# JohannesErnst/WeaSAL

Hardware: AMD Instinct MI355X
Metric: points/sec fwd+bwd KPFCNN on DALES spheres; achieved HBM GB/s on KPConv gather (higher is better)
Workload: dtype f32; 1 GPU; DALES_PseudoLabel KP-FCNN, in_radius=10m, 50k pts/sphere, batch=8, fp32, step = GPU pyramid + fwd + loss + bwd + SGD; contrast_loss term included (trainer_PseudoLabel.py:204-208); pyramid of the next batch overlapped on a second stream; parallelism=dp1, dist_world_size=1, allreduce_bytes=0

## Files before the change

### include/weasal_hip.h

```cpp
#ifndef WEASAL_HIP_H
#define WEASAL_HIP_H

#include <stdint.h>

#ifdef __cplusplus
extern "C" {
#endif

typedef enum {
    WS_OK = 0,
    WS_ERR_INVALID = 1,
    WS_ERR_UNSUPPORTED = 2,
    WS_ERR_HIP = 3,
    WS_ERR_EMPTY = 4,
    WS_ERR_CAPACITY = 5
} ws_status;

enum { WS_INFLUENCE_LINEAR = 0, WS_INFLUENCE_CONSTANT = 1, WS_INFLUENCE_GAUSSIAN = 2 };
enum { WS_AGGREGATION_SUM = 0, WS_AGGREGATION_CLOSEST = 1 };

const char* ws_last_error(void);
int64_t ws_launch_count(void);
const char* ws_version(void);
int ws_device_count(void);
// ... 137 lines not shown
int ws_subsample_ws_create(ws_subsample_ws** ws);
void ws_subsample_ws_destroy(ws_subsample_ws* ws);
int ws_grid_subsample_plan(ws_subsample_ws* ws, const float* points, int64_t n,
                           const int32_t* h_lens, int32_t nb, float dl, int32_t max_p,
                           int32_t order_mode, int32_t* h_out_lens, int64_t* h_m, void* stream);
int ws_grid_subsample_fill(ws_subsample_ws* ws,
                           const float* features, int32_t fd,
                           const int32_t* labels, int32_t ld,
                           float* out_points, float* out_features, int32_t* out_labels,
                           uint64_t* out_keys,
                           int32_t* out_counts,
                           void* stream);

int ws_rotate_clouds(const float* points, int64_t n, const int32_t* lens , int32_t nb,
                     const float* rot , int32_t transpose, float* out, void* stream);

int ws_rotate_clouds_host(const float* points, int64_t n, const int32_t* h_lens, int32_t nb,
                          const float* h_rot, int32_t transpose, float* out, void* stream);

#define WS_PYRAMID_MAX_LEVELS 8
#define WS_PYRAMID_MAX_BATCH 64
typedef struct ws_pyramid_desc {
    int32_t n_levels, nb, want_grids, want_tables;
    const float* points;
    int64_t n0;
    const float* h_rot;
    void* arena; int64_t arena_bytes;
    void* scratch; int64_t scratch_bytes;
    int32_t conv_on[WS_PYRAMID_MAX_LEVELS], pool_on[WS_PYRAMID_MAX_LEVELS];
    float r_conv[WS_PYRAMID_MAX_LEVELS], r_pool[WS_PYRAMID_MAX_LEVELS], r_up[WS_PYRAMID_MAX_LEVELS], dl[WS_PYRAMID_MAX_LEVELS];
    int32_t limit[WS_PYRAMID_MAX_LEVELS + 1];
    int32_t nearest_up;
    int32_t lens[WS_PYRAMID_MAX_LEVELS][WS_PYRAMID_MAX_BATCH];
    int64_t needed_bytes;
    int64_t n[WS_PYRAMID_MAX_LEVELS];
    int64_t off_points[WS_PYRAMID_MAX_LEVELS], off_neighbors[WS_PYRAMID_MAX_LEVELS], off_pools[WS_PYRAMID_MAX_LEVELS],
            off_upsamples[WS_PYRAMID_MAX_LEVELS], off_order[WS_PYRAMID_MAX_LEVELS], off_key_last[WS_PYRAMID_MAX_LEVELS],
            off_blob[WS_PYRAMID_MAX_LEVELS], blob_bytes[WS_PYRAMID_MAX_LEVELS], grid_cells[WS_PYRAMID_MAX_LEVELS];
    int64_t off_lens, off_slots;
    int32_t max_count[3 * WS_PYRAMID_MAX_LEVELS], width[3 * WS_PYRAMID_MAX_LEVELS], final_width[3 * WS_PYRAMID_MAX_LEVELS];
    int32_t cap[3 * WS_PYRAMID_MAX_LEVELS];
    int64_t off_toffsets[3 * WS_PYRAMID_MAX_LEVELS], off_tpairs[3 * WS_PYRAMID_MAX_LEVELS];
} ws_pyramid_desc;
int ws_pyramid_build(ws_neighbors_ws* nws, ws_subsample_ws* sws, ws_pyramid_desc* desc, void* stream);
int64_t ws_pyramid_desc_bytes(void);



int ws_contrast_rows_fwd(const float* on, int64_t n, int32_t c, const float* xs, int32_t s, const int64_t* slc_idx,
                         const uint8_t* certain, const int64_t* lbl, float temperature, float eps, float* loss,
                         float* rowmax, float* den, float* npos, void* stream);
int64_t ws_contrast_rows_bwd_scratch_bytes(int64_t n, int32_t c, int32_t s);
int ws_contrast_rows_bwd(const float* on, int64_t n, int32_t c, const float* xs, int32_t s, const int64_t* slc_idx,
                         const uint8_t* certain, const int64_t* lbl, float temperature, const float* rowmax,
                         const float* den, const float* npos, const float* g, float* d_on, float* d_xs, void* scratch,
                         void* stream);

int64_t ws_contrast_head_scratch_bytes(int64_t n);
int ws_contrast_head_fwd(const float* x, int64_t n, int32_t c, int64_t ldx, const int64_t* labels, float threshold,
                         const float* u, const int64_t* r_given, int32_t s, float* on, float* inv_norm, uint8_t* certain,
                         int64_t* lbl, int64_t* slc_idx, float* xs, int32_t* state, void* scratch, void* stream);
int64_t ws_contrast_tail_scratch_bytes(int64_t n);
int ws_contrast_tail_fwd(const float* pts_loss, const int64_t* lbl, int64_t n, int32_t n_cls, int32_t* state, float* per_class,
                         float* w_cls, float* loss, void* scratch, void* stream);
int ws_contrast_tail_bwd(const float* pts_loss, const int64_t* lbl, int64_t n, int32_t n_cls, const float* w_cls, const float* g,
                         float* g_row, void* stream);
int ws_contrast_head_bwd(float* d_on, const float* d_xs, const int64_t* slc_idx, int32_t s, const float* on,
                         const float* inv_norm, int64_t n, int32_t c, float* d_x, int64_t ldd, void* stream);


int ws_kpconv_gather_fwd_bf16(const float* q_pts, int64_t nq, const float* s_pts, int64_t ns, const int64_t* inds, int32_t h,
                              const uint16_t* x, int32_t ci, const float* kernel_points, int32_t k, const float* deformed_kp,
                              const float* modulations, float extent, int32_t influence, int32_t aggregation,
                              const int32_t* order, uint16_t* wf, float* min_d2, void* stream);
int ws_kpconv_gather_bwd_x_bf16(const float* q_pts, int64_t nq, const float* s_pts, int64_t ns, const int64_t* inds, int32_t h,
                                const int32_t* t_offsets, const int32_t* t_pairs, const uint16_t* dwf, int32_t ci,
                                const float* kernel_points, int32_t k, const float* deformed_kp, const float* modulations,
                                float extent, int32_t influence, int32_t aggregation, const int32_t* order, uint16_t* dx,
                                void* stream);
int ws_kpconv_gather_bwd_x_grid_bf16(const float* s_pts, int64_t ns, const void* grid_blob, int32_t nb, int64_t cells,
                                     const uint64_t* key_last, float radius, const uint16_t* dwf, int32_t ci,
                                     const float* kernel_points, int32_t k, const float* deformed_kp, const float* modulations,
                                     float extent, int32_t influence, int32_t aggregation, const int32_t* order, uint16_t* dx,
                                     int32_t* overflow, void* stream);
int ws_kpconv_gather_bwd_geom_bf16(const float* q_pts, int64_t nq, const float* s_pts, int64_t ns, const int64_t* inds, int32_t h,
                                   const uint16_t* x, int32_t ci, const uint16_t* dwf, const float* kernel_points, int32_t k,
                                   const float* deformed_kp, const float* modulations, const float* d_min_d2, float extent,
                                   int32_t influence, int32_t aggregation, float* d_deformed_kp, float* d_modulations,
                                   void* stream);
int ws_max_pool_fwd_bf16(const uint16_t* x, int64_t ns, int32_t c, const int64_t* inds, int64_t nq, int32_t h,
                         uint16_t* out, int32_t* arg, void* stream);
int ws_max_pool_bwd_bf16(const uint16_t* dy, const int32_t* arg, int64_t nq, int32_t h, int32_t c, const int32_t* t_offsets,
                         const int32_t* t_pairs, int64_t ns, uint16_t* dx, void* stream);
int ws_closest_pool_fwd_bf16(const uint16_t* x, int64_t ns, int32_t c, const int64_t* inds, int64_t nq, int32_t h,
                             uint16_t* out, void* stream);
int ws_closest_pool_bwd_bf16(const uint16_t* dy, int64_t nq, int32_t h, int32_t c, const int32_t* t_offsets,
                             const int32_t* t_pairs, int64_t ns, uint16_t* dx, void* stream);

int ws_gemm_xbt_bf16(const uint16_t* x, int64_t m, int32_t k, int64_t ldx, const uint16_t* bt, int32_t n, int64_t ldbt,
                     const float* bias, const uint16_t* residual, int64_t ldr, int32_t act, float slope,
                     void* y, int64_t ldy, int32_t out_f32, void* stream);
int ws_gemm_xty_bf16(const uint16_t* x, int64_t m, int32_t k, int64_t ldx, const uint16_t* y, int32_t n, int64_t ldy,
                     float* out, void* scratch, void* stream);
int64_t ws_act_bwd_colsum_bf16_scratch_bytes(int64_t m, int32_t n);
int ws_act_bwd_colsum_bf16(const void* dy, int32_t dy_f32, int64_t m, int32_t n, int64_t lddy, const uint16_t* y, int64_t ldy,
                           float slope, uint16_t* dz, int64_t lddz, float* colsum, void* scratch, void* stream);


typedef struct ws_kpblock {
    const float* q_pts; int64_t nq;
    const float* s_pts; int64_t ns;
    const int64_t* inds; int32_t h;
    const float* kernel_points; int32_t k; float extent;
    const int32_t* order_q;
    const int32_t* order_s;
    const void* grid_blob; int32_t grid_nb; int64_t grid_cells; const uint64_t* key_last; float grid_radius;
    int32_t* grid_overflow;
    const int32_t* t_offsets; const int32_t* t_pairs;
    int32_t in_dim, conv_in, conv_out, out_dim, strided;
    float slope;
    const float *w1, *b1, *wk, *bk, *w2, *b2, *ws, *bs;
    const float* feat; float* x1; float* wf; float* x2; float* pooled; int32_t* arg; float* out;
    const float* dout; float* dfeat; float *dw1, *db1, *dwk, *dbk, *dw2, *db2, *dws;
    int32_t timed;
    int32_t rows_sorted;
    int32_t infer;
    int32_t dout_pregated;
    int32_t gate_dfeat;
    const float* dfeat_add;
} ws_kpblock;

int64_t ws_kpblock_fwd_scratch_bytes(const ws_kpblock* d);
int64_t ws_kpblock_bwd_scratch_bytes(const ws_kpblock* d);
int ws_kpblock_fwd(const ws_kpblock* d, void* scratch, int64_t scratch_bytes, void* stream);
int ws_kpblock_bwd(const ws_kpblock* d, void* scratch, int64_t scratch_bytes, void* stream);

typedef struct ws_upunary {
    const float* xc; int64_t nc; int32_t c_up;
    const float* skip; int64_t nf; int32_t c_skip;
    const int64_t* ups; int32_t h_up;
    const int32_t* t_offsets; const int32_t* t_pairs;
    const float* w; int64_t ldw; const float* b; int32_t out_dim; int32_t relu; float slope;
    float* yc; float* out;
    const float* dout; float* dxc; float* dskip; float* dw; float* db;
    float drop_p; uint64_t drop_seed;
    int32_t dout_pregated;
    int32_t gate_dxc;
} ws_upunary;

int64_t ws_upunary_fwd_scratch_bytes(const ws_upunary* d);
int64_t ws_upunary_bwd_scratch_bytes(const ws_upunary* d);
int ws_upunary_fwd(const ws_upunary* d, void* scratch, int64_t scratch_bytes, void* stream);
int ws_upunary_bwd(const ws_upunary* d, void* scratch, int64_t scratch_bytes, void* stream);

int ws_gemm_xb_epilogue_strided(const float* x, int64_t m, int32_t k, int64_t ldx, const float* b, int64_t b_row_stride,
                                int64_t b_col_stride, int32_t n, const float* bias, const float* residual, int64_t ldr,
                                int32_t act, float slope, float* y, int64_t ldy, void* scratch, int64_t scratch_bytes,
                                void* stream);

int ws_gemm_xb_dropout_strided(const float* x, int64_t m, int32_t k, int64_t ldx, const float* b, int64_t b_row_stride,
                               int64_t b_col_stride, int32_t n, const float* bias, const float* residual, int64_t ldr,
                               int32_t act, float slope, float drop_p, uint64_t drop_seed, float* y, int64_t ldy, void* scratch,
                               int64_t scratch_bytes, void* stream);

int ws_gemm_xb_gate_dropout(const float* x, int64_t m, int32_t k, int64_t ldx, const float* b, int32_t n, const float* gate_y,
                            int64_t ldg, float gate_slope, float drop_p, uint64_t drop_seed, float* y, int64_t ldy, void* scratch,
                            int64_t scratch_bytes, void* stream);

int ws_act_bwd_colsum_dropout(const float* dy, int64_t m, int32_t n, int64_t lddy, const float* y, int64_t ldy, float slope,
                              float drop_p, uint64_t drop_seed, float* dz, int64_t lddz, float* colsum, void* scratch, void* stream);

int ws_gemm_xb_gated_strided(const float* x, int64_t m, int32_t k, int64_t ldx, const float* b, int64_t b_row_stride,
                             int64_t b_col_stride, int32_t n, const float* bias, const float* residual, int64_t ldr,
                             int32_t act, float slope, const float* gate_y, int64_t ldg, float gate_slope, const uint8_t* mask,
                             int64_t ldm, float mask_scale, float* y, int64_t ldy, void* scratch, int64_t scratch_bytes,
                             void* stream);

int ws_timer_reset(void);
int ws_timer_count(void);
int ws_timer_read(int32_t i, int64_t* nq, int32_t* h, int32_t* ci, float* ms);
int ws_timer_read_layer(int32_t i, float* ms);


int ws_vote_update(const float* logits, int64_t n, int32_t c, const float* points, float radius_mask, const int64_t* inds,
                   float* probs, int64_t n_cloud, float smooth, void* stream);
int ws_project_confusion(const float* probs, int32_t c, const int32_t* proj, int64_t m, const int32_t* labels, int32_t* preds,
                         int32_t nc, int64_t* confusion, void* stream);
int64_t ws_potentials_scratch_bytes(int64_t n);
int ws_potentials_update(const float* pot_points, int64_t n, const double* h_center, double radius, double* potentials,
                         double* out_min, int64_t* out_argmin, void* scratch, void* stream);

int ws_al_point_scores(const float* probs, int64_t n, int32_t c, const double* class_score, float* entropy, int32_t* preds,
                       double* score, void* stream);
int ws_al_anchor_scores(const float* entropy, const int32_t* preds, int64_t n, const int64_t* anchor_ptr, const int64_t* anchor_idx,
                        int64_t nnz, int64_t n_anchors, const double* class_score, int32_t c, float* out, void* stream);
int64_t ws_topk_scratch_bytes(int64_t n, int64_t k);
int ws_topk_select(const double* score, int64_t n, const int64_t* h_exclude, int64_t m, int64_t k, int64_t* ids, void* scratch,
                   void* stream);

enum { WS_REFINE_BAD_ANCHOR_IDX = 0, WS_REFINE_BAD_ANCHOR_SEL = 1, WS_REFINE_BAD_PROJ = 2, WS_REFINE_STATUS_WORDS = 3 };
int ws_weak_mask(uint32_t* mask, int64_t n, int32_t c, const int64_t* anchor_ptr, const int64_t* anchor_idx, int64_t nnz,
                 const uint32_t* anchor_bits, int64_t n_anchors, const int64_t* anchor_sel, int64_t n_sel, int64_t* status,
                 void* stream);
int ws_refine_labels(const float* probs, const int32_t* preds, int64_t m, int32_t c, const uint32_t* mask, const int32_t* proj,
                     int64_t n, double thr, int32_t no_label, int32_t* labels, int64_t* counts, int32_t n_counts, int64_t* status,
                     void* stream);

enum { WS_ANCHOR_BAD_LABEL = 0, WS_ANCHOR_BAD_SEL = 1, WS_ANCHOR_STATUS_WORDS = 2 };
enum { WS_ANCHOR_TOTAL_ROWS = 0, WS_ANCHOR_TOTAL_NNZ = 1, WS_ANCHOR_TOTAL_BASE = 2, WS_ANCHOR_TOTAL_WORDS = 3 };
int ws_anchor_bounds(const float* points, int64_t n, float* bounds, void* stream);
int64_t ws_anchor_scratch_bytes(int64_t items);
int ws_anchor_members_plan(const float* points, const int32_t* labels, int64_t n, int32_t n_class, const double* anchors, int64_t a0,
                           double radius, const double* h_grid, const int32_t* cell_start, const int32_t* cell_item,
                           int32_t* counts, int32_t* slot, int32_t* ptr32, uint32_t* bits, int64_t* totals, int64_t* status,
                           void* scratch, void* stream);
int ws_anchor_members_fill(const float* points, int64_t n, const double* anchors, int64_t a0, double radius, const double* h_grid,
                           const int32_t* cell_start, const int32_t* cell_item, int32_t* counts, const int32_t* slot,
                           const int32_t* ptr32, const uint32_t* bits, int64_t n_kept, int64_t nnz, int64_t* kept, int64_t* anchor_ptr,
                           int64_t* anchor_idx, double* centres, uint32_t* anchor_bits, int32_t* cursor, void* stream);
int ws_anchor_pairs_plan(const double* centres, int64_t n_anchors, const int64_t* sel, int64_t n_sel, double radius,
                         const double* h_grid, const int32_t* cell_start, const int32_t* cell_item, int32_t* pair_cnt,
                         int32_t* pair_ptr, int64_t* totals, int64_t* status, void* scratch, void* stream);
int ws_anchor_pairs_fill(const double* centres, int64_t n_anchors, const int64_t* sel, int64_t n_sel, double radius,
                         const double* h_grid, const int32_t* cell_start, const int32_t* cell_item, const int32_t* pair_ptr,
                         int64_t n_pairs, int32_t* pair_i, int32_t* pair_j, void* stream);
int ws_anchor_overlap_plan(const int64_t* anchor_ptr, const int64_t* anchor_idx, int64_t nnz, const uint32_t* anchor_bits,
                           int64_t n_anchors, const int64_t* sel, int64_t n_sel, const int32_t* pair_i, const int32_t* pair_j,
                           int64_t n_pairs, int32_t* inter_cnt, int32_t* new_slot, int32_t* new_ptr, int32_t* sel_ptr, int64_t* totals,
                           void* scratch, void* stream);
int ws_anchor_overlap_fill(const float* points, int64_t n, const int64_t* anchor_ptr, const int64_t* anchor_idx, int64_t nnz,
                           const uint32_t* anchor_bits, const double* centres, int64_t n_anchors, const int64_t* sel, int64_t n_sel,
                           const int32_t* pair_i, const int32_t* pair_j, int64_t n_pairs, const int32_t* inter_cnt,
                           const int32_t* new_slot, const int32_t* new_ptr, const int32_t* sel_ptr, int64_t n_new, int64_t nnz_new,
                           int64_t nnz_sel, int64_t* out_ptr, int64_t* out_idx, uint32_t* out_bits, double* out_centres, void* stream);

enum { WS_REGION_TOTAL_ROWS = 0, WS_REGION_TOTAL_NNZ = 1, WS_REGION_BAD_LABEL = 2, WS_REGION_WORDS = 3 };
enum { WS_REGION_MAX_SPHERES = 64, WS_REGION_MAX_WIDTH = 256 };
int64_t ws_region_scratch_bytes(int64_t pairs);
int ws_region_cut_count(const double* centres, const int64_t* anchor_ptr, const int64_t* anchor_idx, int64_t anchor_nnz,
                        int64_t n_anchors, const int32_t* group, int32_t n_group, int32_t n_spheres, const double* sphere_centres,
                        const int64_t* row_off, const int64_t* pair_off, const int64_t* input_inds, int64_t n_rows, int64_t pairs,
                        double radius, int32_t* cnt, void* stream);
int ws_region_cut_scan(int32_t* cnt, int64_t pairs, int32_t* slot, int32_t* ptr32, const int64_t* labels, const int64_t* row_off,
                       int64_t n_rows, int32_t n_spheres, int32_t n_class, float* cloud_lb, int64_t* words, void* scratch, void* stream);
int ws_region_cut_fill(const int64_t* anchor_ptr, const int64_t* anchor_idx, int64_t anchor_nnz, const uint32_t* anchor_bits,
                       int64_t n_anchors, const int32_t* group, int32_t n_group, int32_t n_spheres, const int64_t* row_off,
                       const int64_t* pair_off, const int64_t* input_inds, int64_t n_rows, int64_t pairs, const int32_t* cnt,
                       const int32_t* slot, const int32_t* ptr32, int64_t n_regions, int64_t nnz, int32_t n_class, int64_t* out_ptr,
                       int64_t* out_idx, int32_t* out_reg, int32_t* out_sphere, int64_t* out_anchor, float* out_lb, float* out_inv_len,
                       void* stream);
int ws_region_mean_fwd(const float* x, int64_t n, int32_t w, const int64_t* region_ptr, const int64_t* region_idx, int64_t nnz,
                       const float* inv_len, int64_t n_regions, float* out, void* stream);
int ws_region_mean_bwd(const float* grad_out, int64_t n_regions, int32_t w, const int64_t* t_ptr, const int32_t* t_reg, int64_t nnz,
                       const float* inv_len, int64_t n, float* grad_x, void* stream);

typedef struct ws_sampler ws_sampler;
int ws_sampler_create(ws_sampler** ws);
void ws_sampler_destroy(ws_sampler* ws);
int ws_sampler_add_cloud(ws_sampler* ws, const float* sub_points, const int32_t* sub_labels, int64_t n, const float* pot_points,
                         double* potentials, int64_t p, void* stream);
int64_t ws_sampler_state_bytes(void);
int64_t ws_sampler_draw_bytes(void);
int ws_sampler_batch(ws_sampler* ws, const void* h_draws, int32_t max_spheres, int32_t resume, int64_t batch_limit, double in_radius,
                     float augment_noise, uint64_t seed, uint64_t seq0, int32_t fd, const int32_t* label_lut, int32_t lut_n,
                     int32_t labels_zero, int32_t update_potentials, float* out_points, float* out_features, int64_t* out_labels,
                     int64_t* out_input_inds, int32_t* out_lengths, float* out_scales, float* out_rots, int32_t* out_cloud_inds,
                     int32_t* out_point_inds, int64_t capacity_rows, void* d_state, void* stream);

int ws_dropout_apply(const float* in, int64_t n, float p, uint64_t seed, float* out, void* stream);

int64_t ws_softmax_ce_scratch_bytes(int64_t n);
int ws_softmax_ce_fwd(const float* logits, int64_t n, int32_t c, int64_t ldl, const int64_t* labels, const int64_t* lut,
                      int32_t lut_n, const float* class_w, float* loss, float* wsum, void* scratch, void* stream);
int ws_softmax_ce_bwd(const float* logits, int64_t n, int32_t c, int64_t ldl, const int64_t* labels, const int64_t* lut,
                      int32_t lut_n, const float* class_w, const float* grad_loss, const float* wsum, float* dlogits, int64_t ldd,
                      void* stream);
int ws_sgd_step(float* const* h_params, const float* const* h_grads, float* const* h_bufs, const int64_t* h_sizes, int32_t count,
                float lr, float momentum, float weight_decay, float clip_value, int32_t first, void* stream);

int ws_kpconv_deform_prepare(const float* offset_features, int64_t n, int32_t od, const float* kernel_points, int32_t k,
                             float extent, int32_t modulated, float* deformed_kp, float* modulations, float* kp4, float* kp_rmax,
                             void* stream);
int ws_kpconv_deform_prepare_bwd(const float* d_kp4, const float* d_deformed_kp, const float* kp4, int64_t n, int32_t od, int32_t k,
                                 float extent, int32_t modulated, float* d_offset_features, void* stream);
int ws_kpconv_gather_fwd_def(const float* q_pts, int64_t nq, const float* s_pts, int64_t ns, const int64_t* inds, int32_t h,
                             const void* x, int32_t ci, const float* kp4, int32_t k, float extent, const int32_t* order,
                             void* wf, float* min_d2, int32_t rows_bf16, int32_t rows_sorted, void* stream);
int ws_kpconv_gather_fwd_ex(const float* q_pts, int64_t nq, const float* s_pts, int64_t ns, const int64_t* inds, int32_t h,
                            const void* x, int32_t ci, const float* kernel_points, int32_t k, const float* deformed_kp,
                            const float* modulations, float extent, int32_t influence, int32_t aggregation, const int32_t* order,
                            void* wf, float* min_d2, int32_t rows_bf16, int32_t rows_sorted, void* stream);
int ws_kpconv_gather_bwd_x_def(const float* q_pts, int64_t nq, const float* s_pts, int64_t ns, int32_t h,
                               const int32_t* t_offsets, const int32_t* t_pairs, const void* dwf, int32_t ci, const float* kp4,
                               int32_t k, float extent, const int32_t* order, void* dx, int32_t rows_bf16, void* stream);
int ws_kpconv_gather_bwd_x_grid_wide(const float* s_pts, int64_t ns, const void* grid_blob, int32_t nb, int64_t cells,
                                     const uint64_t* key_last, float radius, const void* dwf, int32_t ci,
                                     const float* kernel_points, int32_t k, const float* kp4, const float* kp_rmax, float extent,
                                     const int32_t* order, const int64_t* rows, int32_t rows_h, void* dx, int32_t rows_bf16,
                                     void* stream);
int ws_kpconv_gather_bwd_geom_def(const float* q_pts, int64_t nq, const float* s_pts, int64_t ns, const int64_t* inds, int32_t h,
                                  const void* x, int32_t ci, const void* dwf, const float* kp4, int32_t k, const float* d_min_d2,
                                  float extent, const int32_t* order, float* d_kp4, int32_t rows_bf16, int32_t rows_sorted,
                                  void* stream);
int ws_kpconv_layer_fwd_fused(const float* q_pts, int64_t nq, const float* s_pts, int64_t ns, const int64_t* inds, int32_t h,
                              const float* x, int32_t ci, const float* kernel_points, int32_t k, float extent,
                              const int32_t* order, const float* weights, int32_t co, const float* bias, int32_t act, float slope,
// ... 47 lines not shown
```

### weasal_amd/_lib.py

```python
import ctypes as C
import os

_HERE = os.path.dirname(os.path.abspath(__file__))
LIB_PATH = os.path.join(_HERE, "libweasal_hip.so")

_vp = C.c_void_p
_i32 = C.c_int32
_i64 = C.c_int64
_f32 = C.c_float

SIGNATURES = {
    "ws_last_error": (C.c_char_p, []),
    "ws_version": (C.c_char_p, []),
    "ws_device_count": (C.c_int, []),
    "ws_kpconv_gather_fwd": (C.c_int, [_vp, _i64, _vp, _i64, _vp, _i32, _vp, _i32, _vp, _i32, _vp, _vp,
                                      _f32, _i32, _i32, _vp, _vp, _vp, _vp]),
    "ws_kpconv_gather_bwd_x": (C.c_int, [_vp, _i64, _vp, _i64, _vp, _i32, _vp, _vp, _vp, _i32, _vp, _i32,
                                        _vp, _vp, _f32, _i32, _i32, _vp, _vp, _vp]),
    "ws_kpconv_gather_bwd_geom": (C.c_int, [_vp, _i64, _vp, _i64, _vp, _i32, _vp, _i32, _vp, _vp, _i32,
                                           _vp, _vp, _vp, _f32, _i32, _i32, _vp, _vp, _vp]),
    "ws_transpose_scratch_bytes": (_i64, [_i64, _i32, _i64]),
    "ws_transpose_build": (C.c_int, [_vp, _i64, _i32, _i64, _vp, _vp, _vp, _vp]),
    "ws_max_pool_fwd": (C.c_int, [_vp, _i64, _i32, _vp, _i64, _i32, _vp, _vp, _vp]),
    "ws_max_pool_bwd": (C.c_int, [_vp, _vp, _i64, _i32, _i32, _vp, _vp, _i64, _vp, _vp]),
    "ws_closest_pool_fwd": (C.c_int, [_vp, _i64, _i32, _vp, _i64, _i32, _vp, _vp]),
    "ws_closest_pool_bwd": (C.c_int, [_vp, _i64, _i32, _i32, _vp, _vp, _i64, _vp, _vp]),
    "ws_gemm_xb": (C.c_int, [_vp, _i64, _i32, _i64, _vp, _i32, _vp, _i64, _vp]),
    "ws_gemm_xb_epilogue": (C.c_int, [_vp, _i64, _i32, _i64, _vp, _i32, _vp, _vp, _i64, _i32, _f32, _vp, _i64, _vp]),
    "ws_act_bwd_colsum_scratch_bytes": (_i64, [_i64, _i32]),
    "ws_act_bwd_colsum": (C.c_int, [_vp, _i64, _i32, _i64, _vp, _i64, C.c_float, _vp, _i64, _vp, _vp, _vp]),
    "ws_contrast_rows_fwd": (C.c_int, [_vp, _i64, _i32, _vp, _i32, _vp, _vp, _vp, C.c_float, C.c_float, _vp, _vp, _vp, _vp, _vp]),
    "ws_contrast_rows_bwd_scratch_bytes": (_i64, [_i64, _i32, _i32]),
    "ws_contrast_rows_bwd": (C.c_int, [_vp, _i64, _i32, _vp, _i32, _vp, _vp, _vp, C.c_float, _vp, _vp, _vp, _vp, _vp, _vp,
                                       _vp, _vp]),
    "ws_launch_count": (_i64, []),
    "ws_radius_neighbors_async_cap": (_i32, [_i32]),
    "ws_radius_neighbors_nearest_async": (C.c_int, [_vp, _vp, _i64, _vp, _i64, _vp, _vp, _i32, C.c_float, _vp, _vp, _vp, _vp]),
    "ws_max_pool_fwd_ordered": (C.c_int, [_vp, _i64, _i32, _vp, _i64, _i32, _vp, _vp, _vp, _vp]),
    "ws_max_pool_bwd_ordered": (C.c_int, [_vp, _vp, _i64, _i32, _i32, _vp, _vp, _i64, _vp, _vp, _vp]),
    "ws_max_pool_fwd_ordered_bf16": (C.c_int, [_vp, _i64, _i32, _vp, _i64, _i32, _vp, _vp, _vp, _vp]),
    "ws_max_pool_bwd_ordered_bf16": (C.c_int, [_vp, _vp, _i64, _i32, _i32, _vp, _vp, _i64, _vp, _vp, _vp]),
    "ws_dropout_apply": (C.c_int, [_vp, _i64, C.c_float, C.c_uint64, _vp, _vp]),
    "ws_gemm_xb_dropout_strided": (C.c_int, [_vp, _i64, _i32, _i64, _vp, _i64, _i64, _i32, _vp, _vp, _i64, _i32, _f32, _f32, C.c_uint64,
                                             _vp, _i64, _vp, _i64, _vp]),
    "ws_gemm_xb_gate_dropout": (C.c_int, [_vp, _i64, _i32, _i64, _vp, _i32, _vp, _i64, _f32, _f32, C.c_uint64, _vp, _i64, _vp, _i64, _vp]),
    "ws_act_bwd_colsum_dropout": (C.c_int, [_vp, _i64, _i32, _i64, _vp, _i64, _f32, _f32, C.c_uint64, _vp, _i64, _vp, _vp, _vp]),
    "ws_pyramid_build": (C.c_int, [_vp, _vp, _vp, _vp]),
    "ws_pyramid_desc_bytes": (_i64, []),
    "ws_contrast_head_scratch_bytes": (_i64, [_i64]),
    "ws_contrast_head_fwd": (C.c_int, [_vp, _i64, _i32, _i64, _vp, C.c_float, _vp, _vp, _i32, _vp, _vp, _vp, _vp, _vp, _vp, _vp,
                                       _vp, _vp]),
    "ws_contrast_tail_scratch_bytes": (_i64, [_i64]),
    "ws_contrast_tail_fwd": (C.c_int, [_vp, _vp, _i64, _i32, _vp, _vp, _vp, _vp, _vp, _vp]),
    "ws_contrast_tail_bwd": (C.c_int, [_vp, _vp, _i64, _i32, _vp, _vp, _vp, _vp]),
    "ws_contrast_head_bwd": (C.c_int, [_vp, _vp, _vp, _i32, _vp, _vp, _i64, _i32, _vp, _i64, _vp]),
    "ws_radius_neighbors_set_key_last": (C.c_int, [_vp, _vp]),
    "ws_radius_neighbors_reuse_grid": (C.c_int, [_vp, _i32]),
    "ws_radius_neighbors_grid_info": (C.c_int, [_vp, _vp, _vp, _vp, _vp]),
    "ws_radius_neighbors_grid_export": (C.c_int, [_vp, _vp, _vp]),
    "ws_kpconv_gather_bwd_x_grid": (C.c_int, [_vp, _i64, _vp, _i32, _i64, _vp, C.c_float, _vp, _i32, _vp, _i32, _vp, _vp,
                                              C.c_float, _i32, _i32, _vp, _vp, _vp, _vp]),
    "ws_gemm_xb_scratch_bytes": (_i64, [_i64, _i32, _i32]),
    "ws_gemm_xb_epilogue_splitk": (C.c_int, [_vp, _i64, _i32, _i64, _vp, _i32, _vp, _vp, _i64, _i32, C.c_float, _vp, _i64,
                                             _vp, _i64, _vp]),
    "ws_gemm_xty_scratch_bytes": (_i64, [_i64, _i32, _i32]),
    "ws_gemm_xty": (C.c_int, [_vp, _i64, _i32, _i64, _vp, _i32, _i64, _vp, _vp, _vp]),
    "ws_neighbors_ws_create": (C.c_int, [C.POINTER(_vp)]),
    "ws_neighbors_ws_destroy": (None, [_vp]),
    "ws_radius_neighbors_plan": (C.c_int, [_vp, _vp, _i64, _vp, _i64, _vp, _vp, _i32, _f32,
                                          C.POINTER(_i32), _vp]),
    "ws_radius_neighbors_fill": (C.c_int, [_vp, _i32, _vp, _vp, _vp]),
    "ws_radius_neighbors_search": (C.c_int, [_vp, _vp, _i64, _vp, _i64, _vp, _vp, _i32, _f32, _i32, _vp, _vp,
                                            C.POINTER(_i32), _vp]),
    "ws_radius_neighbors_search_async": (C.c_int, [_vp, _vp, _i64, _vp, _i64, _vp, _vp, _i32, _f32, _i32, _vp, _vp,
                                                  _vp, _vp]),
    "ws_radius_neighbors_order": (C.c_int, [_vp, _vp, _vp]),
    "ws_radius_neighbors_counts": (_vp, [_vp]),
    "ws_subsample_ws_create": (C.c_int, [C.POINTER(_vp)]),
    "ws_subsample_ws_destroy": (None, [_vp]),
    "ws_grid_subsample_plan": (C.c_int, [_vp, _vp, _i64, _vp, _i32, _f32, _i32, _i32, _vp,
                                        C.POINTER(_i64), _vp]),
    "ws_grid_subsample_fill": (C.c_int, [_vp, _vp, _i32, _vp, _i32, _vp, _vp, _vp, _vp, _vp, _vp]),
    "ws_rotate_clouds": (C.c_int, [_vp, _i64, _vp, _i32, _vp, _i32, _vp, _vp]),
    "ws_rotate_clouds_host": (C.c_int, [_vp, _i64, _vp, _i32, _vp, _i32, _vp, _vp]),
    "ws_kpconv_gather_fwd_bf16": (C.c_int, [_vp, _i64, _vp, _i64, _vp, _i32, _vp, _i32, _vp, _i32, _vp, _vp,
                                           _f32, _i32, _i32, _vp, _vp, _vp, _vp]),
    "ws_kpconv_gather_bwd_x_bf16": (C.c_int, [_vp, _i64, _vp, _i64, _vp, _i32, _vp, _vp, _vp, _i32, _vp, _i32,
                                             _vp, _vp, _f32, _i32, _i32, _vp, _vp, _vp]),
    "ws_kpconv_gather_bwd_geom_bf16": (C.c_int, [_vp, _i64, _vp, _i64, _vp, _i32, _vp, _i32, _vp, _vp, _i32,
                                                _vp, _vp, _vp, _f32, _i32, _i32, _vp, _vp, _vp]),
    "ws_kpconv_gather_bwd_x_grid_bf16": (C.c_int, [_vp, _i64, _vp, _i32, _i64, _vp, C.c_float, _vp, _i32, _vp, _i32, _vp, _vp,
                                                   C.c_float, _i32, _i32, _vp, _vp, _vp, _vp]),
    "ws_max_pool_fwd_bf16": (C.c_int, [_vp, _i64, _i32, _vp, _i64, _i32, _vp, _vp, _vp]),
    "ws_max_pool_bwd_bf16": (C.c_int, [_vp, _vp, _i64, _i32, _i32, _vp, _vp, _i64, _vp, _vp]),
    "ws_closest_pool_fwd_bf16": (C.c_int, [_vp, _i64, _i32, _vp, _i64, _i32, _vp, _vp]),
    "ws_closest_pool_bwd_bf16": (C.c_int, [_vp, _i64, _i32, _i32, _vp, _vp, _i64, _vp, _vp]),
    "ws_gemm_xbt_bf16": (C.c_int, [_vp, _i64, _i32, _i64, _vp, _i32, _i64, _vp, _vp, _i64, _i32, _f32, _vp, _i64, _i32, _vp]),
    "ws_gemm_xty_bf16": (C.c_int, [_vp, _i64, _i32, _i64, _vp, _i32, _i64, _vp, _vp, _vp]),
    "ws_act_bwd_colsum_bf16_scratch_bytes": (_i64, [_i64, _i32]),
    "ws_act_bwd_colsum_bf16": (C.c_int, [_vp, _i32, _i64, _i32, _i64, _vp, _i64, C.c_float, _vp, _i64, _vp, _vp, _vp]),
    "ws_kpblock_fwd_scratch_bytes": (_i64, [_vp]),
    "ws_kpblock_bwd_scratch_bytes": (_i64, [_vp]),
    "ws_kpblock_fwd": (C.c_int, [_vp, _vp, _i64, _vp]),
    "ws_kpblock_bwd": (C.c_int, [_vp, _vp, _i64, _vp]),
    "ws_upunary_fwd_scratch_bytes": (_i64, [_vp]),
    "ws_upunary_bwd_scratch_bytes": (_i64, [_vp]),
    "ws_upunary_fwd": (C.c_int, [_vp, _vp, _i64, _vp]),
    "ws_upunary_bwd": (C.c_int, [_vp, _vp, _i64, _vp]),
    "ws_gemm_xb_epilogue_strided": (C.c_int, [_vp, _i64, _i32, _i64, _vp, _i64, _i64, _i32, _vp, _vp, _i64, _i32, _f32, _vp, _i64,
                                              _vp, _i64, _vp]),
    "ws_gemm_xb_gated_strided": (C.c_int, [_vp, _i64, _i32, _i64, _vp, _i64, _i64, _i32, _vp, _vp, _i64, _i32, _f32, _vp, _i64, _f32,
                                           _vp, _i64, _f32, _vp, _i64, _vp, _i64, _vp]),
    "ws_kpconv_gather_bwd_x_gated": (C.c_int, [_vp, _i64, _vp, _i64, _vp, _i32, _vp, _vp, _vp, _i32, _vp, _i32,
                                              _vp, _vp, _f32, _i32, _i32, _vp, _vp, _f32, _vp, _vp]),
    "ws_kpconv_gather_bwd_x_packed": (C.c_int, [_vp, _i64, _vp, _i64, _vp, _i32, _vp, _vp, _vp, _i32, _vp, _i32,
                                               _vp, _vp, _f32, _i32, _i32, _vp, _vp, _f32, _vp, _vp]),
    "ws_kpconv_gather_bwd_x_packed_variant": (C.c_int, [_i64, _i64, _i32, _i32, _vp, _vp, _i32, _i32, _i32, _i32, _i32, _i32,
                                                       C.c_char_p, _i32]),
    "ws_kpconv_gather_bwd_x_grid_gated": (C.c_int, [_vp, _i64, _vp, _i32, _i64, _vp, C.c_float, _vp, _i32, _vp, _i32, _vp, _vp,
                                                    C.c_float, _i32, _i32, _vp, _vp, _f32, _vp, _i32, _vp, _vp, _vp]),
    "ws_vote_update": (C.c_int, [_vp, _i64, _i32, _vp, _f32, _vp, _vp, _i64, _f32, _vp]),
    "ws_project_confusion": (C.c_int, [_vp, _i32, _vp, _i64, _vp, _vp, _i32, _vp, _vp]),
    "ws_potentials_scratch_bytes": (_i64, [_i64]),
    "ws_potentials_update": (C.c_int, [_vp, _i64, _vp, C.c_double, _vp, _vp, _vp, _vp, _vp]),
    "ws_al_point_scores": (C.c_int, [_vp, _i64, _i32, _vp, _vp, _vp, _vp, _vp]),
    "ws_al_anchor_scores": (C.c_int, [_vp, _vp, _i64, _vp, _vp, _i64, _i64, _vp, _i32, _vp, _vp]),
    "ws_topk_scratch_bytes": (_i64, [_i64, _i64]),
    "ws_topk_select": (C.c_int, [_vp, _i64, _vp, _i64, _i64, _vp, _vp, _vp]),
    "ws_weak_mask": (C.c_int, [_vp, _i64, _i32, _vp, _vp, _i64, _vp, _i64, _vp, _i64, _vp, _vp]),
    "ws_refine_labels": (C.c_int, [_vp, _vp, _i64, _i32, _vp, _vp, _i64, C.c_double, _i32, _vp, _vp, _i32, _vp, _vp]),
    "ws_anchor_bounds": (C.c_int, [_vp, _i64, _vp, _vp]),
    "ws_anchor_scratch_bytes": (_i64, [_i64]),
    "ws_anchor_members_plan": (C.c_int, [_vp, _vp, _i64, _i32, _vp, _i64, C.c_double, _vp, _vp, _vp, _vp, _vp, _vp, _vp, _vp, _vp,
                                        _vp, _vp]),
    "ws_anchor_members_fill": (C.c_int, [_vp, _i64, _vp, _i64, C.c_double, _vp, _vp, _vp, _vp, _vp, _vp, _vp, _i64, _i64, _vp, _vp,
                                        _vp, _vp, _vp, _vp, _vp]),
    "ws_anchor_pairs_plan": (C.c_int, [_vp, _i64, _vp, _i64, C.c_double, _vp, _vp, _vp, _vp, _vp, _vp, _vp, _vp, _vp]),
    "ws_anchor_pairs_fill": (C.c_int, [_vp, _i64, _vp, _i64, C.c_double, _vp, _vp, _vp, _vp, _i64, _vp, _vp, _vp]),
    "ws_anchor_overlap_plan": (C.c_int, [_vp, _vp, _i64, _vp, _i64, _vp, _i64, _vp, _vp, _i64, _vp, _vp, _vp, _vp, _vp, _vp, _vp]),
    "ws_anchor_overlap_fill": (C.c_int, [_vp, _i64, _vp, _vp, _i64, _vp, _vp, _i64, _vp, _i64, _vp, _vp, _i64, _vp, _vp, _vp, _vp,
                                        _i64, _i64, _i64, _vp, _vp, _vp, _vp, _vp]),
    "ws_region_scratch_bytes": (_i64, [_i64]),
    "ws_region_cut_count": (C.c_int, [_vp, _vp, _vp, _i64, _i64, _vp, _i32, _i32, _vp, _vp, _vp, _vp, _i64, _i64, C.c_double, _vp, _vp]),
    "ws_region_cut_scan": (C.c_int, [_vp, _i64, _vp, _vp, _vp, _vp, _i64, _i32, _i32, _vp, _vp, _vp, _vp]),
    "ws_region_cut_fill": (C.c_int, [_vp, _vp, _i64, _vp, _i64, _vp, _i32, _i32, _vp, _vp, _vp, _i64, _i64, _vp, _vp, _vp, _i64, _i64,
                                    _i32, _vp, _vp, _vp, _vp, _vp, _vp, _vp, _vp]),
    "ws_region_mean_fwd": (C.c_int, [_vp, _i64, _i32, _vp, _vp, _i64, _vp, _i64, _vp, _vp]),
    "ws_region_mean_bwd": (C.c_int, [_vp, _i64, _i32, _vp, _vp, _i64, _vp, _i64, _vp, _vp]),
    "ws_sampler_create": (C.c_int, [C.POINTER(_vp)]),
    "ws_sampler_destroy": (None, [_vp]),
    "ws_sampler_add_cloud": (C.c_int, [_vp, _vp, _vp, _i64, _vp, _vp, _i64, _vp]),
    "ws_sampler_state_bytes": (_i64, []),
    "ws_sampler_draw_bytes": (_i64, []),
    "ws_sampler_batch": (C.c_int, [_vp, _vp, _i32, _i32, _i64, C.c_double, _f32, C.c_uint64, C.c_uint64, _i32, _vp, _i32, _i32, _i32,
                                   _vp, _vp, _vp, _vp, _vp, _vp, _vp, _vp, _vp, _i64, _vp, _vp]),
    "ws_softmax_ce_scratch_bytes": (_i64, [_i64]),
    "ws_softmax_ce_fwd": (C.c_int, [_vp, _i64, _i32, _i64, _vp, _vp, _i32, _vp, _vp, _vp, _vp, _vp]),
    "ws_softmax_ce_bwd": (C.c_int, [_vp, _i64, _i32, _i64, _vp, _vp, _i32, _vp, _vp, _vp, _vp, _i64, _vp]),
    "ws_sgd_step": (C.c_int, [_vp, _vp, _vp, _vp, _i32, _f32, _f32, _f32, _f32, _i32, _vp]),
    "ws_kpconv_deform_prepare": (C.c_int, [_vp, _i64, _i32, _vp, _i32, _f32, _i32, _vp, _vp, _vp, _vp, _vp]),
    "ws_kpconv_gather_fwd_ex": (C.c_int, [_vp, _i64, _vp, _i64, _vp, _i32, _vp, _i32, _vp, _i32, _vp, _vp, _f32, _i32, _i32, _vp,
                                         _vp, _vp, _i32, _i32, _vp]),
    "ws_kpconv_deform_prepare_bwd": (C.c_int, [_vp, _vp, _vp, _i64, _i32, _i32, _f32, _i32, _vp, _vp]),
    "ws_kpconv_gather_fwd_def": (C.c_int, [_vp, _i64, _vp, _i64, _vp, _i32, _vp, _i32, _vp, _i32, _f32, _vp, _vp, _vp, _i32, _i32, _vp]),
    "ws_kpconv_gather_bwd_x_def": (C.c_int, [_vp, _i64, _vp, _i64, _i32, _vp, _vp, _vp, _i32, _vp, _i32, _f32, _vp, _vp, _i32, _vp]),
    "ws_kpconv_gather_bwd_x_grid_wide": (C.c_int, [_vp, _i64, _vp, _i32, _i64, _vp, _f32, _vp, _i32, _vp, _i32, _vp, _vp, _f32, _vp,
                                                   _vp, _i32, _vp, _i32, _vp]),
    "ws_kpconv_gather_bwd_geom_def": (C.c_int, [_vp, _i64, _vp, _i64, _vp, _i32, _vp, _i32, _vp, _vp, _i32, _vp, _f32, _vp, _vp,
                                                _i32, _i32, _vp]),
    "ws_kpconv_layer_fwd_fused": (C.c_int, [_vp, _i64, _vp, _i64, _vp, _i32, _vp, _i32, _vp, _i32, _f32, _vp, _vp, _i32, _vp, _i32, _f32,
                                           _vp, _vp]),
    "ws_kpconv_gather_fwd_variant": (C.c_int, [_i32, _i32, _i32, _i32, _i32, _i32, C.c_char_p, _i32]),
    "ws_kpconv_gather_variant": (C.c_int, [_i32, _i64, _i64, _i32, _vp, _vp, _i32, _i32, _i32, _i32, _i32, _i32, _i32, C.c_char_p, _i32]),
    "ws_gemm_xb_variant": (C.c_int, [_vp, _i64, _i32, _i64, _vp, _i64, _i64, _i32, _vp, _vp, _i64, _vp, _i64, _vp, _i64, _vp, _i64,
                                     _vp, _i64, C.c_char_p, _i32]),
    "ws_gemm_xty_variant": (C.c_int, [_vp, _i64, _i32, _i64, _vp, _i32, _i64, _vp, _i64, _vp, _i32, C.c_char_p, _i32]),
    "ws_act_bwd_colsum_variant": (C.c_int, [_vp, _i64, _i32, _i64, _vp, _i64, _vp, _i64, _vp, _vp, C.c_char_p, _i32]),
    "ws_gemm_xbt_bf16_variant": (C.c_int, [_i64, _i32, _i32, _vp, _vp, _i64, _vp, _i64, _i32, C.c_char_p, _i32]),
    "ws_act_bwd_colsum_bf16_variant": (C.c_int, [_i32, _i64, _i32, _vp, _vp, C.c_char_p, _i32]),
    "ws_p2p_regularizer_scratch_bytes": (_i64, [_i64]),
    "ws_p2p_regularizer_fwd": (C.c_int, [_vp, _vp, _vp, _i64, _i32, _f32, _f32, _vp, _vp, _vp]),
    "ws_p2p_regularizer_bwd": (C.c_int, [_vp, _vp, _vp, _i64, _i32, _f32, _f32, _vp, _vp, _vp, _vp]),
    "ws_sphere_attention_fwd": (C.c_int, [_vp, _vp, _vp, _i64, _i32, _i32, _vp, _i32, _vp, _vp, _vp, _vp]),
    "ws_sphere_attention_bwd_scratch_bytes": (_i64, [_i64, _i32]),
    "ws_sphere_attention_bwd": (C.c_int, [_vp, _vp, _vp, _vp, _vp, _vp, _vp, _i64, _i32, _i32, _vp, _i32, _vp, _vp, _vp, _vp, _i64, _vp]),
    "ws_channel_attention_scratch_bytes": (_i64, [_vp, _i32, _i32, _i32]),
    "ws_channel_attention_fwd": (C.c_int, [_vp, _vp, _vp, _i64, _i32, _vp, _i32, _i32, _vp, _vp, _vp, _i64, _vp]),
    "ws_channel_attention_bwd": (C.c_int, [_vp, _vp, _vp, _vp, _vp, _i64, _i32, _vp, _i32, _i32, _vp, _vp, _vp, _vp, _i64, _vp]),
    "ws_timer_reset": (C.c_int, []),
    "ws_timer_count": (C.c_int, []),
    "ws_timer_read": (C.c_int, [_i32, _vp, _vp, _vp, _vp]),
    "ws_timer_read_layer": (C.c_int, [_i32, _vp]),
}

ENV_SWITCHES = (
    ("WEASAL_NB_WIDE_CAPS", "ws_nb_wide_caps"),
    ("WEASAL_CLOSEST_BWD_VEC", "ws_closest_bwd_vec"),
    ("WEASAL_GEMM_STAGED", "ws_gemm_staged"),
    ("WEASAL_GEMM_SHALLOW", "ws_gemm_shallow"),
)

_lib = None


class WeasalHipError(RuntimeError):
    pass


def lib():
    global _lib
    if _lib is None:
        if not os.path.exists(LIB_PATH):
            raise WeasalHipError(
                "%s not found: build it with `python -c 'import __graft_entry__ as g; g.build()'` "
                "or `make -C weasal_amd/csrc` (there is no CPU fallback)" % LIB_PATH)
        handle = C.CDLL(LIB_PATH)
        for name, (res, args) in SIGNATURES.items():
            fn = getattr(handle, name)
            fn.restype = res
            fn.argtypes = args
        for env, sym in ENV_SWITCHES:
            if env in os.environ:
                C.c_int.in_dll(handle, sym).value = int(os.environ[env])
        _lib = handle
    return _lib


def check(rc):
    if rc != 0:
        msg = lib().ws_last_error()
        raise WeasalHipError("libweasal_hip status %d: %s" % (rc, msg.decode() if msg else "?"))


def ptr(t):
    return None if t is None else _vp(t.data_ptr())


_raw_stream = None


def current_stream():
    global _raw_stream
    import torch
    if _raw_stream is None:
        get = getattr(torch._C, "_cuda_getCurrentRawStream", None)
        dev = getattr(torch._C, "_cuda_getDevice", None)
        if get is not None and dev is not None and torch.cuda.is_available():
            torch.cuda.current_stream()
            _raw_stream = lambda: get(dev())
        else:
            _raw_stream = lambda: torch.cuda.current_stream().cuda_stream
    return _vp(_raw_stream())
```

### weasal_amd/architectures.py

```python
import os

import numpy as np
import torch
import torch.nn as nn

from . import fused, ops
from .blocks import KPConv, NearestUpsampleBlock, UnaryBlock, block_decider, closest_pool
from .regions import SphereRegions

_LAYER_CHANGE = ('pool', 'strided', 'upsample', 'global')
REGULARIZER_KERNEL = os.environ.get("WEASAL_REG_KERNEL", "1") != "0"
DROPOUT_KERNEL = os.environ.get("WEASAL_DROPOUT_KERNEL", "1") != "0"
DROPOUT_FUSED = os.environ.get("WEASAL_DROPOUT_FUSED", "1") != "0"
CONTRAST_KERNELS = os.environ.get("WEASAL_CONTRAST_KERNELS", "1") != "0"


def p2p_fitting_regularizer(net):
    fitting_loss = 0
    repulsive_loss = 0
    layers = getattr(net, "_deformable_layers", None)
    if layers is None:
        layers = [m for m in net.modules() if isinstance(m, KPConv) and m.deformable]
        net._deformable_layers = layers
    for m in layers:
        if REGULARIZER_KERNEL and m.min_d2.is_cuda and net.K == 15 and ops.kpconv_gather is ops._KPCONV_GATHER_SELF:
            fr = ops.p2p_regularizer(m.deformed_KP, m.min_d2, m.KP_extent, net.repulse_extent)
            fitting_loss = fitting_loss + fr[0]
            repulsive_loss = repulsive_loss + fr[1]
            continue
        kp_min_d2 = m.min_d2 / (m.KP_extent ** 2)
        fitting_loss = fitting_loss + net.l1(kp_min_d2, torch.zeros_like(kp_min_d2))
        locs = m.deformed_KP / m.KP_extent
        diff = locs.unsqueeze(2) - locs.detach().unsqueeze(1)
        off_diag = ~torch.eye(net.K, dtype=torch.bool, device=locs.device)
        dist = torch.sqrt(torch.sum(diff ** 2, dim=3) + (~off_diag).to(locs.dtype))
        pen = torch.clamp_max(dist - net.repulse_extent, max=0.0) ** 2
        rep = torch.sum(pen * off_diag, dim=2)
        repulsive_loss = repulsive_loss + torch.sum(torch.mean(torch.abs(rep), dim=0)) / net.K
    return net.deform_fitting_power * (2 * fitting_loss + repulsive_loss)


class KPFCNN(nn.Module):

    def __init__(self, config, lbl_values, ign_lbls):
        super(KPFCNN, self).__init__()
        arch = list(config.architecture)
        layer = 0
        r = config.first_subsampling_dl * config.conv_radius
        in_dim = config.in_features_dim
        out_dim = config.first_features_dim
        self.K = config.num_kernel_points
        self.C = len(lbl_values) - len(ign_lbls)

        self.encoder_blocks = nn.ModuleList()
        self.encoder_skip_dims = []
        self.encoder_skips = []
        for block_i, block in enumerate(arch):
            if 'equivariant' in block and out_dim % 3 != 0:
                raise ValueError('Equivariant block but features dimension is not a factor of 3')
            if any(tag in block for tag in _LAYER_CHANGE):
                self.encoder_skips.append(block_i)
                self.encoder_skip_dims.append(in_dim)
            if 'upsample' in block:
                break
            self.encoder_blocks.append(block_decider(block, r, in_dim, out_dim, layer, config))
            in_dim = out_dim // 2 if 'simple' in block else out_dim
            if 'pool' in block or 'strided' in block:
                layer += 1
                r *= 2
                out_dim *= 2

        self.decoder_blocks = nn.ModuleList()
        self.decoder_concats = []
        start_i = next((i for i, b in enumerate(arch) if 'upsample' in b), 0)
        for block_i, block in enumerate(arch[start_i:]):
            if block_i > 0 and 'upsample' in arch[start_i + block_i - 1]:
                in_dim += self.encoder_skip_dims[layer]
                self.decoder_concats.append(block_i)
            self.decoder_blocks.append(block_decider(block, r, in_dim, out_dim, layer, config))
            in_dim = out_dim
            if 'upsample' in block:
                layer -= 1
                r *= 0.5
                out_dim = out_dim // 2

        self.head_mlp = UnaryBlock(out_dim, config.first_features_dim, False, 0)
        self.head_softmax = UnaryBlock(config.first_features_dim, self.C, False, 0)
        self.dropout = config.dropout
        if config.dropout:
            self.droplayer = nn.Dropout(p=float(config.dropout))

        self.valid_labels = np.sort([c for c in lbl_values if c not in ign_lbls])
        if len(config.class_w) > 0:
            class_w = torch.from_numpy(np.array(config.class_w, dtype=np.float32))
            self.criterion = torch.nn.CrossEntropyLoss(weight=class_w, ignore_index=-1)
        else:
            self.criterion = torch.nn.CrossEntropyLoss(ignore_index=-1)
        self.deform_fitting_mode = config.deform_fitting_mode
        self.deform_fitting_power = config.deform_fitting_power
        self.deform_lr_factor = config.deform_lr_factor
        self.repulse_extent = config.repulse_extent
        self.output_loss = 0
        self.reg_loss = 0
        self.l1 = nn.L1Loss()
        self.fuse_decoder = True
        self.feature_dtype = torch.bfloat16 if getattr(config, 'feature_dtype', 'f32') == 'bf16' else torch.float32
        if self.feature_dtype == torch.bfloat16:
            self.head_softmax.out_f32 = True

    def _fused_upsample_unary(self, x, skip, up_block, unary, batch, drop=None):
        if fused.upunary_eligible(x, skip, unary):
            return fused.upunary(x, skip, unary, batch.upsamples[up_block.layer_ind - 1], drop, batch)
        assert drop is None
        c_up = x.shape[1]
        w = unary.mlp.weight
        y = closest_pool(ops.linear(x, w[:, :c_up]), batch.upsamples[up_block.layer_ind - 1])
        return ops.matmul_epilogue(skip, w[:, c_up:].t(), bias=unary.batch_norm.epilogue_bias(), residual=y,
                                   slope=None if unary.no_relu else 0.1)

    def forward(self, batch, config):
        if hasattr(batch, "activate"):
            batch.activate()
        else:
            ops.clear_batch_hints()
        x = batch.features.clone().detach()
        skips = []
        slots = []
        link = None
        for block_i, block_op in enumerate(self.encoder_blocks):
            slot = None
            if block_i in self.encoder_skips:
                skips.append(x)
                slot = fused.SkipSlot()
                slots.append(slot)
            batch.skip_slot = slot
            batch.gate_link_in, batch.gate_link_out = link, fused.GateLink()
            link = batch.gate_link_out
            x = block_op(x, batch)
            batch.skip_slot = None
            batch.gate_link_in = batch.gate_link_out = None
            if block_i == 0 and self.feature_dtype == torch.bfloat16 and x.dtype == torch.float32 and x.shape[1] % 32 == 0:
                x = x.to(torch.bfloat16)
        nd = len(self.decoder_blocks)
        block_i = 0
        dropped = False
        while block_i < nd:
            block_op = self.decoder_blocks[block_i]
            nxt = self.decoder_blocks[block_i + 1] if block_i + 1 < nd else None
            if (self.fuse_decoder and isinstance(block_op, NearestUpsampleBlock) and isinstance(nxt, UnaryBlock)
                    and (block_i + 1) in self.decoder_concats and block_i not in self.decoder_concats):
                drop = None
                if (block_i + 2 == nd and self.dropout and DROPOUT_KERNEL and DROPOUT_FUSED and self.training and not nxt.no_relu
                        and torch.is_grad_enabled() and x.dtype == torch.float32 and fused.upunary_eligible(x, skips[-1], nxt)):
                    drop = (float(self.dropout), int(torch.randint(0, 1 << 62, (1,)).item()))
                    dropped = True
                batch.gate_link_in, batch.gate_link_out = link, fused.GateLink()
                link = batch.gate_link_out
                x = self._fused_upsample_unary(x, fused.skip_tap(skips.pop(), slots.pop()), block_op, nxt, batch, drop)
                batch.gate_link_in = batch.gate_link_out = None
                block_i += 2
                continue
            if block_i in self.decoder_concats:
                x = torch.cat([x, fused.skip_tap(skips.pop(), slots.pop())], dim=1)
            link = None
            x = block_op(x, batch)
            block_i += 1
        if self.dropout and not dropped:
            link = None
            if DROPOUT_KERNEL and self.training and x.is_cuda and x.dtype == torch.float32 and x.requires_grad:
                x = ops.dropout(x, float(self.dropout))
            else:
                x = self.droplayer(x)
        batch.gate_link_in, batch.gate_link_out = link, fused.GateLink()
        link = batch.gate_link_out
        x = self.head_mlp(x, batch)
        batch.gate_link_in, batch.gate_link_out = link, None
        x = self.head_softmax(x, batch)
        batch.gate_link_in = None
        return x

    def _label_lut(self, device):
        lut = getattr(self, "_target_lut", None)
        if lut is None or lut.device != device:
            vmax = int(max(int(np.max(self.valid_labels)) if len(self.valid_labels) else 0, 0))
            lut = -torch.ones(vmax + 2, dtype=torch.int64)
            for i, c in enumerate(self.valid_labels):
                if 0 <= int(c) <= vmax:
                    lut[int(c)] = i
            lut = lut.to(device)
            self._target_lut = lut
        return lut

    def _targets(self, labels):
        lut = self._label_lut(labels.device)
        idx = torch.where((labels >= 0) & (labels < lut.shape[0] - 1), labels, torch.full_like(labels, lut.shape[0] - 1))
        return lut[idx]

    def loss(self, outputs, labels):
        self.output_loss = ops.cross_entropy(outputs, labels, self._label_lut(labels.device), self.criterion.weight)
        if self.deform_fitting_mode == 'point2point':
            self.reg_loss = p2p_fitting_regularizer(self)
        elif self.deform_fitting_mode == 'point2plane':
            raise ValueError('point2plane fitting mode not implemented yet.')
        else:
            raise ValueError('Unknown fitting mode: ' + self.deform_fitting_mode)
        return self.output_loss + self.reg_loss

    def contrast_loss(self, outputs, labels, config, threshold=0.2, slice_draw=None):
        temperature = 0.1
        base_temperature = 1
        slc_con = 1000
        dev = outputs.device
        N = outputs.shape[0]
        eps = 1e-8
        threshold = config.contrast_thd / 100
        self.pts_loss = 0
        self.pts_loss_self = 0

        if CONTRAST_KERNELS and outputs.is_cuda and outputs.dtype == torch.float32 and outputs.shape[1] <= 16:
            if slice_draw is None:
                draw = torch.rand(slc_con, device=dev)
            else:
                slice_draw = slice_draw.to(dev).to(torch.int64)
                nv_host = slc_con - slice_draw.shape[0]
                draw = slice_draw if nv_host <= 0 else torch.cat((torch.arange(nv_host, device=dev), slice_draw), dim=0)
            loss, self.pts_loss, self.contrast_slice, _ = ops.contrast_loss(outputs, labels, draw, threshold, temperature, eps)
            return loss if base_temperature == 1 else loss / base_temperature

        prob = torch.softmax(outputs, 1)
        pseudo_logits = prob.max(1)[0]
        label_id = labels < 10
        certain_label = (pseudo_logits > threshold) | label_id
        pseudo_lbs = torch.argmax(prob, dim=1)
        pseudo_lbs = torch.where(label_id, labels.to(pseudo_lbs.dtype), pseudo_lbs)
        cs = torch.cumsum(certain_label.to(torch.int64), dim=0)
        num_valid = cs[-1]
        j = torch.arange(slc_con, device=dev)
        if slice_draw is None:
            u = torch.rand(slc_con, device=dev)
            r_rand = (u * num_valid.to(torch.float32)).floor().to(torch.int64)
            r = torch.where((num_valid < slc_con) & (j < num_valid), j, r_rand)
        else:
            slice_draw = slice_draw.to(dev).to(torch.int64)
            nv_host = slc_con - slice_draw.shape[0]
            r = slice_draw if nv_host <= 0 else torch.cat((torch.arange(nv_host, device=dev), slice_draw), dim=0)
        r = torch.minimum(r, (num_valid - 1).clamp(min=0).to(torch.int64))
        slc_idx = torch.searchsorted(cs, r + 1).clamp(max=N - 1)

        outputs = nn.functional.normalize(outputs, dim=1)
        pts_loss = ops.contrast_rows(outputs, outputs[slc_idx], slc_idx, certain_label, pseudo_lbs, temperature, eps)
        if base_temperature != 1:
            pts_loss = pts_loss / base_temperature
        keep = (pts_loss > 0).to(pts_loss.dtype)
        n_cls = max(int(outputs.shape[1]), 10)
        sums = torch.zeros(n_cls, dtype=pts_loss.dtype, device=dev).index_add(0, pseudo_lbs, pts_loss * keep)
        cnts = torch.zeros(n_cls, dtype=pts_loss.dtype, device=dev).index_add(0, pseudo_lbs, keep)
        per_class = sums / cnts.clamp(min=1)
        sel = (per_class > 0).to(pts_loss.dtype)
        self.pts_loss = per_class
        loss = (per_class * sel).sum() / sel.sum()
        return torch.where(num_valid > 0, loss, torch.zeros((), dtype=loss.dtype, device=dev))

    def accuracy(self, outputs, labels):
        target = self._targets(labels)
        predicted = torch.argmax(outputs.data, dim=1)
        return (predicted == target).sum().item() / target.size(0)


class KPFCNN_mprm(nn.Module):

    def __init__(self, config, lbl_values, ign_lbls):
        super(KPFCNN_mprm, self).__init__()
        from .blocks import ele_att, global_average_block, multi_path_att
        arch = list(config.architecture)
        layer = 0
        r = config.first_subsampling_dl * config.conv_radius
        in_dim = config.in_features_dim
        out_dim = config.first_features_dim
        self.K = config.num_kernel_points
        self.C = len(lbl_values) - len(ign_lbls)
        self.features_layer = 'encoder_blocks.5.unary_shortcut.mlp'
        self.forward_features = {}
        self.backward_features = {}

        self.encoder_blocks = nn.ModuleList()
        self.encoder_skip_dims = []
        self.encoder_skips = []
        for block_i, block in enumerate(arch):
            if 'equivariant' in block and out_dim % 3 != 0:
                raise ValueError('Equivariant block but features dimension is not a factor of 3')
            if any(tag in block for tag in _LAYER_CHANGE + ('attention',)):
                self.encoder_skips.append(block_i)
                self.encoder_skip_dims.append(in_dim)
            if 'attention' in block or 'upsample' in block:
                break
            self.encoder_blocks.append(block_decider(block, r, in_dim, out_dim, layer, config))
            in_dim = out_dim // 2 if 'simple' in block else out_dim
            if 'pool' in block or 'strided' in block:
                layer += 1
                r *= 2
                out_dim *= 2

        nc = config.num_classes
        self.multi_att = multi_path_att('attention', out_dim, out_dim, r, layer, config)
        self.ele_head = ele_att('ele_attention', 2, out_dim, r, layer, config)
        self.no_ga = global_average_block('ga1', nc, nc, layer, config)
        self.da_ga = global_average_block('ga2', nc, nc, layer, config)
        self.spa_ga = global_average_block('ga3', nc, nc, layer, config)
# ... 121 lines not shown
```

### weasal_amd/csrc/blocks.hip

```cpp
#include <vector>

#include "ws_common.h"

extern "C" int ws_block_gates = 1;
extern "C" int ws_block_gather_residual = 1;
extern "C" int64_t ws_block_group_rows = (int64_t)1 << 62;
extern "C" int ws_block_fused_infer = 1;
extern "C" int ws_block_pool_order = 1;
extern "C" int ws_block_packed_k4 = 1;

namespace {

struct Arena {
    char* base;
    int64_t cap, off;
    Arena(void* b, int64_t c) : base((char*)b), cap(c), off(0) {}
    template <typename T> T* take(int64_t count)
    {
        off = (off + 255) & ~(int64_t)255;
        T* p = base ? reinterpret_cast<T*>(base + off) : nullptr;
        off += count * (int64_t)sizeof(T);
        return p;
    }
    bool fits() const { return off <= cap; }
};

inline int64_t arena_bytes(const Arena& ar) { return ((ar.off + 255) & ~(int64_t)255) + 256; }

inline int64_t max3(int64_t a, int64_t b, int64_t c) { return a > b ? (a > c ? a : c) : (b > c ? b : c); }

__global__ __launch_bounds__(256) void transpose_small_kernel(const float* __restrict__ w, int rows, int cols, int64_t ld,
                                                               float* __restrict__ out)
{
    const int64_t e = (int64_t)blockIdx.x * 256 + threadIdx.x;
    if (e >= (int64_t)rows * cols) return;
    const int c = (int)(e / rows), r = (int)(e % rows);
    out[e] = w[(int64_t)r * ld + c];
}

__global__ __launch_bounds__(256) void add_rows_kernel(float* __restrict__ a, const float* __restrict__ b, int64_t n4)
{
    for (int64_t e = (int64_t)blockIdx.x * 256 + threadIdx.x; e < n4; e += (int64_t)gridDim.x * 256) {
        float4 x = reinterpret_cast<float4*>(a)[e];
        const float4 y = reinterpret_cast<const float4*>(b)[e];
        x.x += y.x; x.y += y.y; x.z += y.z; x.w += y.w;
        reinterpret_cast<float4*>(a)[e] = x;
    }
}

struct Lin {
    const float* w; int n, k; int64_t ldw;
    bool in_place() const { return k % 32 == 0 && n % 4 == 0 && ldw % 4 == 0 && ((uintptr_t)w & 15u) == 0; }
    int64_t tr_floats() const { return in_place() ? 0 : (int64_t)k * n; }
};

int linear_fwd(const Lin& l, const float* x, int64_t m, int64_t ldx, const float* bias, const float* residual, int64_t ldr,
               int act, float slope, float* y, float* tr, void* tmp, int64_t tmp_bytes, hipStream_t st)
{
    if (l.in_place())
        return ws_gemm_xb_epilogue_strided(x, m, l.k, ldx, l.w, 1, l.ldw, l.n, bias, residual, ldr, act, slope, y, l.n, tmp, tmp_bytes, st);
    transpose_small_kernel<<<(unsigned)ws_ceil_div((int64_t)l.k * l.n, 256), 256, 0, st>>>(l.w, l.n, l.k, l.ldw, tr);
    return ws_gemm_xb_epilogue_strided(x, m, l.k, ldx, tr, l.n, 1, l.n, bias, residual, ldr, act, slope, y, l.n, tmp, tmp_bytes, st);
}

#define WS_TRY(call)            \
    do {                        \
        int rc__ = (call);      \
        if (rc__) return rc__;  \
    } while (0)

inline bool grouped_rows(int64_t rows) { return ws_block_group_rows > 0 && rows > 0 && rows < ws_block_group_rows; }

inline ws_xb_problem xb_problem(const float* x, int64_t m, int k, int64_t ldx, const float* b, int64_t brs, int64_t bcs, int n,
                                const float* bias, const float* residual, int64_t ldr, int act, float slope, const float* gate_y,
                                int64_t ldg, float gate_slope, float* y, int64_t ldy, void* scratch, int64_t scratch_bytes)
{
    ws_xb_problem q{};
    q.x = x; q.m = m; q.k = k; q.ldx = ldx; q.b = b; q.b_row_stride = brs; q.b_col_stride = bcs; q.n = n;
    q.bias = bias; q.residual = residual; q.ldr = ldr; q.act = act; q.slope = slope;
    q.gate_y = gate_y; q.ldg = ldg; q.gate_slope = gate_slope;
    q.y = y; q.ldy = ldy; q.scratch = scratch; q.scratch_bytes = scratch_bytes;
    return q;
}

struct Leaves {
    bool on;
    hipStream_t st;
    ws_xty_problem q[4];
    int n = 0;
    Leaves(bool on_, hipStream_t st_) : on(on_), st(st_) {}
    int add(const float* x, int64_t m, int k, int64_t ldx, const float* y, int nn, int64_t ldy, float* out, int64_t ldo, void* scratch,
            int64_t scratch_bytes)
    {
        if (!on) return ws_priv_gemm_xty_pitched(x, m, k, ldx, y, nn, ldy, out, ldo > nn ? ldo : nn, scratch, st);
        WS_REQUIRE(n < 4, "more than 4 collected weight-gradient products");
        q[n++] = ws_xty_problem{x, m, k, ldx, y, nn, ldy, out, ldo, scratch, scratch_bytes};
        return WS_OK;
    }
    int flush()
    {
        const int c = n;
        n = 0;
        return c ? ws_priv_gemm_xty_group(q, c, st) : WS_OK;
    }
};

struct TimerRec { hipEvent_t a, b, c; int64_t nq; int32_t h, ci; };
std::vector<TimerRec>& timer_recs() { static std::vector<TimerRec> v; return v; }

bool arg_bytes(const ws_kpblock* d)
{
    return d->h <= 255 && d->in_dim % 4 == 0 && ((uintptr_t)d->feat & 15u) == 0 && ((uintptr_t)d->pooled & 15u) == 0 &&
           ((uintptr_t)d->arg & 3u) == 0;
}

int check_kpblock(const ws_kpblock* d)
{
    WS_REQUIRE(d, "NULL descriptor");
    WS_REQUIRE(d->nq >= 0 && d->ns >= 0 && d->h >= 1, "bad sizes nq=%lld ns=%lld h=%d", (long long)d->nq, (long long)d->ns, d->h);
    if (d->k != 15) return ws_fail(WS_ERR_UNSUPPORTED, "num_kernel_points=%d: K=15 only", d->k);
    WS_REQUIRE(d->in_dim >= 1 && d->conv_in >= 1 && d->conv_out >= 1 && d->out_dim >= 1, "bad widths");
    WS_REQUIRE(d->q_pts && d->s_pts && d->inds && d->kernel_points && d->feat && d->wk && (d->wf || d->infer) && d->out, "NULL argument");
    WS_REQUIRE(d->w1 ? (d->x1 != nullptr) : (d->conv_in == d->in_dim), "unary1: x1 buffer missing or conv_in != in_dim");
    WS_REQUIRE(d->w2 ? (d->x2 != nullptr) : (d->out_dim == d->conv_out), "unary2: x2 buffer missing or out_dim != conv_out");
    WS_REQUIRE(!d->w2 || d->ws || d->in_dim == d->out_dim, "shortcut needs a projection (ws) when in_dim != out_dim");
    WS_REQUIRE(!d->strided || !d->w2 || (d->pooled && d->arg), "strided block: pooled / arg buffers missing");
    WS_REQUIRE(d->strided || d->nq == d->ns, "non-strided block: nq must equal ns");
    if (d->conv_out % 4 || d->out_dim % 4 || (d->w1 && d->conv_in % 4) || (d->w2 && d->in_dim % 4))
        return ws_fail(WS_ERR_UNSUPPORTED, "block widths must be multiples of 4 (in=%d conv=%d->%d out=%d)", d->in_dim, d->conv_in,
                       d->conv_out, d->out_dim);
    return WS_OK;
}

int64_t kpblock_tmp_fwd(const ws_kpblock* d)
{
    int64_t t = ws_gemm_xb_scratch_bytes(d->nq, d->k * d->conv_in, d->conv_out);
    if (d->w1) t = max3(t, ws_gemm_xb_scratch_bytes(d->ns, d->in_dim, d->conv_in), 0);
    if (d->w2) t = max3(t, ws_gemm_xb_scratch_bytes(d->nq, d->conv_out, d->out_dim), d->ws ? ws_gemm_xb_scratch_bytes(d->nq, d->in_dim, d->out_dim) : 0);
    return t;
}

int kpblock_fwd(const ws_kpblock* d, Arena& ar, hipStream_t st, bool run)
{
    const int64_t nq = d->nq, ns = d->ns;
    const Lin l1{d->w1, d->conv_in, d->in_dim, d->in_dim}, l2{d->w2, d->out_dim, d->conv_out, d->conv_out},
        lsc{d->ws, d->out_dim, d->in_dim, d->in_dim};
    float* tr1 = d->w1 ? ar.take<float>(l1.tr_floats()) : nullptr;
    float* tr2 = d->w2 ? ar.take<float>(l2.tr_floats()) : nullptr;
    float* trs = d->ws ? ar.take<float>(lsc.tr_floats()) : nullptr;
    float* sc = (d->w2 && d->ws) ? ar.take<float>(nq * d->out_dim) : nullptr;
    const int64_t tmp_bytes = kpblock_tmp_fwd(d);
    void* tmp = ar.take<char>(tmp_bytes > 16 ? tmp_bytes : 16);
    const bool pair_in = grouped_rows(nq) && d->w1 && d->w2 && d->ws && !d->strided && l1.in_place() && lsc.in_place();
    const int64_t sc_bytes = pair_in ? ws_gemm_xb_scratch_bytes(nq, d->in_dim, d->out_dim) : 0;
    void* tmp_sc = pair_in ? (void*)ar.take<char>(sc_bytes > 16 ? sc_bytes : 16) : nullptr;
    if (!run) return WS_OK;
    if (nq == 0) return WS_OK;
    const float* x1 = d->feat;
    if (pair_in) {
        const ws_xb_problem q[2] = {
            xb_problem(d->feat, ns, l1.k, d->in_dim, l1.w, 1, l1.ldw, l1.n, d->b1, nullptr, 0, 1, d->slope, nullptr, 0, 0.0f, d->x1, l1.n,
                       tmp, tmp_bytes),
// ... 103 lines not shown
            else WS_HIP(hipMemsetAsync(d->dfeat, 0, sizeof(float) * (size_t)ns * d->in_dim, st));
        }
        return WS_OK;
    }
    bool gated2 = false;
    Leaves leaves(grp, st);
    const float* sc_res = nullptr;
    bool added = false;
    const float* gin = d->dout;
    const float* yconv = d->out;
    WS_REQUIRE(!(d->gate_dfeat && d->dfeat_add && !(d->strided && want_sc)),
               "gate_dfeat with dfeat_add needs the strided shortcut (the sum has to be complete before the gate)");
    if (d->w2) {
        if (d->dout_pregated) {
            if (d->db2) WS_TRY(ws_act_bwd_colsum(d->dout, nq, d->out_dim, d->out_dim, nullptr, 0, 0.0f, nullptr, 0, d->db2, tmp, st));
            dz = const_cast<float*>(d->dout);
        } else
        WS_TRY(ws_act_bwd_colsum(d->dout, nq, d->out_dim, d->out_dim, d->out, d->out_dim, d->slope, dz, d->out_dim, d->db2, tmp, st));
        WS_TRY(leaves.add(dz, nq, d->out_dim, d->out_dim, d->x2, d->conv_out, d->conv_out, d->dw2, 0, t_dw2, b_dw2));
        if (d->ws) {
            const float* sc_in = d->strided ? d->pooled : d->feat;
            WS_TRY(leaves.add(dz, nq, d->out_dim, d->out_dim, sc_in, d->in_dim, d->in_dim, d->dws, 0, t_dws, b_dws));
        }
        gated2 = !d->dbk && ws_block_gates;
        const bool pair_dz = grp && want_sc && d->ws;
        if (pair_dz) {
            const ws_xb_problem q[2] = {
                xb_problem(dz, nq, d->out_dim, d->out_dim, d->ws, d->in_dim, 1, d->in_dim, nullptr, nullptr, 0, 0, 0.0f, nullptr, 0, 0.0f,
                           dscin, d->in_dim, tmp, tmp_bytes),
                xb_problem(dz, nq, d->out_dim, d->out_dim, d->w2, d->conv_out, 1, d->conv_out, nullptr, nullptr, 0, 0, 0.0f,
                           gated2 ? d->x2 : nullptr, d->conv_out, d->slope, g2, d->conv_out, t_g2, b_g2)};
            WS_TRY(ws_priv_gemm_xb_group(q, 2, st));
        }
        if (want_sc) {
            const float* dsc = dz;
            if (d->ws) {
                if (!pair_dz)
                    WS_TRY(ws_gemm_xb_epilogue_strided(dz, nq, d->out_dim, d->out_dim, d->ws, d->in_dim, 1, d->in_dim, nullptr, nullptr, 0,
                                                       0, 0.0f, dscin, d->in_dim, tmp, tmp_bytes, st));
                dsc = dscin;
            }
            if (d->strided) {
                WS_REQUIRE(d->t_offsets && d->t_pairs, "strided block backward needs the transposed table");
                if (arg_bytes(d))
                {
                    WS_TRY(ws_priv_max_pool_bwd_u8(dsc, reinterpret_cast<const uint8_t*>(d->arg), nq, d->h, d->in_dim, d->t_offsets,
                                                   d->t_pairs, ns, dfsc, ws_block_pool_order ? d->order_s : nullptr, d->dfeat_add, st));
                    added = d->dfeat_add != nullptr;
                }
                else {
                    WS_TRY(ws_max_pool_bwd(dsc, d->arg, nq, d->h, d->in_dim, d->t_offsets, d->t_pairs, ns, dfsc, st));
                    if (d->dfeat_add) {
                        WS_REQUIRE(d->in_dim % 4 == 0, "dfeat_add needs in_dim %% 4 == 0");
                        const int64_t n4 = ns * d->in_dim / 4;
                        add_rows_kernel<<<ws_grid(n4, 256), 256, 0, st>>>(dfsc, d->dfeat_add, n4);
                        WS_LAUNCH_CHECK();
                        added = true;
                    }
                }
                sc_res = dfsc;
            } else {
                sc_res = dsc;
            }
        }
        if (!pair_dz)
            WS_TRY(ws_gemm_xb_gated_strided(dz, nq, d->out_dim, d->out_dim, d->w2, d->conv_out, 1, d->conv_out, nullptr, nullptr, 0, 0, 0.0f,
                                            gated2 ? d->x2 : nullptr, d->conv_out, d->slope, nullptr, 0, 0.0f, g2, d->conv_out, tmp,
                                            tmp_bytes, st));
        gin = g2;
        yconv = d->x2;
    }
    if (!d->w2 && d->dout_pregated) {
        if (d->dbk) WS_TRY(ws_act_bwd_colsum(gin, nq, d->conv_out, d->conv_out, nullptr, 0, 0.0f, nullptr, 0, d->dbk, tmp, st));
        g2 = const_cast<float*>(gin);
    } else if (!gated2)
        WS_TRY(ws_act_bwd_colsum(gin, nq, d->conv_out, d->conv_out, yconv, d->conv_out, d->slope, g2, d->conv_out, d->dbk, tmp, st));
    WS_TRY(leaves.add(d->wf, nq, kc, kc, g2, d->conv_out, d->conv_out, d->dwk, 0, t_dwk, b_dwk));
    if (!need_dx1) return leaves.flush();
    WS_TRY(linear_fwd(lk, g2, nq, d->conv_out, nullptr, nullptr, 0, 0, 0.0f, dwf, trk, tmp, tmp_bytes, st));
    float* dx1_out = d->w1 ? dx1 : d->dfeat;
    const float* gate1 = (d->w1 && !d->db1 && ws_block_gates) ? d->x1 : nullptr;
    if (!d->w1 && d->gate_dfeat && d->dfeat) gate1 = d->feat;
    if (d->grid_blob) {
        WS_REQUIRE(d->key_last && d->grid_overflow && nq == ns, "grid backward needs key_last / overflow and a self-query layer");
        WS_TRY(ws_kpconv_gather_bwd_x_grid_gated(d->s_pts, ns, d->grid_blob, d->grid_nb, d->grid_cells, d->key_last, d->grid_radius, dwf,
                                                 d->conv_in, d->kernel_points, d->k, nullptr, nullptr, d->extent, WS_INFLUENCE_LINEAR,
                                                 WS_AGGREGATION_SUM, d->order_s, gate1, d->slope, d->inds, d->h, dx1_out,
                                                 d->grid_overflow, st));
    } else {
        WS_REQUIRE(d->t_offsets && d->t_pairs, "KPConv backward needs the search grid or the transposed table");
        WS_TRY((ws_block_packed_k4 ? ws_kpconv_gather_bwd_x_packed : ws_kpconv_gather_bwd_x_gated)(
            d->q_pts, nq, d->s_pts, ns, d->inds, d->h, d->t_offsets, d->t_pairs, dwf, d->conv_in, d->kernel_points, d->k, nullptr, nullptr,
            d->extent, WS_INFLUENCE_LINEAR, WS_AGGREGATION_SUM, d->order_s, gate1, d->slope, dx1_out, st));
    }
    if (d->w1) {
        if (!gate1)
            WS_TRY(ws_act_bwd_colsum(dx1, ns, d->conv_in, d->conv_in, d->x1, d->conv_in, d->slope, dx1, d->conv_in, d->db1, tmp, st));
        WS_TRY(leaves.add(dx1, ns, d->conv_in, d->conv_in, d->feat, d->in_dim, d->in_dim, d->dw1, 0, t_dw1, b_dw1));
        if (d->dfeat)
            WS_TRY(ws_gemm_xb_gated_strided(dx1, ns, d->conv_in, d->conv_in, d->w1, d->in_dim, 1, d->in_dim, nullptr, sc_res, d->in_dim,
                                            0, 0.0f, d->gate_dfeat ? d->feat : nullptr, d->in_dim, d->slope, nullptr, 0, 0.0f, d->dfeat,
                                            d->in_dim, tmp, tmp_bytes, st));
    } else if (d->dfeat && sc_res) {
        WS_REQUIRE(!d->gate_dfeat, "gate_dfeat: a block without unary1 has no shortcut to add after the gate");
        const int64_t n4 = ns * d->in_dim / 4;
        add_rows_kernel<<<ws_grid(n4, 256), 256, 0, st>>>(d->dfeat, sc_res, n4);
        WS_LAUNCH_CHECK();
    }
    if (d->dfeat && d->dfeat_add && !added) {
        WS_REQUIRE(d->in_dim % 4 == 0, "dfeat_add needs in_dim %% 4 == 0");
        const int64_t n4 = ns * d->in_dim / 4;
        add_rows_kernel<<<ws_grid(n4, 256), 256, 0, st>>>(d->dfeat, d->dfeat_add, n4);
        WS_LAUNCH_CHECK();
    }
    return leaves.flush();
}

int check_upunary(const ws_upunary* d)
{
    WS_REQUIRE(d, "NULL descriptor");
    WS_REQUIRE(d->nc >= 0 && d->nf >= 0 && d->c_up >= 1 && d->c_skip >= 1 && d->out_dim >= 1 && d->h_up >= 1, "bad sizes");
    WS_REQUIRE(d->xc && d->skip && d->ups && d->w && d->out && d->ldw >= d->c_up + d->c_skip, "NULL argument / bad ldw");
    if (d->c_up % 32 || d->c_skip % 32 || d->out_dim % 32 || d->ldw % 4 || ((uintptr_t)d->w & 15u))
        return ws_fail(WS_ERR_UNSUPPORTED, "decoder step: widths must be multiples of 32 (c_up=%d c_skip=%d out=%d)", d->c_up, d->c_skip,
                       d->out_dim);
    WS_REQUIRE(d->drop_p >= 0.0f && d->drop_p < 1.0f, "bad drop probability %g", (double)d->drop_p);
    if (d->drop_p > 0.0f && !d->relu) return ws_fail(WS_ERR_UNSUPPORTED, "decoder step: the fused dropout follows a LeakyReLU (relu = 0)");
    WS_REQUIRE(!(d->dout_pregated && !d->relu), "dout_pregated needs this step's LeakyReLU");
    return WS_OK;
}

int upunary_fwd(const ws_upunary* d, Arena& ar, hipStream_t st, bool run)
{
    float* up = ar.take<float>(d->nf * d->out_dim);
    const int64_t tmp_bytes = max3(ws_gemm_xb_scratch_bytes(d->nc, d->c_up, d->out_dim), ws_gemm_xb_scratch_bytes(d->nf, d->c_skip, d->out_dim), 16);
    void* tmp = ar.take<char>(tmp_bytes);
    if (!run || d->nf == 0) return WS_OK;
    WS_REQUIRE(d->yc, "yc buffer missing");
    if (d->nc > 0)
        WS_TRY(ws_gemm_xb_epilogue_strided(d->xc, d->nc, d->c_up, d->c_up, d->w, 1, d->ldw, d->out_dim, nullptr, nullptr, 0, 0, 0.0f, d->yc,
                                           d->out_dim, tmp, tmp_bytes, st));
    if (ws_block_gather_residual && d->nc > 0)
        return ws_priv_gemm_xb_ex(d->skip, d->nf, d->c_skip, d->c_skip, d->w + d->c_up, 1, d->ldw, d->out_dim, d->b, d->yc, d->out_dim,
                                  d->ups, d->h_up, d->nc, d->relu ? 1 : 0, d->slope, d->drop_p, d->drop_seed, d->out, d->out_dim, tmp,
                                  tmp_bytes, st);
    WS_TRY(ws_closest_pool_fwd(d->yc, d->nc, d->out_dim, d->ups, d->nf, d->h_up, up, st));
    if (d->drop_p > 0.0f)
        return ws_gemm_xb_dropout_strided(d->skip, d->nf, d->c_skip, d->c_skip, d->w + d->c_up, 1, d->ldw, d->out_dim, d->b, up, d->out_dim,
                                          1, d->slope, d->drop_p, d->drop_seed, d->out, d->out_dim, tmp, tmp_bytes, st);
    return ws_gemm_xb_epilogue_strided(d->skip, d->nf, d->c_skip, d->c_skip, d->w + d->c_up, 1, d->ldw, d->out_dim, d->b, up, d->out_dim,
                                       d->relu ? 1 : 0, d->slope, d->out, d->out_dim, tmp, tmp_bytes, st);
}

int upunary_bwd(const ws_upunary* d, Arena& ar, hipStream_t st, bool run)
{
    float* dz = ar.take<float>(d->nf * d->out_dim);
    float* dyc = ar.take<float>(d->nc * d->out_dim);
    int64_t tmp_bytes = max3(ws_act_bwd_colsum_scratch_bytes(d->nf, d->out_dim), ws_gemm_xty_scratch_bytes(d->nf, d->out_dim, d->c_skip),
                             ws_gemm_xty_scratch_bytes(d->nc, d->out_dim, d->c_up));
    tmp_bytes = max3(tmp_bytes, ws_gemm_xb_scratch_bytes(d->nf, d->out_dim, d->c_skip), ws_gemm_xb_scratch_bytes(d->nc, d->out_dim, d->c_up));
    void* tmp = ar.take<char>(tmp_bytes > 16 ? tmp_bytes : 16);
    const bool grp = grouped_rows(d->nf > d->nc ? d->nf : d->nc) && d->nf > 0 && d->nc > 0;
    const int64_t b_skip = ws_gemm_xty_scratch_bytes(d->nf, d->out_dim, d->c_skip), b_up = ws_gemm_xty_scratch_bytes(d->nc, d->out_dim, d->c_up);
    void* t_skip = grp ? (void*)ar.take<char>(b_skip > 16 ? b_skip : 16) : tmp;
    void* t_up = grp ? (void*)ar.take<char>(b_up > 16 ? b_up : 16) : tmp;
    if (!run) return WS_OK;
    WS_REQUIRE(d->dout && d->dw && d->dxc && d->dskip && d->t_offsets && d->t_pairs, "NULL gradient buffer / table");
    const int64_t cw = d->c_up + d->c_skip;
    if (d->nf == 0 || d->nc == 0) {
        WS_HIP(hipMemsetAsync(d->dw, 0, sizeof(float) * (size_t)d->out_dim * cw, st));
        if (d->db) WS_HIP(hipMemsetAsync(d->db, 0, sizeof(float) * d->out_dim, st));
        if (d->nc > 0) WS_HIP(hipMemsetAsync(d->dxc, 0, sizeof(float) * (size_t)d->nc * d->c_up, st));
        if (d->nf > 0) WS_HIP(hipMemsetAsync(d->dskip, 0, sizeof(float) * (size_t)d->nf * d->c_skip, st));
        return WS_OK;
    }
    const float* g = d->dout;
    if (d->relu && d->dout_pregated) {
        if (d->db) WS_TRY(ws_act_bwd_colsum(d->dout, d->nf, d->out_dim, d->out_dim, nullptr, 0, 0.0f, nullptr, 0, d->db, tmp, st));
    } else if (d->drop_p > 0.0f) {
        WS_TRY(ws_act_bwd_colsum_dropout(d->dout, d->nf, d->out_dim, d->out_dim, d->out, d->out_dim, d->slope, d->drop_p, d->drop_seed, dz,
                                         d->out_dim, d->db, tmp, st));
        g = dz;
    } else if (d->relu) {
        WS_TRY(ws_act_bwd_colsum(d->dout, d->nf, d->out_dim, d->out_dim, d->out, d->out_dim, d->slope, dz, d->out_dim, d->db, tmp, st));
        g = dz;
    } else if (d->db) {
        WS_TRY(ws_act_bwd_colsum(d->dout, d->nf, d->out_dim, d->out_dim, nullptr, 0, 0.0f, nullptr, 0, d->db, tmp, st));
    }
    Leaves leaves(grp, (hipStream_t)st);
    WS_TRY(leaves.add(g, d->nf, d->out_dim, d->out_dim, d->skip, d->c_skip, d->c_skip, d->dw + d->c_up, cw, t_skip, b_skip));
    WS_TRY(ws_gemm_xb_epilogue_strided(g, d->nf, d->out_dim, d->out_dim, d->w + d->c_up, d->ldw, 1, d->c_skip, nullptr, nullptr, 0, 0, 0.0f,
                                       d->dskip, d->c_skip, tmp, tmp_bytes, st));
    WS_TRY(ws_closest_pool_bwd(g, d->nf, 1, d->out_dim, d->t_offsets, d->t_pairs, d->nc, dyc, st));
    WS_TRY(leaves.add(dyc, d->nc, d->out_dim, d->out_dim, d->xc, d->c_up, d->c_up, d->dw, cw, t_up, b_up));
    WS_TRY(ws_gemm_xb_gated_strided(dyc, d->nc, d->out_dim, d->out_dim, d->w, d->ldw, 1, d->c_up, nullptr, nullptr, 0, 0, 0.0f,
                                    d->gate_dxc ? d->xc : nullptr, d->c_up, d->slope, nullptr, 0, 0.0f, d->dxc, d->c_up, tmp, tmp_bytes, st));
    return leaves.flush();
}

}

extern "C" {

int64_t ws_kpblock_fwd_scratch_bytes(const ws_kpblock* d)
{
    if (check_kpblock(d)) return -1;
    Arena ar(nullptr, 0);
    kpblock_fwd(d, ar, nullptr, false);
    return arena_bytes(ar);
}

int64_t ws_kpblock_bwd_scratch_bytes(const ws_kpblock* d)
{
    if (check_kpblock(d)) return -1;
    Arena ar(nullptr, 0);
    kpblock_bwd(d, ar, nullptr, false);
    return arena_bytes(ar);
}

int ws_kpblock_fwd(const ws_kpblock* d, void* scratch, int64_t scratch_bytes, void* stream)
{
    WS_TRY(check_kpblock(d));
    WS_REQUIRE(scratch && ((uintptr_t)scratch & 15u) == 0, "scratch must be a 16-byte aligned device buffer");
    Arena plan(nullptr, 0);
    kpblock_fwd(d, plan, nullptr, false);
    if (arena_bytes(plan) > scratch_bytes) return ws_fail(WS_ERR_CAPACITY, "scratch too small: %lld < %lld bytes", (long long)scratch_bytes, (long long)arena_bytes(plan));
    Arena ar(scratch, scratch_bytes);
    return kpblock_fwd(d, ar, (hipStream_t)stream, true);
}

int ws_kpblock_bwd(const ws_kpblock* d, void* scratch, int64_t scratch_bytes, void* stream)
{
    WS_TRY(check_kpblock(d));
    WS_REQUIRE(scratch && ((uintptr_t)scratch & 15u) == 0, "scratch must be a 16-byte aligned device buffer");
    Arena plan(nullptr, 0);
    kpblock_bwd(d, plan, nullptr, false);
    if (arena_bytes(plan) > scratch_bytes) return ws_fail(WS_ERR_CAPACITY, "scratch too small: %lld < %lld bytes", (long long)scratch_bytes, (long long)arena_bytes(plan));
    Arena ar(scratch, scratch_bytes);
    return kpblock_bwd(d, ar, (hipStream_t)stream, true);
}

int64_t ws_upunary_fwd_scratch_bytes(const ws_upunary* d)
{
    if (check_upunary(d)) return -1;
    Arena ar(nullptr, 0);
    upunary_fwd(d, ar, nullptr, false);
    return arena_bytes(ar);
}

int64_t ws_upunary_bwd_scratch_bytes(const ws_upunary* d)
{
    if (check_upunary(d)) return -1;
    Arena ar(nullptr, 0);
    upunary_bwd(d, ar, nullptr, false);
    return arena_bytes(ar);
}

int ws_upunary_fwd(const ws_upunary* d, void* scratch, int64_t scratch_bytes, void* stream)
{
    WS_TRY(check_upunary(d));
    WS_REQUIRE(scratch && ((uintptr_t)scratch & 15u) == 0, "scratch must be a 16-byte aligned device buffer");
    Arena plan(nullptr, 0);
    upunary_fwd(d, plan, nullptr, false);
    if (arena_bytes(plan) > scratch_bytes) return ws_fail(WS_ERR_CAPACITY, "scratch too small: %lld < %lld bytes", (long long)scratch_bytes, (long long)arena_bytes(plan));
    Arena ar(scratch, scratch_bytes);
    return upunary_fwd(d, ar, (hipStream_t)stream, true);
}

int ws_upunary_bwd(const ws_upunary* d, void* scratch, int64_t scratch_bytes, void* stream)
{
    WS_TRY(check_upunary(d));
    WS_REQUIRE(scratch && ((uintptr_t)scratch & 15u) == 0, "scratch must be a 16-byte aligned device buffer");
    Arena plan(nullptr, 0);
    upunary_bwd(d, plan, nullptr, false);
    if (arena_bytes(plan) > scratch_bytes) return ws_fail(WS_ERR_CAPACITY, "scratch too small: %lld < %lld bytes", (long long)scratch_bytes, (long long)arena_bytes(plan));
    Arena ar(scratch, scratch_bytes);
    return upunary_bwd(d, ar, (hipStream_t)stream, true);
}

int ws_timer_reset(void)
{
    for (auto& r : timer_recs()) {
        (void)hipEventDestroy(r.a);
        (void)hipEventDestroy(r.b);
        (void)hipEventDestroy(r.c);
    }
    timer_recs().clear();
    return WS_OK;
}

int ws_timer_count(void) { return (int)timer_recs().size(); }

int ws_timer_read(int32_t i, int64_t* nq, int32_t* h, int32_t* ci, float* ms)
{
    WS_REQUIRE(i >= 0 && i < (int)timer_recs().size() && nq && h && ci && ms, "bad timer record index %d", i);
    const TimerRec& r = timer_recs()[i];
    WS_HIP(hipEventSynchronize(r.b));
    WS_HIP(hipEventElapsedTime(ms, r.a, r.b));
    *nq = r.nq; *h = r.h; *ci = r.ci;
    return WS_OK;
}

int ws_timer_read_layer(int32_t i, float* ms)
{
    WS_REQUIRE(i >= 0 && i < (int)timer_recs().size() && ms, "bad timer record index %d", i);
    const TimerRec& r = timer_recs()[i];
    WS_HIP(hipEventSynchronize(r.c));
    WS_HIP(hipEventElapsedTime(ms, r.a, r.c));
    return WS_OK;
}

}
```

### weasal_amd/csrc/gemm.hip

```cpp
#include "ws_common.h"
#include "ws_bf16.h"

namespace {

typedef float f32x16 __attribute__((ext_vector_type(16)));

constexpr int BM = 128;
constexpr int BK = 32;

struct XbGate {
    const float* y; int64_t ld; float slope;
    const uint8_t* mask; int64_t ldm; float mscale;
    WsDrop drop; int64_t dn;
    const int64_t* rrows; int64_t rld; int64_t rn;
};
__device__ __forceinline__ const float* xb_res_row(const float* residual, int64_t ldr, const XbGate& g, int64_t row)
{
    if (!residual) return nullptr;
    if (!g.rrows) return residual + row * ldr;
    const int64_t i = g.rrows[row * g.rld];
    return (i >= 0 && i < g.rn) ? residual + i * ldr : nullptr;
}
__device__ __forceinline__ void xb_gate4(float4& v, const XbGate& g, int64_t row, int col)
{
// ... 336 lines not shown
        load_x(c + 1 < last ? c + 1 : last);
        load_w(c + 2 < last ? c + 2 : last);
        const float* wb = &Ws[((c - cbeg) & 1) * WBUF + wn * (NT * 1024) + (h * 32 + idx) * 4];
#pragma unroll
        for (int j = 0; j < 4; ++j) {
            __builtin_amdgcn_sched_barrier(0);
#pragma unroll
            for (int i = 0; i < NT; ++i) {
                const float4 a4 = *reinterpret_cast<const float4*>(wb + (i * 4 + j) * 256);
                acc[i] = __builtin_amdgcn_mfma_f32_32x32x2f32(a4.x, xc[j].x, acc[i], 0, 0, 0);
                acc[i] = __builtin_amdgcn_mfma_f32_32x32x2f32(a4.y, xc[j].y, acc[i], 0, 0, 0);
                acc[i] = __builtin_amdgcn_mfma_f32_32x32x2f32(a4.z, xc[j].z, acc[i], 0, 0, 0);
                acc[i] = __builtin_amdgcn_mfma_f32_32x32x2f32(a4.w, xc[j].w, acc[i], 0, 0, 0);
            }
        }
        __syncthreads();
    }
    if (staged) {
        const int64_t row0 = (int64_t)bx * (32 * WM) + wm * 32;
        float* stage = &Ws[wave * XB_STAGE_FLOATS];
        if (partial)
            xb_rows_epilogue_staged<NT>(acc, row0, m, n0 + wn * (32 * NT), n, lane, partial + (int64_t)bz * m * n, n, nullptr,
                                        nullptr, 0, 0, 0.0f, XbGate{}, stage);
        else
            xb_rows_epilogue_staged<NT>(acc, row0, m, n0 + wn * (32 * NT), n, lane, y, ldy, bias, residual, ldr, act, slope, gate, stage);
        return;
    }
    if (partial)
        xb_rows_epilogue<NT>(acc, row, m, n0 + wn * (32 * NT), n, h, partial + (int64_t)bz * m * n, n, nullptr, nullptr, 0,
                             0, 0.0f, XbGate{});
    else
        xb_rows_epilogue<NT>(acc, row, m, n0 + wn * (32 * NT), n, h, y, ldy, bias, residual, ldr, act, slope, gate);
}

template <int NT, int WN>
__global__ __launch_bounds__(256) __attribute__((amdgpu_waves_per_eu(3))) void gemm_xb2_kernel(
    const float* __restrict__ x, int64_t m, int k, int64_t ldx, const float* __restrict__ b, int n, int ldb, int bcs,
    float* __restrict__ y, int64_t ldy, const float* __restrict__ bias, const float* __restrict__ residual, int64_t ldr,
    int act, float slope, int csplit, float* __restrict__ partial, const XbGate gate, int staged)
{
    gemm_xb2_body<NT, WN>(blockIdx.x, blockIdx.y, blockIdx.z, x, m, k, ldx, b, n, ldb, bcs, y, ldy, bias, residual, ldr, act, slope,
                          csplit, partial, gate, staged);
}

constexpr int GROUP_MAX = 8;
struct GroupIndex { unsigned end[GROUP_MAX]; };
__device__ __forceinline__ int group_find(const GroupIndex& gi, unsigned& local)
{
    const unsigned b = blockIdx.x;
    int i = 0;
    unsigned beg = 0;
#pragma unroll
    for (int j = 0; j < GROUP_MAX - 1; ++j) {
        const bool past = b >= gi.end[j];
        i += past ? 1 : 0;
        beg = past ? gi.end[j] : beg;
    }
    local = b - beg;
    return i;
}

struct Xb2Problem {
    const float* x; int64_t m; int64_t ldx; const float* b; float* y; int64_t ldy; const float* bias; const float* residual;
    int64_t ldr; float* partial; XbGate gate;
    int k, n, ldb, bcs, act, csplit, staged; float slope;
    unsigned gx, gy;
};
struct Xb2Group { GroupIndex gi; Xb2Problem p[GROUP_MAX]; };
static_assert(sizeof(Xb2Group) < 4096, "the group travels in the kernel arguments");

template <int NT, int WN>
__global__ __launch_bounds__(256) __attribute__((amdgpu_waves_per_eu(3))) void gemm_xb2_group_kernel(const Xb2Group g)
{
    unsigned l;
    const Xb2Problem& p = g.p[group_find(g.gi, l)];
    const unsigned gx = p.gx, gy = p.gy;
    const unsigned bx = l % gx, q = l / gx;
    gemm_xb2_body<NT, WN>(bx, q % gy, q / gy, p.x, p.m, p.k, p.ldx, p.b, p.n, p.ldb, p.bcs, p.y, p.ldy, p.bias, p.residual, p.ldr,
                          p.act, p.slope, p.csplit, p.partial, p.gate, p.staged);
}

__global__ __launch_bounds__(256) void gemm_xb_shallow_kernel(const float* __restrict__ x, int64_t m, int k, int64_t ldx,
                                                               const float* __restrict__ b, int n, float* __restrict__ y, int64_t ldy,
                                                               const float* __restrict__ bias, const float* __restrict__ residual,
                                                               int64_t ldr, int act, float slope, const XbGate gate, int rows_per_wg)
{
    extern __shared__ __attribute__((aligned(16))) float shallow_lds[];
    const int kp = (k + 3) & ~3;
    float* bs = shallow_lds;
    float* xs = shallow_lds + kp * n;
    const int t = threadIdx.x;
    for (int e = t; e < kp * n / 4; e += 256)
        reinterpret_cast<float4*>(bs)[e] = e < k * n / 4 ? reinterpret_cast<const float4*>(b)[e] : make_float4(0.f, 0.f, 0.f, 0.f);
    const int64_t r0 = (int64_t)blockIdx.x * rows_per_wg;
    const int64_t r1 = r0 + rows_per_wg < m ? r0 + rows_per_wg : m;
    const int nrows = (int)(r1 - r0);
    {
        int r = t / kp, kk = t - r * kp;
        const int dr = 256 / kp, dk = 256 - dr * kp;
        for (int e = t; e < nrows * kp; e += 256) {
            xs[e] = kk < k ? x[(r0 + r) * ldx + kk] : 0.0f;
            r += dr; kk += dk;
            if (kk >= kp) { kk -= kp; ++r; }
        }
    }
    __syncthreads();
    const int n4 = n >> 2;
    const int per = 256 / n4;
    const int c = (t % n4) * 4, rl = t / n4;
    if (rl >= per) return;
    float4 bq = make_float4(0.f, 0.f, 0.f, 0.f);
    if (bias) bq = *reinterpret_cast<const float4*>(bias + c);
    for (int rb = rl; rb < nrows; rb += 4 * per) {
        float4 v[4];
        const float* xr[4];
#pragma unroll
        for (int u = 0; u < 4; ++u) {
            v[u] = make_float4(0.f, 0.f, 0.f, 0.f);
            const int r = rb + u * per;
            xr[u] = xs + (r < nrows ? r : rb) * kp;
        }
        for (int kk = 0; kk < kp; kk += 4) {
            const float4 w0 = *reinterpret_cast<const float4*>(&bs[kk * n + c]);
            const float4 w1 = *reinterpret_cast<const float4*>(&bs[(kk + 1) * n + c]);
            const float4 w2 = *reinterpret_cast<const float4*>(&bs[(kk + 2) * n + c]);
            const float4 w3 = *reinterpret_cast<const float4*>(&bs[(kk + 3) * n + c]);
#pragma unroll
            for (int u = 0; u < 4; ++u) {
                const float4 a = *reinterpret_cast<const float4*>(xr[u] + kk);
                v[u].x = fmaf(a.x, w0.x, v[u].x); v[u].y = fmaf(a.x, w0.y, v[u].y); v[u].z = fmaf(a.x, w0.z, v[u].z); v[u].w = fmaf(a.x, w0.w, v[u].w);
                v[u].x = fmaf(a.y, w1.x, v[u].x); v[u].y = fmaf(a.y, w1.y, v[u].y); v[u].z = fmaf(a.y, w1.z, v[u].z); v[u].w = fmaf(a.y, w1.w, v[u].w);
                v[u].x = fmaf(a.z, w2.x, v[u].x); v[u].y = fmaf(a.z, w2.y, v[u].y); v[u].z = fmaf(a.z, w2.z, v[u].z); v[u].w = fmaf(a.z, w2.w, v[u].w);
                v[u].x = fmaf(a.w, w3.x, v[u].x); v[u].y = fmaf(a.w, w3.y, v[u].y); v[u].z = fmaf(a.w, w3.z, v[u].z); v[u].w = fmaf(a.w, w3.w, v[u].w);
            }
        }
#pragma unroll
        for (int u = 0; u < 4; ++u) {
            const int r = rb + u * per;
            if (r >= nrows) break;
            const int64_t row = r0 + r;
            float4 o = v[u];
            if (residual) {
                const float* rrow = xb_res_row(residual, ldr, gate, row);
                if (rrow) { const float4 rq = *reinterpret_cast<const float4*>(rrow + c); o.x += rq.x; o.y += rq.y; o.z += rq.z; o.w += rq.w; }
            }
            o.x += bq.x; o.y += bq.y; o.z += bq.z; o.w += bq.w;
            if (act) {
                o.x = o.x > 0.0f ? o.x : o.x * slope; o.y = o.y > 0.0f ? o.y : o.y * slope;
                o.z = o.z > 0.0f ? o.z : o.z * slope; o.w = o.w > 0.0f ? o.w : o.w * slope;
            }
            if (gate.y || gate.mask || gate.drop.on) xb_gate4(o, gate, row, c);
            *reinterpret_cast<float4*>(y + row * ldy + c) = o;
        }
    }
}

__device__ __forceinline__ void splitk_epilogue_body(const unsigned bx, const unsigned nb, const float* __restrict__ partial, int splits,
                                                     int64_t m, int n, float* __restrict__ y, int64_t ldy,
                                                     const float* __restrict__ bias, const float* __restrict__ residual, int64_t ldr,
                                                     int act, float slope, const XbGate& gate)
{
    const int n4 = n >> 2;
    const int64_t total = m * n4;
    for (int64_t e = (int64_t)bx * 256 + threadIdx.x; e < total; e += (int64_t)nb * 256) {
        const int64_t r = e / n4;
        const int c = (int)(e % n4) * 4;
        float4 v = *reinterpret_cast<const float4*>(partial + r * n + c);
        for (int z = 1; z < splits; ++z) {
            const float4 p = *reinterpret_cast<const float4*>(partial + ((int64_t)z * m + r) * n + c);
            v.x += p.x; v.y += p.y; v.z += p.z; v.w += p.w;
        }
        if (bias) { const float4 bq = *reinterpret_cast<const float4*>(bias + c); v.x += bq.x; v.y += bq.y; v.z += bq.z; v.w += bq.w; }
        if (residual) {
            const float* rrow = xb_res_row(residual, ldr, gate, r);
            if (rrow) {
                const float4 rq = *reinterpret_cast<const float4*>(rrow + c);
                v.x += rq.x; v.y += rq.y; v.z += rq.z; v.w += rq.w;
            }
        }
        if (act) {
            v.x = v.x > 0.0f ? v.x : v.x * slope; v.y = v.y > 0.0f ? v.y : v.y * slope;
            v.z = v.z > 0.0f ? v.z : v.z * slope; v.w = v.w > 0.0f ? v.w : v.w * slope;
        }
        xb_gate4(v, gate, r, c);
        *reinterpret_cast<float4*>(y + r * ldy + c) = v;
    }
}

__global__ __launch_bounds__(256) void splitk_epilogue_kernel(const float* __restrict__ partial, int splits, int64_t m, int n,
                                                               float* __restrict__ y, int64_t ldy, const float* __restrict__ bias,
                                                               const float* __restrict__ residual, int64_t ldr, int act, float slope,
                                                               const XbGate gate)
{
    splitk_epilogue_body(blockIdx.x, gridDim.x, partial, splits, m, n, y, ldy, bias, residual, ldr, act, slope, gate);
}

struct SplitkProblem {
    const float* partial; int64_t m; float* y; int64_t ldy; const float* bias; const float* residual; int64_t ldr; XbGate gate;
    int splits, n, act; float slope; unsigned nb;
};
struct SplitkGroup { GroupIndex gi; SplitkProblem p[GROUP_MAX]; };
static_assert(sizeof(SplitkGroup) < 4096, "the group travels in the kernel arguments");
__global__ __launch_bounds__(256) void splitk_epilogue_group_kernel(const SplitkGroup g)
{
    unsigned l;
    const SplitkProblem& p = g.p[group_find(g.gi, l)];
    splitk_epilogue_body(l, p.nb, p.partial, p.splits, p.m, p.n, p.y, p.ldy, p.bias, p.residual, p.ldr, p.act, p.slope, p.gate);
}

template <int NT, int KT>
__global__ __launch_bounds__(256) void gemm_xty_kernel(const float* __restrict__ x, int64_t m, int k, int64_t ldx,
                                                        const float* __restrict__ yy, int n, int64_t ldy,
                                                        float* __restrict__ partial, int64_t chunk, int vecx, int vecy)
{
    constexpr int BN = 32 * NT;
    constexpr int BKO = 32 * KT;
    constexpr int RG = 4 / KT;
    constexpr int XS_FLOATS = BK * BKO, YS_FLOATS = BK * BN;
    constexpr int RED_FLOATS = (RG > 1) ? KT * NT * 16 * 64 : 0;
    constexpr int LDS_FLOATS = (XS_FLOATS + YS_FLOATS) > RED_FLOATS ? (XS_FLOATS + YS_FLOATS) : RED_FLOATS;
    __shared__ __attribute__((aligned(16))) float lds[LDS_FLOATS];
    float (*Xs)[BKO] = reinterpret_cast<float (*)[BKO]>(lds);
    float (*Ys)[BN] = reinterpret_cast<float (*)[BN]>(lds + XS_FLOATS);
    const int t = threadIdx.x;
    const int wave = __builtin_amdgcn_readfirstlane(t >> 6);
    const int lane = t & 63;
    const int kt = wave % KT, rg = wave / KT;
    const int k0 = blockIdx.y * BKO;
    const int n0 = blockIdx.z * BN;
    const int64_t mbeg = (int64_t)blockIdx.x * chunk;
    const int64_t mend = mbeg + chunk < m ? mbeg + chunk : m;
    constexpr int XPT = (XS_FLOATS / 4 + 255) / 256;
    constexpr int YPT = (YS_FLOATS / 4 + 255) / 256;
    f32x16 acc[NT];
#pragma unroll
    for (int i = 0; i < NT; ++i)
#pragma unroll
        for (int r = 0; r < 16; ++r) acc[i][r] = 0.0f;

    float4 xv[XPT], yv[YPT];
    auto load_tiles = [&](int64_t r0) {
#pragma unroll
        for (int i = 0; i < XPT; ++i) {
            const int idx = t + 256 * i;
            const int rr = idx / (BKO / 4), cc = (idx % (BKO / 4)) * 4;
            xv[i] = (rr < BK) ? ld4_guard(x, r0 + rr, mend, k0 + cc, k, ldx, vecx) : make_float4(0.f, 0.f, 0.f, 0.f);
        }
#pragma unroll
        for (int i = 0; i < YPT; ++i) {
            const int idx = t + 256 * i;
            const int rr = idx / (BN / 4), cc = (idx % (BN / 4)) * 4;
            yv[i] = (rr < BK) ? ld4_guard(yy, r0 + rr, mend, n0 + cc, n, ldy, vecy) : make_float4(0.f, 0.f, 0.f, 0.f);
        }
    };
    auto store_tiles = [&]() {
#pragma unroll
        for (int i = 0; i < XPT; ++i) {
            const int idx = t + 256 * i;
            const int rr = idx / (BKO / 4), cc = (idx % (BKO / 4)) * 4;
            if (rr < BK) *reinterpret_cast<float4*>(&Xs[rr][cc]) = xv[i];
        }
#pragma unroll
        for (int i = 0; i < YPT; ++i) {
            const int idx = t + 256 * i;
            const int rr = idx / (BN / 4), cc = (idx % (BN / 4)) * 4;
            if (rr < BK) *reinterpret_cast<float4*>(&Ys[rr][cc]) = yv[i];
        }
    };

    load_tiles(mbeg);
    const int ai = kt * 32 + (lane & 31), kk = lane >> 5, bj = lane & 31;
    for (int64_t r0 = mbeg; r0 < mend; r0 += BK) {
        store_tiles();
        __syncthreads();
        if (r0 + BK < mend) load_tiles(r0 + BK);
#pragma unroll
        for (int ss = 0; ss < BK / 2 / RG; ++ss) {
            const int s = ss * RG + rg;
            const float a = Xs[2 * s + kk][ai];
#pragma unroll
            for (int i = 0; i < NT; ++i) {
                const float bb = Ys[2 * s + kk][32 * i + bj];
                acc[i] = __builtin_amdgcn_mfma_f32_32x32x2f32(a, bb, acc[i], 0, 0, 0);
            }
        }
        __syncthreads();
    }
    if (RG > 1) {
        float* red = lds;
        for (int src = 1; src < RG; ++src) {
            if (rg == src) {
#pragma unroll
                for (int i = 0; i < NT; ++i)
#pragma unroll
                    for (int r = 0; r < 16; ++r) red[((kt * NT + i) * 16 + r) * 64 + lane] = acc[i][r];
            }
            __syncthreads();
            if (rg == 0) {
#pragma unroll
                for (int i = 0; i < NT; ++i)
#pragma unroll
                    for (int r = 0; r < 16; ++r) acc[i][r] += red[((kt * NT + i) * 16 + r) * 64 + lane];
            }
            __syncthreads();
        }
    }
// ... 604 lines not shown
int ws_gemm_xb_dropout_strided(const float* x, int64_t m, int32_t k, int64_t ldx, const float* b, int64_t b_row_stride,
                               int64_t b_col_stride, int32_t n, const float* bias, const float* residual, int64_t ldr,
                               int32_t act, float slope, float drop_p, uint64_t drop_seed, float* y, int64_t ldy, void* scratch,
                               int64_t scratch_bytes, void* stream)
{
    WS_REQUIRE(drop_p >= 0.0f && drop_p < 1.0f, "bad drop probability %g", (double)drop_p);
    XbGate gate{};
    gate.drop = ws_drop_args(drop_p, drop_seed);
    gate.dn = n;
    return gemm_xb_impl(x, m, k, ldx, b, n, bias, residual, ldr, act, slope, y, ldy, scratch, scratch_bytes, stream,
                        b_row_stride, b_col_stride, gate);
}

int ws_gemm_xb_gate_dropout(const float* x, int64_t m, int32_t k, int64_t ldx, const float* b, int32_t n, const float* gate_y,
                            int64_t ldg, float gate_slope, float drop_p, uint64_t drop_seed, float* y, int64_t ldy, void* scratch,
                            int64_t scratch_bytes, void* stream)
{
    WS_REQUIRE(drop_p >= 0.0f && drop_p < 1.0f, "bad drop probability %g", (double)drop_p);
    WS_REQUIRE(!gate_y || ldg >= n, "gate leading dimension too small");
    XbGate gate{};
    gate.y = gate_y; gate.ld = ldg; gate.slope = gate_slope;
    gate.drop = ws_drop_args(drop_p, drop_seed);
    gate.dn = n;
    return gemm_xb_impl(x, m, k, ldx, b, n, nullptr, nullptr, 0, 0, 0.0f, y, ldy, scratch, scratch_bytes, stream, -1, 1, gate);
}

int ws_priv_gemm_xb_ex(const float* x, int64_t m, int32_t k, int64_t ldx, const float* b, int64_t b_row_stride, int64_t b_col_stride,
                       int32_t n, const float* bias, const float* residual, int64_t ldr, const int64_t* res_rows, int64_t res_rows_ld,
                       int64_t res_nrows, int32_t act, float slope, float drop_p, uint64_t drop_seed, float* y, int64_t ldy,
                       void* scratch, int64_t scratch_bytes, void* stream)
{
    WS_REQUIRE(drop_p >= 0.0f && drop_p < 1.0f, "bad drop probability %g", (double)drop_p);
    WS_REQUIRE(!res_rows || (residual && res_rows_ld >= 1 && res_nrows >= 0), "gathered residual: NULL residual / bad sizes");
    XbGate gate{};
    gate.drop = ws_drop_args(drop_p, drop_seed);
    gate.dn = n;
    gate.rrows = res_rows; gate.rld = res_rows_ld; gate.rn = res_nrows;
    return gemm_xb_impl(x, m, k, ldx, b, n, bias, residual, ldr, act, slope, y, ldy, scratch, scratch_bytes, stream,
                        b_row_stride, b_col_stride, gate);
}

static XbGate xb_problem_gate(const ws_xb_problem& q)
{
    XbGate g{};
    g.y = q.gate_y; g.ld = q.ldg; g.slope = q.gate_slope;
    g.mask = q.mask; g.ldm = q.ldm; g.mscale = q.mask_scale;
    g.drop = ws_drop_args(q.drop_p, q.drop_seed);
    g.dn = q.n;
    g.rrows = q.res_rows; g.rld = q.res_rows_ld; g.rn = q.res_nrows;
    return g;
}
static int xb_problem_alone(const ws_xb_problem& q, void* stream)
{
    return gemm_xb_impl(q.x, q.m, q.k, q.ldx, q.b, q.n, q.bias, q.residual, q.ldr, q.act, q.slope, q.y, q.ldy, q.scratch, q.scratch_bytes,
                        stream, q.b_row_stride, q.b_col_stride, xb_problem_gate(q));
}
constexpr int GROUP_CALL_MAX = 16;
struct IdList {
    int n = 0;
    int v[GROUP_CALL_MAX];
    void push_back(int i) { v[n++] = i; }
    int size() const { return n; }
    const int* data() const { return v; }
    int operator[](int i) const { return v[i]; }
};
constexpr int64_t GROUP_MEMBER_BLOCKS = 1ll << 27;

static int xb2_group_launch(const ws_xb_problem* q, const XbPlan* plan, const int* ids, int cnt, hipStream_t st)
{
    Xb2Group g{};
    SplitkGroup e{};
    int ne = 0, last_e = -1;
    unsigned total = 0, etotal = 0;
    for (int j = 0; j < cnt; ++j) {
        const ws_xb_problem& a = q[ids[j]];
        const XbPlan& p = plan[ids[j]];
        const XbGate gate = xb_problem_gate(a);
        float* part = p.splits > 1 ? (float*)a.scratch : nullptr;
        g.p[j] = Xb2Problem{a.x, a.m, a.ldx, a.b, a.y, a.ldy, a.bias, a.residual, a.ldr, part, gate, a.k, a.n,
                            (int)(a.b_row_stride < 0 ? a.n : a.b_row_stride), (int)a.b_col_stride, a.act, p.csplit, p.staged, a.slope,
                            p.grid.x, p.grid.y};
        total += p.grid.x * p.grid.y * p.grid.z;
        g.gi.end[j] = total;
        if (p.splits > 1) {
            const unsigned nb = (unsigned)ws_grid(a.m * (a.n / 4), 256);
            e.p[ne] = SplitkProblem{part, a.m, a.y, a.ldy, a.bias, a.residual, a.ldr, gate, p.splits, a.n, a.act, a.slope, nb};
            etotal += nb;
            e.gi.end[ne++] = etotal;
            last_e = ids[j];
        }
    }
    for (int j = cnt; j < GROUP_MAX; ++j) g.gi.end[j] = total;
    for (int j = ne; j < GROUP_MAX; ++j) e.gi.end[j] = etotal;
    const XbPlan& p0 = plan[ids[0]];
    if (p0.wn == 1) {
        if (p0.nt == 1) gemm_xb2_group_kernel<1, 1><<<total, 256, 0, st>>>(g);
        else if (p0.nt == 2) gemm_xb2_group_kernel<2, 1><<<total, 256, 0, st>>>(g);
        else gemm_xb2_group_kernel<4, 1><<<total, 256, 0, st>>>(g);
    } else {
        if (p0.nt == 1) gemm_xb2_group_kernel<1, 2><<<total, 256, 0, st>>>(g);
        else gemm_xb2_group_kernel<2, 2><<<total, 256, 0, st>>>(g);
    }
    WS_LAUNCH_CHECK();
    if (ne == 1) {
        const SplitkProblem& s1 = e.p[0];
        splitk_epilogue_kernel<<<s1.nb, 256, 0, st>>>(s1.partial, s1.splits, s1.m, s1.n, s1.y, s1.ldy, s1.bias, s1.residual, s1.ldr, s1.act,
                                                      s1.slope, xb_problem_gate(q[last_e]));
        WS_HIP(hipGetLastError());
    } else if (ne > 1) {
        splitk_epilogue_group_kernel<<<etotal, 256, 0, st>>>(e);
        WS_LAUNCH_CHECK();
    }
    return WS_OK;
}

int ws_priv_gemm_xb_group(const ws_xb_problem* q, int32_t count, void* stream)
{
    WS_REQUIRE(count >= 0 && (q || count == 0), "bad group");
    for (; count > GROUP_CALL_MAX; q += GROUP_CALL_MAX, count -= GROUP_CALL_MAX) {
        const int rc = ws_priv_gemm_xb_group(q, GROUP_CALL_MAX, stream);
        if (rc != WS_OK) return rc;
    }
    hipStream_t st = (hipStream_t)stream;
    XbPlan plan[GROUP_CALL_MAX];
    IdList bucket[5];
    for (int i = 0; i < count; ++i) {
        const ws_xb_problem& a = q[i];
        WS_REQUIRE(a.m >= 0 && a.k >= 1 && a.n >= 1 && a.ldx >= a.k && a.ldy >= a.n, "member %d: bad sizes m=%lld k=%d n=%d", i, (long long)a.m, a.k, a.n);
        WS_REQUIRE(!a.residual || a.ldr >= a.n, "member %d: residual leading dimension too small", i);
        WS_REQUIRE(a.act == 0 || a.act == 1, "member %d: unknown activation %d", i, a.act);
        WS_REQUIRE(a.drop_p >= 0.0f && a.drop_p < 1.0f, "member %d: bad drop probability %g", i, (double)a.drop_p);
        WS_REQUIRE(!a.res_rows || (a.residual && a.res_rows_ld >= 1 && a.res_nrows >= 0), "member %d: gathered residual: NULL residual / bad sizes", i);
        WS_REQUIRE(!a.gate_y || a.ldg >= a.n, "member %d: gate leading dimension too small", i);
        WS_REQUIRE(!a.mask || a.ldm >= a.n, "member %d: mask leading dimension too small", i);
        if (a.m == 0) continue;
        WS_REQUIRE(a.x && a.b && a.y, "member %d: NULL argument", i);
        const int rc = xb_plan(a.x, a.m, a.k, a.ldx, a.b, a.n, a.bias, a.residual, a.ldr, a.y, a.ldy, a.scratch, a.scratch_bytes,
                               a.b_row_stride < 0 ? a.n : a.b_row_stride, a.b_col_stride, xb_problem_gate(a), plan[i]);
        if (rc != WS_OK) return rc;
        const XbPlan& p = plan[i];
        if (p.kind != XB_XB2 || (int64_t)p.grid.x * p.grid.y * p.grid.z >= GROUP_MEMBER_BLOCKS) {
            const int r1 = xb_problem_alone(a, stream);
            if (r1 != WS_OK) return r1;
            continue;
        }
        bucket[p.wn == 1 ? (p.nt == 1 ? 0 : p.nt == 2 ? 1 : 2) : (p.nt == 1 ? 3 : 4)].push_back(i);
    }
    for (const IdList& ids : bucket)
        for (int off = 0; off < ids.size(); off += GROUP_MAX) {
            const int cnt = ids.size() - off < GROUP_MAX ? ids.size() - off : GROUP_MAX;
            const int rc = cnt == 1 ? xb_problem_alone(q[ids[off]], stream) : xb2_group_launch(q, plan, ids.data() + off, cnt, st);
            if (rc != WS_OK) return rc;
        }
    return WS_OK;
}

int ws_gemm_xb(const float* x, int64_t m, int32_t k, int64_t ldx, const float* b, int32_t n, float* y, int64_t ldy,
               void* stream)
{
    return gemm_xb_impl(x, m, k, ldx, b, n, nullptr, nullptr, 0, 0, 0.0f, y, ldy, nullptr, 0, stream);
}

int64_t ws_gemm_xty_scratch_bytes(int64_t m, int32_t k, int32_t n)
{
    const int64_t rows = m > 0 ? m : 1;
    return ws_ceil_div(rows, xty_chunk(rows, k, n)) * (int64_t)k * n * (int64_t)sizeof(float);
}

static int gemm_xty_core(const float* x, int64_t m, int32_t k, int64_t ldx, const float* y, int32_t n, int64_t ldy,
                         float* out, void* scratch, void* stream, int64_t ldo = 0);

int ws_gemm_xty(const float* x, int64_t m, int32_t k, int64_t ldx, const float* y, int32_t n, int64_t ldy,
                float* out, void* scratch, void* stream)
{
    return gemm_xty_core(x, m, k, ldx, y, n, ldy, out, scratch, stream);
}

struct XtyPlan {
    int lds;
    int kt, nt, wk, wn;
    int vecx, vecy;
    int64_t chunk;
    int chunks;
    float* partial;
    int reduce;
    bool pitched;
    dim3 grid;
};

static int xty_plan(const void* x, int64_t m, int32_t k, int64_t ldx, const void* y, int32_t n, int64_t ldy, float* out, void* scratch,
                    int64_t ldo, bool bf16, XtyPlan& p)
{
    p = XtyPlan{};
    p.pitched = ldo > n;
    if (m == 0) return WS_OK;
    p.chunk = xty_chunk(m, k, n);
    p.chunks = (int)ws_ceil_div(m, p.chunk);
    const int64_t span = p.chunk * (ldx > ldy ? ldx : ldy);
    if (bf16) WS_REQUIRE(span * 2 < (1ll << 31), "operand exceeds the 32-bit buffer offsets");
    p.partial = (p.chunks == 1 && !p.pitched) ? out : (float*)scratch;
    p.lds = !bf16 && span * 4 >= (1ll << 31);
    if (!p.lds) {
        const bool a2x = bf16 ? (reinterpret_cast<uintptr_t>(x) & 3u) == 0 && ldx % 2 == 0 && k % 2 == 0
                              : (reinterpret_cast<uintptr_t>(x) & 7u) == 0 && ldx % 2 == 0;
        const bool a2y = bf16 ? (reinterpret_cast<uintptr_t>(y) & 3u) == 0 && ldy % 2 == 0 && n % 2 == 0
                              : (reinterpret_cast<uintptr_t>(y) & 7u) == 0 && ldy % 2 == 0;
        p.kt = (k > 32 && a2x) ? 2 : 1;
        p.nt = (n > 32 && a2y) ? 2 : 1;
        p.wk = k > 32 * p.kt ? 2 : 1;
        p.wn = (n > 32 * p.nt && p.wk == 1) || (n > 32 * p.nt && k > 32 * p.kt) ? 2 : 1;
        p.grid = dim3(p.chunks, (unsigned)ws_ceil_div(k, 32 * p.kt * p.wk), (unsigned)ws_ceil_div(n, 32 * p.nt * p.wn));
    } else {
        p.vecx = al16(x) && (ldx % 4 == 0);
        p.vecy = al16(y) && (ldy % 4 == 0);
        p.kt = k <= 32 ? 1 : (k <= 64 ? 2 : 4);
        p.nt = n <= 32 ? 1 : (n <= 64 ? 2 : 4);
        p.grid = dim3(p.chunks, (unsigned)ws_ceil_div(k, 32 * p.kt), (unsigned)ws_ceil_div(n, 32 * p.nt));
    }
    if (p.chunks > 1 || p.pitched)
        p.reduce = reduce_partials_wide(p.partial, (int64_t)k * n, p.chunks, out, n, p.pitched ? ldo : 0) ? 2 : 1;
    return WS_OK;
}

static void xty_product_launch(const XtyPlan& p, const float* x, int64_t m, int32_t k, int64_t ldx, const float* y, int32_t n, int64_t ldy,
                               hipStream_t st);

static int gemm_xty_core(const float* x, int64_t m, int32_t k, int64_t ldx, const float* y, int32_t n, int64_t ldy,
                         float* out, void* scratch, void* stream, int64_t ldo)
{
    const bool pitched = ldo > n;
    WS_REQUIRE(m >= 0 && k >= 1 && n >= 1 && ldx >= k && ldy >= n, "bad sizes m=%lld k=%d n=%d", (long long)m, k, n);
    WS_REQUIRE(out, "NULL argument");
    hipStream_t st = (hipStream_t)stream;
    if (m == 0) {
        if (pitched) WS_HIP(hipMemset2DAsync(out, sizeof(float) * (size_t)ldo, 0, sizeof(float) * (size_t)n, (size_t)k, st));
        else WS_HIP(hipMemsetAsync(out, 0, sizeof(float) * (size_t)k * n, st));
        return WS_OK;
    }
    WS_REQUIRE(x && y && scratch, "NULL argument");
    XtyPlan p;
    const int rc = xty_plan(x, m, k, ldx, y, n, ldy, out, scratch, ldo, false, p);
    if (rc != WS_OK) return rc;
    xty_product_launch(p, x, m, k, ldx, y, n, ldy, st);
    WS_LAUNCH_CHECK();
    if (p.reduce) {
        const int64_t elems = (int64_t)k * n;
        launch_reduce_partials(p.partial, elems, p.chunks, out, st, n, pitched ? ldo : 0);
        WS_LAUNCH_CHECK();
    }
    return WS_OK;
}

static void xty_product_launch(const XtyPlan& p, const float* x, int64_t m, int32_t k, int64_t ldx, const float* y, int32_t n, int64_t ldy,
                               hipStream_t st)
{
    if (!p.lds) {
#define WS_XTY2(KTV, NTV, WKV, WNV) gemm_xty2_kernel<KTV, NTV, WKV, WNV><<<p.grid, 256, 0, st>>>(x, m, k, ldx, y, n, ldy, p.partial, p.chunk)
#define WS_XTY2_W(KTV, NTV)                          \
    do {                                             \
        if (p.wk == 2 && p.wn == 2) WS_XTY2(KTV, NTV, 2, 2); \
        else if (p.wk == 2) WS_XTY2(KTV, NTV, 2, 1);   \
        else if (p.wn == 2) WS_XTY2(KTV, NTV, 1, 2);   \
        else WS_XTY2(KTV, NTV, 1, 1);                \
    } while (0)
        if (p.kt == 2 && p.nt == 2) WS_XTY2_W(2, 2);
        else if (p.kt == 2) WS_XTY2_W(2, 1);
        else if (p.nt == 2) WS_XTY2_W(1, 2);
        else WS_XTY2_W(1, 1);
#undef WS_XTY2_W
#undef WS_XTY2
    } else {
#define WS_XTY(NTV, KTV) gemm_xty_kernel<NTV, KTV><<<p.grid, 256, 0, st>>>(x, m, k, ldx, y, n, ldy, p.partial, p.chunk, p.vecx, p.vecy)
#define WS_XTY_K(NTV)                    \
    do {                                 \
        if (p.kt == 1) WS_XTY(NTV, 1);     \
        else if (p.kt == 2) WS_XTY(NTV, 2); \
        else WS_XTY(NTV, 4);             \
    } while (0)
        if (p.nt == 1) WS_XTY_K(1);
        else if (p.nt == 2) WS_XTY_K(2);
        else WS_XTY_K(4);
#undef WS_XTY_K
#undef WS_XTY
    }
}

int ws_priv_gemm_xty_pitched(const float* x, int64_t m, int32_t k, int64_t ldx, const float* y, int32_t n, int64_t ldy, float* out,
                             int64_t ldo, void* scratch, void* stream)
{
    WS_REQUIRE(ldo >= n, "output pitch smaller than a row");
    return gemm_xty_core(x, m, k, ldx, y, n, ldy, out, scratch, stream, ldo);
}

static int xty2_group_launch(const ws_xty_problem* q, const XtyPlan* plan, const int* ids, int cnt, hipStream_t st)
{
    Xty2Group g{};
    unsigned total = 0;
    for (int j = 0; j < cnt; ++j) {
        const ws_xty_problem& a = q[ids[j]];
        const XtyPlan& p = plan[ids[j]];
        g.p[j] = Xty2Problem{a.x, a.m, a.ldx, a.y, a.ldy, p.partial, p.chunk, a.k, a.n, p.grid.x, p.grid.y};
        total += p.grid.x * p.grid.y * p.grid.z;
        g.gi.end[j] = total;
    }
    for (int j = cnt; j < GROUP_MAX; ++j) g.gi.end[j] = total;
    const XtyPlan& p0 = plan[ids[0]];
// ... 200 lines not shown
```

### weasal_amd/csrc/ws_common.h

```cpp
#pragma once
#include <hip/hip_runtime.h>
#include <stdint.h>
#include <stdio.h>
#include <stdarg.h>
#include "../../include/weasal_hip.h"

#define WS_WAVE 64

char* ws_errbuf();
inline int ws_fail(int code, const char* fmt, ...)
{
    va_list ap;
    va_start(ap, fmt);
    vsnprintf(ws_errbuf(), 512, fmt, ap);
    va_end(ap);
    return code;
}

#define WS_HIP(call)                                                                     \
    do {                                                                                 \
        hipError_t e__ = (call);                                                         \
        if (e__ != hipSuccess)                                                           \
            return ws_fail(WS_ERR_HIP, "%s failed: %s (%s:%d)", #call, hipGetErrorString(e__), \
                           __FILE__, __LINE__);                                          \
    } while (0)

#define WS_REQUIRE(cond, ...)                                   \
    do {                                                        \
        if (!(cond)) return ws_fail(WS_ERR_INVALID, __VA_ARGS__); \
    } while (0)

extern "C" long long ws_launch_counter;
#define WS_LAUNCH_CHECK()                         \
    do {                                          \
        __atomic_fetch_add(&ws_launch_counter, 1ll, __ATOMIC_RELAXED); \
        WS_HIP(hipGetLastError());                \
    } while (0)

static inline int64_t ws_ceil_div(int64_t a, int64_t b) { return (a + b - 1) / b; }

extern "C" int ws_priv_max_pool_fwd_u8(const float* x, int64_t ns, int32_t c, const int64_t* inds, int64_t nq, int32_t h, float* out,
                                       uint8_t* arg, const int32_t* order_q, void* stream);
extern "C" int ws_priv_max_pool_bwd_u8(const float* dy, const uint8_t* arg, int64_t nq, int32_t h, int32_t c, const int32_t* t_offsets,
                                       const int32_t* t_pairs, int64_t ns, float* dx, const int32_t* order_s, const float* add,
                                       void* stream);

extern "C" int ws_priv_gemm_xb_ex(const float* x, int64_t m, int32_t k, int64_t ldx, const float* b, int64_t b_row_stride, int64_t b_col_stride,
                                  int32_t n, const float* bias, const float* residual, int64_t ldr, const int64_t* res_rows,
                                  int64_t res_rows_ld, int64_t res_nrows, int32_t act, float slope, float drop_p, uint64_t drop_seed,
                                  float* y, int64_t ldy, void* scratch, int64_t scratch_bytes, void* stream);

extern "C" int ws_priv_gemm_xty_pitched(const float* x, int64_t m, int32_t k, int64_t ldx, const float* y, int32_t n, int64_t ldy,
                                        float* out, int64_t ldo, void* scratch, void* stream);

struct ws_xb_problem {
    const float* x; int64_t m; int32_t k; int64_t ldx;
    const float* b; int64_t b_row_stride, b_col_stride; int32_t n;
    const float* bias; const float* residual; int64_t ldr;
    const int64_t* res_rows; int64_t res_rows_ld, res_nrows;
    int32_t act; float slope;
    const float* gate_y; int64_t ldg; float gate_slope;
    const uint8_t* mask; int64_t ldm; float mask_scale;
    float drop_p; uint64_t drop_seed;
    float* y; int64_t ldy;
    void* scratch; int64_t scratch_bytes;
};
struct ws_xty_problem {
    const float* x; int64_t m; int32_t k; int64_t ldx;
    const float* y; int32_t n; int64_t ldy;
    float* out; int64_t ldo;
    void* scratch; int64_t scratch_bytes;
};
extern "C" int ws_priv_gemm_xb_group(const ws_xb_problem* p, int32_t count, void* stream);
extern "C" int ws_priv_gemm_xty_group(const ws_xty_problem* p, int32_t count, void* stream);

static inline int ws_grid(int64_t items, int per_block, int max_blocks = 256 * 16)
{
    int64_t b = ws_ceil_div(items, per_block);
    if (b < 1) b = 1;
    if (b > max_blocks) b = max_blocks;
    if (b > 8) b = (b + 7) / 8 * 8;
    return (int)b;
}

#ifdef __HIPCC__
__device__ __forceinline__ int ws_lane() { return threadIdx.x & 63; }
__device__ __forceinline__ float ws_readlane_f(float v, int lane)
{
    return __int_as_float(__builtin_amdgcn_readlane(__float_as_int(v), lane));
}
__device__ __forceinline__ void ws_block_range(int64_t n_items, int64_t& beg, int64_t& end)
{
    const int nblk = gridDim.x;
    int b = blockIdx.x;
    if ((nblk & 7) == 0) b = (b & 7) * (nblk >> 3) + (b >> 3);
    const int64_t per = (n_items + nblk - 1) / nblk;
    beg = (int64_t)b * per;
    end = beg + per < n_items ? beg + per : n_items;
    if (beg > n_items) beg = n_items;
}
__device__ __forceinline__ void ws_wave_items(int64_t n_items, int ilv, int wave, int64_t& i0, int64_t& step, int64_t& end)
{
    if (ilv > 0 && (gridDim.x & 7) == 0) {
        const int x = blockIdx.x & 7, lb = blockIdx.x >> 3, nbx = gridDim.x >> 3;
        const int64_t per8 = (n_items + 7) / 8;
        const int64_t b8 = (int64_t)x * per8;
        end = b8 + per8 < n_items ? b8 + per8 : n_items;
        i0 = b8 + (int64_t)lb * 4 + wave;
        step = (int64_t)nbx * 4;
    } else {
        int64_t ibeg, iend;
        ws_block_range(n_items, ibeg, iend);
        i0 = ibeg + wave; step = 4; end = iend;
    }
}
__device__ __forceinline__ float ws_wave_sum(float v)
{
#pragma unroll
    for (int o = 32; o > 0; o >>= 1) v += __shfl_xor(v, o, 64);
    return v;
}

struct WsDrop {
    unsigned long long seed;
    unsigned threshold;
    float scale;
    int on;
};
__device__ __forceinline__ unsigned ws_drop_hash(unsigned long long seed, unsigned long long i)
{
    unsigned long long z = seed + i * 0x9E3779B97F4A7C15ull;
    z = (z ^ (z >> 30)) * 0xBF58476D1CE4E5B9ull;
    z = (z ^ (z >> 27)) * 0x94D049BB133111EBull;
    z = z ^ (z >> 31);
    return (unsigned)(z >> 32);
}
__device__ __forceinline__ float ws_drop1(float v, const WsDrop& d, unsigned long long i)
{
    return ws_drop_hash(d.seed, i) >= d.threshold ? v * d.scale : 0.0f;
}
inline WsDrop ws_drop_args(float p, unsigned long long seed)
{
    const double t = (double)p * 4294967296.0;
    return WsDrop{seed, t >= 4294967295.0 ? 4294967295u : (unsigned)t, 1.0f / (1.0f - p), p > 0.0f ? 1 : 0};
}

#endif
```

### weasal_amd/fused.py

```python
import ctypes as C
import os
import weakref

import torch

from . import _lib, ops
from ._lib import check, current_stream

FUSED_BLOCKS = os.environ.get("WEASAL_FUSED_BLOCKS", "1") != "0"
FUSED_INFER = os.environ.get("WEASAL_FUSED_INFER", "1") != "0"
_timed = False


_timed_min_rows = 0


def set_timed(on, min_rows=0):
    global _timed, _timed_min_rows
    _timed = bool(on)
    _timed_min_rows = int(min_rows)


_vp, _i32, _i64, _f32 = C.c_void_p, C.c_int32, C.c_int64, C.c_float


class KPBlockDesc(C.Structure):
    _fields_ = [("q_pts", _vp), ("nq", _i64), ("s_pts", _vp), ("ns", _i64), ("inds", _vp), ("h", _i32),
                ("kernel_points", _vp), ("k", _i32), ("extent", _f32), ("order_q", _vp), ("order_s", _vp),
                ("grid_blob", _vp), ("grid_nb", _i32), ("grid_cells", _i64), ("key_last", _vp), ("grid_radius", _f32),
                ("grid_overflow", _vp), ("t_offsets", _vp), ("t_pairs", _vp),
                ("in_dim", _i32), ("conv_in", _i32), ("conv_out", _i32), ("out_dim", _i32), ("strided", _i32),
                ("slope", _f32),
                ("w1", _vp), ("b1", _vp), ("wk", _vp), ("bk", _vp), ("w2", _vp), ("b2", _vp), ("ws", _vp), ("bs", _vp),
                ("feat", _vp), ("x1", _vp), ("wf", _vp), ("x2", _vp), ("pooled", _vp), ("arg", _vp), ("out", _vp),
                ("dout", _vp), ("dfeat", _vp), ("dw1", _vp), ("db1", _vp), ("dwk", _vp), ("dbk", _vp), ("dw2", _vp),
                ("db2", _vp), ("dws", _vp), ("timed", _i32), ("rows_sorted", _i32), ("infer", _i32), ("dout_pregated", _i32),
                ("gate_dfeat", _i32), ("dfeat_add", _vp)]


class UpUnaryDesc(C.Structure):
    _fields_ = [("xc", _vp), ("nc", _i64), ("c_up", _i32), ("skip", _vp), ("nf", _i64), ("c_skip", _i32),
                ("ups", _vp), ("h_up", _i32), ("t_offsets", _vp), ("t_pairs", _vp),
                ("w", _vp), ("ldw", _i64), ("b", _vp), ("out_dim", _i32), ("relu", _i32), ("slope", _f32),
                ("yc", _vp), ("out", _vp), ("dout", _vp), ("dxc", _vp), ("dskip", _vp), ("dw", _vp), ("db", _vp),
                ("drop_p", _f32), ("drop_seed", C.c_uint64), ("dout_pregated", _i32), ("gate_dxc", _i32)]


_GATES_SET = False


def _bind():
    global _GATES_SET
    lib = _lib.lib()
    if not _GATES_SET:
        C.c_int.in_dll(lib, "ws_block_gates").value = 0 if os.environ.get("WEASAL_BLOCK_GATES", "1") == "0" else 1
        C.c_int.in_dll(lib, "ws_block_fused_infer").value = 1 if FUSED_INFER else 0
        C.c_int.in_dll(lib, "ws_block_gather_residual").value = 0 if os.environ.get("WEASAL_BLOCK_GATHER_RESIDUAL", "1") == "0" else 1
        C.c_int.in_dll(lib, "ws_block_pool_order").value = 0 if os.environ.get("WEASAL_POOL_ORDER", "1") == "0" else 1
        C.c_int.in_dll(lib, "ws_block_packed_k4").value = 0 if os.environ.get("WEASAL_BLOCK_PACKED_K4", "1") == "0" else 1
        if "WEASAL_BLOCK_GROUP_ROWS" in os.environ:
            C.c_int64.in_dll(lib, "ws_block_group_rows").value = int(os.environ["WEASAL_BLOCK_GROUP_ROWS"])
        _GATES_SET = True
    return lib


def timer_records(layer=False):
    lib = _bind()
    out = []
    nq, h, ci, ms, ml = _i64(), _i32(), _i32(), _f32(), _f32()
    for i in range(lib.ws_timer_count()):
        check(lib.ws_timer_read(i, C.byref(nq), C.byref(h), C.byref(ci), C.byref(ms)))
        if layer:
            check(lib.ws_timer_read_layer(i, C.byref(ml)))
            out.append((nq.value, h.value, ci.value, ms.value, ml.value))
        else:
            out.append((nq.value, h.value, ci.value, ms.value))
    return out


def timer_reset():
    _bind().ws_timer_reset()


def _p(t):
    return None if t is None else t.data_ptr()


def _scratch(nbytes, device):
    return torch.empty(max(int(nbytes), 256), dtype=torch.uint8, device=device)


class _Geom:
    __slots__ = ("q_pts", "s_pts", "inds", "kp", "extent", "order_q", "order_s", "dx_route", "grid", "table", "in_dim", "conv_in",
                 "conv_out", "out_dim", "strided", "slope", "has", "rows_sorted", "infer", "skip_slot", "link_in", "link_out")

    def fill(self, d):
        d.q_pts, d.nq = self.q_pts.data_ptr(), self.q_pts.shape[0]
        d.s_pts, d.ns = self.s_pts.data_ptr(), self.s_pts.shape[0]
        d.inds, d.h = self.inds.data_ptr(), self.inds.shape[1]
        d.kernel_points, d.k, d.extent = self.kp.data_ptr(), self.kp.shape[0], float(self.extent)
        d.order_q, d.order_s = _p(self.order_q), _p(self.order_s)
        if self.grid is not None:
            g = self.grid
            d.grid_blob, d.grid_nb, d.grid_cells = g.blob.data_ptr(), g.nb, g.cells
            d.key_last, d.grid_radius, d.grid_overflow = g.key_last.data_ptr(), g.radius, g.overflow.data_ptr()
        if self.table is not None:
            d.t_offsets, d.t_pairs = self.table.offsets.data_ptr(), self.table.pairs.data_ptr()
        d.in_dim, d.conv_in, d.conv_out, d.out_dim = self.in_dim, self.conv_in, self.conv_out, self.out_dim
        d.strided, d.slope = 1 if self.strided else 0, float(self.slope)
        d.rows_sorted = 1 if self.rows_sorted else 0
        d.infer = 1 if self.infer else 0


def _al(n):
    return (n + 63) // 64 * 64


class SkipSlot:
    __slots__ = ("grad", "armed", "taken")

    def __init__(self):
        self.grad, self.armed, self.taken = None, False, False


class GateLink:
    __slots__ = ("out", "pregated", "drop", "slope")

    def __init__(self):
        self.out, self.pregated = None, False
        self.drop = None
        self.slope = 0.1


GATE_LINKS = os.environ.get("WEASAL_GATE_LINKS", "1") != "0"


def linear_links(batch, x, eligible):
    if not eligible or batch is None or not GATE_LINKS:
        return None
    return [_link_in(batch, x), None]


def linear_links_done(batch, links, out, relu):
    if links is not None and batch is not None:
        links[1] = _link_out(batch, out, relu=relu)


def _link_in(batch, x):
    link = getattr(batch, "gate_link_in", None)
    if (link is None or not GATE_LINKS or link.out is None or link.out() is not x or not torch.is_grad_enabled()
            or not x.requires_grad or x.dtype != torch.float32):
        return None
    return link


def _link_out(batch, out, relu=True):
    link = getattr(batch, "gate_link_out", None)
    if link is not None and GATE_LINKS and relu and torch.is_grad_enabled() and out.requires_grad:
        link.out = weakref.ref(out)
        return link
    return None


class _SkipTap(torch.autograd.Function):
    @staticmethod
    def forward(ctx, x, slot):
        ctx.slot = slot
        return x.view_as(x)

    @staticmethod
    def backward(ctx, g):
        slot = ctx.slot
        if slot.armed and not slot.taken and slot.grad is None:
            slot.grad = g
            return None, None
        return g, None


def skip_tap(x, slot):
    if slot is None or not slot.armed or not torch.is_grad_enabled() or not x.requires_grad:
        return x
    return _SkipTap.apply(x, slot)


class _KPBlockFn(torch.autograd.Function):

    @staticmethod
    def forward(ctx, feat, w1, b1, wk, bk, w2, b2, wsc, bsc, geom):
        lib = _bind()
        dev = feat.device
        feat = feat.contiguous()
        g = geom
        nq, ns = g.q_pts.shape[0], g.s_pts.shape[0]
        k = g.kp.shape[0]
        fused_layer = g.infer and g.conv_in == 32 and g.conv_out == 32 and not g.rows_sorted and FUSED_INFER
        sizes = [ns * g.conv_in if w1 is not None else 0, 0 if fused_layer else nq * k * g.conv_in, nq * g.conv_out if w2 is not None else 0,
                 nq * g.in_dim if (g.strided and w2 is not None) else 0, nq * g.in_dim if (g.strided and w2 is not None) else 0]
        offs, tot = [], 0
        for s in sizes:
            offs.append(tot)
            tot += _al(s)
        arena = torch.empty(max(tot, 64), dtype=torch.float32, device=dev)
        base = arena.data_ptr()
        out = torch.empty((nq, g.out_dim), dtype=torch.float32, device=dev)
        d = KPBlockDesc()
        g.fill(d)
        wkc = wk.contiguous()
        d.w1, d.b1, d.wk, d.bk, d.w2, d.b2, d.ws, d.bs = _p(w1), _p(b1), wkc.data_ptr(), _p(bk), _p(w2), _p(b2), _p(wsc), _p(bsc)
        d.feat = feat.data_ptr()
        d.x1 = base + 4 * offs[0] if sizes[0] else None
        d.wf = base + 4 * offs[1] if sizes[1] else None
        d.x2 = base + 4 * offs[2] if sizes[2] else None
        d.pooled = base + 4 * offs[3] if sizes[3] else None
        d.arg = base + 4 * offs[4] if sizes[4] else None
        d.out = out.data_ptr()
        d.timed = 1 if (_timed and g.q_pts.shape[0] >= _timed_min_rows) else 0
        nbytes = lib.ws_kpblock_fwd_scratch_bytes(C.byref(d))
        if nbytes < 0:
            check(1)
        scratch = _scratch(nbytes, dev)
        check(lib.ws_kpblock_fwd(C.byref(d), scratch.data_ptr(), scratch.numel(), current_stream()))
        ctx.geom, ctx.offs, ctx.sizes = g, offs, sizes
        ctx.save_for_backward(feat, arena, out, w1, b1, wkc, bk, w2, b2, wsc, bsc)
        return out

    @staticmethod
    def backward(ctx, dout):
        lib = _bind()
        feat, arena, out, w1, b1, wk, bk, w2, b2, wsc, bsc = ctx.saved_tensors
        g, offs, sizes = ctx.geom, ctx.offs, ctx.sizes
        dev = feat.device
        dout = dout.contiguous()
        nq, ns = g.q_pts.shape[0], g.s_pts.shape[0]
        need = ctx.needs_input_grad
        d = KPBlockDesc()
        g.fill(d)
        d.w1, d.b1, d.wk, d.bk, d.w2, d.b2, d.ws, d.bs = _p(w1), _p(b1), wk.data_ptr(), _p(bk), _p(w2), _p(b2), _p(wsc), _p(bsc)
        base = arena.data_ptr()
        d.feat = feat.data_ptr()
        d.x1 = base + 4 * offs[0] if sizes[0] else None
        d.wf = base + 4 * offs[1]
        d.x2 = base + 4 * offs[2] if sizes[2] else None
        d.pooled = base + 4 * offs[3] if sizes[3] else None
        d.arg = base + 4 * offs[4] if sizes[4] else None
        d.out, d.dout = out.data_ptr(), dout.data_ptr()
        dfeat = torch.empty_like(feat) if need[0] else None
        d.dfeat = _p(dfeat)
        slot = getattr(g, "skip_slot", None)
        extra = None
        if slot is not None:
            slot.taken = True
            extra, slot.grad = slot.grad, None
            if extra is not None and (dfeat is None or extra.shape != feat.shape or extra.dtype != torch.float32):
                raise _lib.WeasalHipError("skip gradient %s does not match the block input %s" % (tuple(extra.shape), tuple(feat.shape)))
            if extra is not None:
                extra = extra.contiguous()
                global skip_slot_hits
                skip_slot_hits += 1
        d.dfeat_add = _p(extra)
        lo, li = getattr(g, "link_out", None), getattr(g, "link_in", None)
        d.dout_pregated = 1 if (lo is not None and lo.pregated) else 0
        if li is not None:
            complete = slot is None or not slot.armed or extra is not None
            li.pregated = bool(dfeat is not None and complete and (extra is None or (g.strided and w2 is not None)))
            d.gate_dfeat = 1 if li.pregated else 0
            global gate_link_hits
            gate_link_hits += d.gate_dfeat
        grads = [None if p is None else torch.empty_like(p) for p in (w1, b1, wk, bk, w2, b2, wsc)]
        d.dw1, d.db1, d.dwk, d.dbk, d.dw2, d.db2, d.dws = [_p(t) for t in grads]
        nbytes = lib.ws_kpblock_bwd_scratch_bytes(C.byref(d))
        if nbytes < 0:
            check(1)
        scratch = _scratch(nbytes, dev)
        check(lib.ws_kpblock_bwd(C.byref(d), scratch.data_ptr(), scratch.numel(), current_stream()))
        dw1, db1, dwk, dbk, dw2, db2, dws = grads
        dbs = db2.clone() if (bsc is not None and db2 is not None) else None
        return dfeat, dw1, db1, dwk, dbk, dw2, db2, dws, dbs, None


gate_link_hits = 0
skip_slot_hits = 0
SKIP_SLOTS = os.environ.get("WEASAL_SKIP_SLOTS", "1") != "0"


def _conv_ok(conv, x):
    return (FUSED_BLOCKS and x.is_cuda and x.dtype == torch.float32 and not conv.deformable and conv.K == 15
            and conv.KP_influence == 'linear' and conv.aggregation_mode == 'sum' and ops.kpconv_gather is _KPCONV_GATHER)


_KPCONV_GATHER = ops.kpconv_gather


def _geometry(conv, q_pts, s_pts, inds, strided):
    g = _Geom()
    g.q_pts, g.s_pts = ops._f32c(q_pts), ops._f32c(s_pts)
    g.inds = ops._as_index(inds)
    g.kp, g.extent = conv.kernel_points, conv.KP_extent
    g.order_q, g.order_s = ops._order_for(g.q_pts), ops._order_for(g.s_pts)
    g.dx_route, g.grid = ops.dx_route(g.inds, g.q_pts, g.s_pts, "block")
    g.table = None
    g.skip_slot = None
    g.link_in = g.link_out = None
    g.strided = strided
    g.rows_sorted = ops.rows_cutoff_pays(g.inds, conv.radius)
    g.infer = not torch.is_grad_enabled()
    return g


MIN_ROWS = int(os.environ.get("WEASAL_FUSED_MIN_ROWS", "0"))


def kpblock_eligible(block, x):
    conv = block.KPConv
    if not _conv_ok(conv, x) or x.shape[0] < MIN_ROWS:
        return False
    dims = [conv.out_channels]
    if hasattr(block, "unary2"):
        dims += [block.out_dim, block.in_dim, conv.in_channels]
    return all(v % 4 == 0 for v in dims)


def simple_block(block, x, batch, q_pts, s_pts, inds):
    conv = block.KPConv
    g = _geometry(conv, q_pts, s_pts, inds, 'strided' in block.block_name)
    g.in_dim = g.conv_in = conv.in_channels
    g.conv_out = g.out_dim = conv.out_channels
    g.slope = 0.1
    if torch.is_grad_enabled() and x.requires_grad and g.dx_route == ops.TABLE:
        g.table = ops.transposed_table(g.inds, g.s_pts.shape[0])
    if getattr(batch, "skip_slot", None) is None:
        g.link_in = _link_in(batch, x)
    out = _KPBlockFn.apply(x, None, None, conv.weights, block.batch_norm.epilogue_bias(), None, None, None, None, g)
    g.link_out = _link_out(batch, out)
    return out


def resnetb_block(block, x, batch, q_pts, s_pts, inds):
    conv = block.KPConv
    strided = 'strided' in block.block_name
    g = _geometry(conv, q_pts, s_pts, inds, strided)
    slot = getattr(batch, "skip_slot", None) if strided else None
    if slot is not None and SKIP_SLOTS and torch.is_grad_enabled() and x.requires_grad and x.dtype == torch.float32:
        g.skip_slot = slot
        slot.armed = True
    g.in_dim, g.conv_in, g.conv_out, g.out_dim = block.in_dim, conv.in_channels, conv.out_channels, block.out_dim
    g.slope = 0.1
    if torch.is_grad_enabled() and (g.dx_route == ops.TABLE or strided):
        g.table = ops.transposed_table(g.inds, g.s_pts.shape[0])
    u1 = block.unary1 if isinstance(block.unary1, torch.nn.Module) and hasattr(block.unary1, "mlp") else None
    us = block.unary_shortcut if hasattr(block.unary_shortcut, "mlp") else None
    if getattr(batch, "skip_slot", None) is None or g.skip_slot is not None:
        g.link_in = _link_in(batch, x)
    out = _KPBlockFn.apply(x,
                           u1.mlp.weight if u1 is not None else None, u1.batch_norm.epilogue_bias() if u1 is not None else None,
                           conv.weights, block.batch_norm_conv.epilogue_bias(),
                           block.unary2.mlp.weight, block.unary2.batch_norm.epilogue_bias(),
                           us.mlp.weight if us is not None else None, us.batch_norm.epilogue_bias() if us is not None else None,
                           g)
    g.link_out = _link_out(batch, out)
    return out


class _UpUnaryFn(torch.autograd.Function):

    @staticmethod
    def forward(ctx, xc, skip, w, b, ups, table, relu, drop_p=0.0, drop_seed=0, links=None):
        lib = _bind()
        dev = xc.device
        xc, skip, w = xc.contiguous(), skip.contiguous(), w.contiguous()
        nc, c_up = xc.shape
        nf, c_skip = skip.shape
        out_dim = w.shape[0]
        yc = torch.empty((max(nc, 1), out_dim), dtype=torch.float32, device=dev)
        out = torch.empty((nf, out_dim), dtype=torch.float32, device=dev)
        d = UpUnaryDesc()
        d.xc, d.nc, d.c_up, d.skip, d.nf, d.c_skip = xc.data_ptr(), nc, c_up, skip.data_ptr(), nf, c_skip
        d.ups, d.h_up = ups.data_ptr(), ups.shape[1]
        d.w, d.ldw, d.b, d.out_dim, d.relu, d.slope = w.data_ptr(), w.stride(0), _p(b), out_dim, 1 if relu else 0, 0.1
        d.yc, d.out = yc.data_ptr(), out.data_ptr()
        d.drop_p, d.drop_seed = float(drop_p), int(drop_seed)
        nbytes = lib.ws_upunary_fwd_scratch_bytes(C.byref(d))
        if nbytes < 0:
            check(1)
        scratch = _scratch(nbytes, dev)
        check(lib.ws_upunary_fwd(C.byref(d), scratch.data_ptr(), scratch.numel(), current_stream()))
        ctx.table, ctx.relu, ctx.drop = table, relu, (float(drop_p), int(drop_seed))
        ctx.links = links if links is not None else [None, None]
        ctx.save_for_backward(xc, skip, w, b, ups, out)
        return out

    @staticmethod
    def backward(ctx, dout):
        lib = _bind()
        xc, skip, w, b, ups, out = ctx.saved_tensors
        dev = xc.device
        dout = dout.contiguous()
        nc, c_up = xc.shape
        nf, c_skip = skip.shape
        out_dim = w.shape[0]
        d = UpUnaryDesc()
        d.xc, d.nc, d.c_up, d.skip, d.nf, d.c_skip = xc.data_ptr(), nc, c_up, skip.data_ptr(), nf, c_skip
        d.ups, d.h_up = ups.data_ptr(), ups.shape[1]
        d.t_offsets, d.t_pairs = ctx.table.offsets.data_ptr(), ctx.table.pairs.data_ptr()
        d.w, d.ldw, d.b, d.out_dim, d.relu, d.slope = w.data_ptr(), w.stride(0), _p(b), out_dim, 1 if ctx.relu else 0, 0.1
        d.out, d.dout = out.data_ptr(), dout.data_ptr()
        d.drop_p, d.drop_seed = ctx.drop
        li, lo = ctx.links
        d.dout_pregated = 1 if (lo is not None and lo.pregated) else 0
        if li is not None:
            li.pregated = bool(ctx.needs_input_grad[0])
            d.gate_dxc = 1 if li.pregated else 0
            global gate_link_hits
            gate_link_hits += d.gate_dxc
        dxc, dskip = torch.empty_like(xc), torch.empty_like(skip)
        dw = torch.empty_like(w)
        db = torch.empty_like(b) if b is not None else None
        d.dxc, d.dskip, d.dw, d.db = dxc.data_ptr(), dskip.data_ptr(), dw.data_ptr(), _p(db)
        nbytes = lib.ws_upunary_bwd_scratch_bytes(C.byref(d))
        if nbytes < 0:
            check(1)
        scratch = _scratch(nbytes, dev)
        check(lib.ws_upunary_bwd(C.byref(d), scratch.data_ptr(), scratch.numel(), current_stream()))
        return dxc, dskip, dw, db, None, None, None, None, None, None


def upunary_eligible(x, skip, unary):
    return (FUSED_BLOCKS and x.is_cuda and x.dtype == torch.float32 and skip.dtype == torch.float32
            and ops.kpconv_gather is _KPCONV_GATHER and x.shape[1] % 32 == 0 and skip.shape[1] % 32 == 0
            and unary.out_dim % 32 == 0 and x.shape[0] > 0 and skip.shape[0] >= MIN_ROWS)


def upunary(x, skip, unary, ups, drop=None, batch=None):
    ups = ops._as_index(ups)
    table = ops.col0_table(ups, x.shape[0]) if torch.is_grad_enabled() else None
    links = [_link_in(batch, x) if batch is not None else None, None]
    if drop is not None:
        if unary.no_relu:
            raise _lib.WeasalHipError("upunary: the fused dropout follows the unary's LeakyReLU")
        out = _UpUnaryFn.apply(x, skip, unary.mlp.weight, unary.batch_norm.epilogue_bias(), ups, table, True, float(drop[0]), int(drop[1]),
                               links)
        if batch is not None:
            links[1] = _link_out(batch, out)
            if links[1] is not None:
                links[1].drop = (float(drop[0]), int(drop[1]))
        return out
    out = _UpUnaryFn.apply(x, skip, unary.mlp.weight, unary.batch_norm.epilogue_bias(), ups, table, not unary.no_relu, 0.0, 0, links)
    if batch is not None:
        links[1] = _link_out(batch, out, relu=not unary.no_relu)
    return out
```

Before: 32.87 million points/s.

## Fuse last decoder unary with head MLP via chained GEMM kernel

Adds a head-chain path that runs the last upsample unary's skip GEMM and the head_mlp GEMM in one chained kernel that keeps the intermediate row tile on chip. The backward pass likewise chains the logits-to-dh, dh-to-dd and dd-to-dskip GEMMs, then skips the separate dskip GEMM in upunary_bwd. The goal is to cut kernel launches and HBM round trips of the full-resolution intermediate activations at the network head. It adds a large new kernel with tricky plumbing for gating, dropout and residual handling, and the logits GEMM is still launched separately.

```diff
diff --git a/include/weasal_hip.h b/include/weasal_hip.h
--- a/include/weasal_hip.h
+++ b/include/weasal_hip.h
@@ -313,6 +313,19 @@
 int64_t ws_upunary_bwd_scratch_bytes(const ws_upunary* d);
 int ws_upunary_fwd(const ws_upunary* d, void* scratch, int64_t scratch_bytes, void* stream);
 int ws_upunary_bwd(const ws_upunary* d, void* scratch, int64_t scratch_bytes, void* stream);
+
+typedef struct ws_headchain {
+    ws_upunary up;
+    const float* wm; const float* bm; int32_t mid; int32_t mlp_relu;
+    float* h;
+    const float* wl; int32_t classes;
+    const float* dz; float* dh; float* dd;
+} ws_headchain;
+int64_t ws_headchain_fwd_scratch_bytes(const ws_headchain* d);
+int64_t ws_headchain_bwd_scratch_bytes(const ws_headchain* d);
+int ws_headchain_fwd(const ws_headchain* d, void* scratch, int64_t scratch_bytes, void* stream);
+int ws_headchain_bwd(const ws_headchain* d, void* scratch, int64_t scratch_bytes, void* stream);
+int ws_headchain_variant(const ws_headchain* d, int32_t backward, char* out, int32_t cap);
 
 int ws_gemm_xb_epilogue_strided(const float* x, int64_t m, int32_t k, int64_t ldx, const float* b, int64_t b_row_stride,
                                 int64_t b_col_stride, int32_t n, const float* bias, const float* residual, int64_t ldr,
diff --git a/weasal_amd/_lib.py b/weasal_amd/_lib.py
--- a/weasal_amd/_lib.py
+++ b/weasal_amd/_lib.py
@@ -107,6 +107,11 @@
     "ws_upunary_bwd_scratch_bytes": (_i64, [_vp]),
     "ws_upunary_fwd": (C.c_int, [_vp, _vp, _i64, _vp]),
     "ws_upunary_bwd": (C.c_int, [_vp, _vp, _i64, _vp]),
+    "ws_headchain_fwd_scratch_bytes": (_i64, [_vp]),
+    "ws_headchain_bwd_scratch_bytes": (_i64, [_vp]),
+    "ws_headchain_fwd": (C.c_int, [_vp, _vp, _i64, _vp]),
+    "ws_headchain_bwd": (C.c_int, [_vp, _vp, _i64, _vp]),
+    "ws_headchain_variant": (C.c_int, [_vp, _i32, C.c_char_p, _i32]),
     "ws_gemm_xb_epilogue_strided": (C.c_int, [_vp, _i64, _i32, _i64, _vp, _i64, _i64, _i32, _vp, _vp, _i64, _i32, _f32, _vp, _i64,
                                               _vp, _i64, _vp]),
     "ws_gemm_xb_gated_strided": (C.c_int, [_vp, _i64, _i32, _i64, _vp, _i64, _i64, _i32, _vp, _vp, _i64, _i32, _f32, _vp, _i64, _f32,
diff --git a/weasal_amd/architectures.py b/weasal_amd/architectures.py
--- a/weasal_amd/architectures.py
+++ b/weasal_amd/architectures.py
@@ -154,6 +154,13 @@
                         and torch.is_grad_enabled() and x.dtype == torch.float32 and fused.upunary_eligible(x, skips[-1], nxt)):
                     drop = (float(self.dropout), int(torch.randint(0, 1 << 62, (1,)).item()))
                     dropped = True
+                if (block_i + 2 == nd and (drop is not None or not self.dropout or not self.training)
+                        and fused.headchain_eligible(x, skips[-1], nxt, self.head_mlp, self.head_softmax)):
+                    batch.gate_link_in, batch.gate_link_out = link, None
+                    x = fused.headchain(x, fused.skip_tap(skips.pop(), slots.pop()), nxt, self.head_mlp, self.head_softmax,
+                                        batch.upsamples[block_op.layer_ind - 1], drop, batch)
+                    batch.gate_link_in = None
+                    return x
                 batch.gate_link_in, batch.gate_link_out = link, fused.GateLink()
                 link = batch.gate_link_out
                 x = self._fused_upsample_unary(x, fused.skip_tap(skips.pop(), slots.pop()), block_op, nxt, batch, drop)
diff --git a/weasal_amd/csrc/blocks.hip b/weasal_amd/csrc/blocks.hip
--- a/weasal_amd/csrc/blocks.hip
+++ b/weasal_amd/csrc/blocks.hip
@@ -8,6 +8,7 @@
 extern "C" int ws_block_fused_infer = 1;
 extern "C" int ws_block_pool_order = 1;
 extern "C" int ws_block_packed_k4 = 1;
+extern "C" int ws_block_head_chain = 1;
 
 namespace {
 
@@ -417,7 +418,7 @@
                                        d->relu ? 1 : 0, d->slope, d->out, d->out_dim, tmp, tmp_bytes, st);
 }
 
-int upunary_bwd(const ws_upunary* d, Arena& ar, hipStream_t st, bool run)
+int upunary_bwd(const ws_upunary* d, Arena& ar, hipStream_t st, bool run, bool have_dskip = false)
 {
     float* dz = ar.take<float>(d->nf * d->out_dim);
     float* dyc = ar.take<float>(d->nc * d->out_dim);
@@ -454,8 +455,9 @@
     }
     Leaves leaves(grp, (hipStream_t)st);
     WS_TRY(leaves.add(g, d->nf, d->out_dim, d->out_dim, d->skip, d->c_skip, d->c_skip, d->dw + d->c_up, cw, t_skip, b_skip));
-    WS_TRY(ws_gemm_xb_epilogue_strided(g, d->nf, d->out_dim, d->out_dim, d->w + d->c_up, d->ldw, 1, d->c_skip, nullptr, nullptr, 0, 0, 0.0f,
-                                       d->dskip, d->c_skip, tmp, tmp_bytes, st));
+    if (!have_dskip)
+        WS_TRY(ws_gemm_xb_epilogue_strided(g, d->nf, d->out_dim, d->out_dim, d->w + d->c_up, d->ldw, 1, d->c_skip, nullptr, nullptr, 0, 0, 0.0f,
+                                           d->dskip, d->c_skip, tmp, tmp_bytes, st));
     WS_TRY(ws_closest_pool_bwd(g, d->nf, 1, d->out_dim, d->t_offsets, d->t_pairs, d->nc, dyc, st));
     WS_TRY(leaves.add(dyc, d->nc, d->out_dim, d->out_dim, d->xc, d->c_up, d->c_up, d->dw, cw, t_up, b_up));
     WS_TRY(ws_gemm_xb_gated_strided(dyc, d->nc, d->out_dim, d->out_dim, d->w, d->ldw, 1, d->c_up, nullptr, nullptr, 0, 0, 0.0f,
@@ -463,9 +465,142 @@
     return leaves.flush();
 }
 
+int check_headchain(const ws_headchain* d, bool bwd)
+{
+    WS_REQUIRE(d, "NULL descriptor");
+    WS_TRY(check_upunary(&d->up));
+    WS_REQUIRE(d->up.nc > 0 && d->up.nf > 0, "head chain: empty level");
+    WS_REQUIRE(d->wm && d->h && d->mid >= 1, "head chain: NULL argument / bad width");
+    if (d->mid % 32 || ((uintptr_t)d->wm & 15u))
+        return ws_fail(WS_ERR_UNSUPPORTED, "head chain: head_mlp's width must be a multiple of 32 (mid=%d) and its weight 16-byte aligned", d->mid);
+    if (bwd) WS_REQUIRE(d->wl && d->dz && d->dh && d->dd && d->classes >= 1, "head chain: NULL gradient buffer");
+    return WS_OK;
+}
+
+inline int chain_or_alone(const ws_xb_problem* q, int count, hipStream_t st)
+{
+    if (ws_block_head_chain) return ws_priv_gemm_xb_chain(q, count, st);
+    for (int i = 0; i < count; ++i) WS_TRY(ws_priv_gemm_xb_group(q + i, 1, st));
+    return WS_OK;
+}
+
+void headchain_fwd_members(const ws_headchain* d, const float* up, void* tmp, int64_t tmp_bytes, ws_xb_problem (&q)[2])
+{
+    const ws_upunary& u = d->up;
+    const bool gather = ws_block_gather_residual != 0;
+    q[0] = xb_problem(u.skip, u.nf, u.c_skip, u.c_skip, u.w + u.c_up, 1, u.ldw, u.out_dim, u.b, gather ? u.yc : up, u.out_dim,
+                      u.relu ? 1 : 0, u.slope, nullptr, 0, 0.0f, u.out, u.out_dim, tmp, tmp_bytes);
+    if (gather) { q[0].res_rows = u.ups; q[0].res_rows_ld = u.h_up; q[0].res_nrows = u.nc; }
+    q[0].drop_p = u.drop_p; q[0].drop_seed = u.drop_seed;
+    q[1] = xb_problem(u.out, u.nf, u.out_dim, u.out_dim, d->wm, 1, u.out_dim, d->mid, d->bm, nullptr, 0, d->mlp_relu ? 1 : 0, u.slope,
+                      nullptr, 0, 0.0f, d->h, d->mid, tmp, tmp_bytes);
+}
+
+void headchain_bwd_members(const ws_headchain* d, void* tmp, int64_t tmp_bytes, ws_xb_problem (&q)[3])
+{
+    const ws_upunary& u = d->up;
+    q[0] = xb_problem(d->dz, u.nf, d->classes, d->classes, d->wl, -1, 1, d->mid, nullptr, nullptr, 0, 0, 0.0f,
+                      d->mlp_relu ? d->h : nullptr, d->mid, u.slope, d->dh, d->mid, tmp, tmp_bytes);
+    q[1] = xb_problem(d->dh, u.nf, d->mid, d->mid, d->wm, -1, 1, u.out_dim, nullptr, nullptr, 0, 0, 0.0f,
+                      u.relu ? u.out : nullptr, u.out_dim, u.slope, d->dd, u.out_dim, tmp, tmp_bytes);
+    q[1].drop_p = u.drop_p; q[1].drop_seed = u.drop_seed;
+    q[2] = xb_problem(d->dd, u.nf, u.out_dim, u.out_dim, u.w + u.c_up, u.ldw, 1, u.c_skip, nullptr, nullptr, 0, 0, 0.0f,
+                      nullptr, 0, 0.0f, u.dskip, u.c_skip, tmp, tmp_bytes);
+}
+
+int headchain_fwd(const ws_headchain* d, Arena& ar, hipStream_t st, bool run)
+{
+    const ws_upunary& u = d->up;
+    float* up = ar.take<float>(u.nf * u.out_dim);
+    const int64_t tmp_bytes = max3(max3(ws_gemm_xb_scratch_bytes(u.nc, u.c_up, u.out_dim), ws_gemm_xb_scratch_bytes(u.nf, u.c_skip, u.out_dim), 16),
+                                   ws_gemm_xb_scratch_bytes(u.nf, u.out_dim, d->mid), 0);
+    void* tmp = ar.take<char>(tmp_bytes);
+    if (!run) return WS_OK;
+    WS_REQUIRE(u.yc, "yc buffer missing");
+    WS_TRY(ws_gemm_xb_epilogue_strided(u.xc, u.nc, u.c_up, u.c_up, u.w, 1, u.ldw, u.out_dim, nullptr, nullptr, 0, 0, 0.0f, u.yc, u.out_dim, tmp,
+                                       tmp_bytes, st));
+    if (!ws_block_gather_residual) WS_TRY(ws_closest_pool_fwd(u.yc, u.nc, u.out_dim, u.ups, u.nf, u.h_up, up, st));
+    ws_xb_problem q[2];
+    headchain_fwd_members(d, up, tmp, tmp_bytes, q);
+    return chain_or_alone(q, 2, st);
+}
+
+int headchain_bwd(const ws_headchain* d, Arena& ar, hipStream_t st, bool run)
+{
+    const ws_upunary& u0 = d->up;
+    const int64_t tmp_bytes = max3(max3(ws_gemm_xb_scratch_bytes(u0.nf, d->classes, d->mid), ws_gemm_xb_scratch_bytes(u0.nf, d->mid, u0.out_dim), 16),
+                                   ws_gemm_xb_scratch_bytes(u0.nf, u0.out_dim, u0.c_skip), 0);
+    void* tmp = ar.take<char>(tmp_bytes);
+    ws_upunary u = u0;
+    u.dout = d->dd;
+    u.dout_pregated = u.relu ? 1 : 0;
+    if (!run) return upunary_bwd(&u, ar, st, false, true);
+    WS_REQUIRE(u.dw && u.dxc && u.dskip && u.t_offsets && u.t_pairs, "NULL gradient buffer / table");
+    ws_xb_problem q[3];
+    headchain_bwd_members(d, tmp, tmp_bytes, q);
+    WS_TRY(chain_or_alone(q, 3, st));
+    return upunary_bwd(&u, ar, st, true, true);
+}
+
 }
 
 extern "C" {
+
+int64_t ws_headchain_fwd_scratch_bytes(const ws_headchain* d)
+{
+    if (check_headchain(d, false)) return -1;
+    Arena ar(nullptr, 0);
+    headchain_fwd(d, ar, nullptr, false);
+    return arena_bytes(ar);
+}
+
+int64_t ws_headchain_bwd_scratch_bytes(const ws_headchain* d)
+{
+    if (check_headchain(d, true)) return -1;
+    Arena ar(nullptr, 0);
+    headchain_bwd(d, ar, nullptr, false);
+    return arena_bytes(ar);
+}
+
+int ws_headchain_fwd(const ws_headchain* d, void* scratch, int64_t scratch_bytes, void* stream)
+{
+    WS_TRY(check_headchain(d, false));
+    WS_REQUIRE(scratch && ((uintptr_t)scratch & 15u) == 0, "scratch must be a 16-byte aligned device buffer");
+    Arena plan(nullptr, 0);
+    headchain_fwd(d, plan, nullptr, false);
+    if (arena_bytes(plan) > scratch_bytes) return ws_fail(WS_ERR_CAPACITY, "scratch too small: %lld < %lld bytes", (long long)scratch_bytes, (long long)arena_bytes(plan));
+    Arena ar(scratch, scratch_bytes);
+    return headchain_fwd(d, ar, (hipStream_t)stream, true);
+}
+
+int ws_headchain_bwd(const ws_headchain* d, void* scratch, int64_t scratch_bytes, void* stream)
+{
+    WS_TRY(check_headchain(d, true));
+    WS_REQUIRE(scratch && ((uintptr_t)scratch & 15u) == 0, "scratch must be a 16-byte aligned device buffer");
+    Arena plan(nullptr, 0);
+    headchain_bwd(d, plan, nullptr, false);
+    if (arena_bytes(plan) > scratch_bytes) return ws_fail(WS_ERR_CAPACITY, "scratch too small: %lld < %lld bytes", (long long)scratch_bytes, (long long)arena_bytes(plan));
+    Arena ar(scratch, scratch_bytes);
+    return headchain_bwd(d, ar, (hipStream_t)stream, true);
+}
+
+int ws_headchain_variant(const ws_headchain* d, int32_t backward, char* out, int32_t cap)
+{
+    WS_TRY(check_headchain(d, backward != 0));
+    WS_REQUIRE(out && cap > 0, "NULL output");
+    if (!ws_block_head_chain) {
+        snprintf(out, (size_t)cap, "single launches: ws_block_head_chain = 0");
+        return WS_OK;
+    }
+    if (backward) {
+        ws_xb_problem q[3];
+        headchain_bwd_members(d, nullptr, 0, q);
+        return ws_gemm_xb_chain_variant(q, 3, out, cap);
+    }
+    ws_xb_problem q[2];
+    headchain_fwd_members(d, d->up.out, nullptr, 0, q);
+    return ws_gemm_xb_chain_variant(q, 2, out, cap);
+}
 
 int64_t ws_kpblock_fwd_scratch_bytes(const ws_kpblock* d)
 {
diff --git a/weasal_amd/csrc/gemm.hip b/weasal_amd/csrc/gemm.hip
--- a/weasal_amd/csrc/gemm.hip
+++ b/weasal_amd/csrc/gemm.hip
@@ -512,6 +512,290 @@
             if (gate.y || gate.mask || gate.drop.on) xb_gate4(o, gate, row, c);
             *reinterpret_cast<float4*>(y + row * ldy + c) = o;
         }
+    }
+}
+
+constexpr int CHAIN_MAX = 3;
+constexpr int CHAIN_GEN_K = 16;
+struct XbChainLink {
+    const float* b; int ldb, bcs, k, n;
+    float* y; int64_t ldy;
+    const float* bias; const float* residual; int64_t ldr; int act; float slope; XbGate gate;
+};
+struct XbChain { const float* x; int64_t m, ldx; XbChainLink l[CHAIN_MAX]; };
+static_assert(sizeof(XbChain) < 4096, "the chain travels in the kernel arguments");
+
+template <int NT>
+__device__ __forceinline__ void xb_rows_math(f32x16 (&acc)[NT], int64_t row, int64_t m, int h, const XbChainLink& L, bool addzero)
+{
+    const int n = L.n;
+    const int64_t rr = row < m ? row : m - 1;
+    const float* rrow = xb_res_row(L.residual, L.ldr, L.gate, rr);
+#pragma unroll
+    for (int i = 0; i < NT; ++i) {
+        if (32 * i >= n) continue;
+        float4 v[4];
+        int col[4];
+#pragma unroll
+        for (int g = 0; g < 4; ++g) {
+            col[g] = 32 * i + 8 * g + 4 * h;
+            v[g] = make_float4(acc[i][4 * g + 0], acc[i][4 * g + 1], acc[i][4 * g + 2], acc[i][4 * g + 3]);
+        }
+        if (rrow) {
+            float4 rq[4];
+#pragma unroll
+            for (int g = 0; g < 4; ++g) rq[g] = *reinterpret_cast<const float4*>(rrow + col[g]);
+#pragma unroll
+            for (int g = 0; g < 4; ++g) { v[g].x += rq[g].x; v[g].y += rq[g].y; v[g].z += rq[g].z; v[g].w += rq[g].w; }
+        }
+        if (L.bias || addzero) {
+#pragma unroll
+            for (int g = 0; g < 4; ++g) {
+                const float4 bq = L.bias ? *reinterpret_cast<const float4*>(L.bias + col[g]) : make_float4(0.f, 0.f, 0.f, 0.f);
+                v[g].x += bq.x; v[g].y += bq.y; v[g].z += bq.z; v[g].w += bq.w;
+            }
+        }
+        if (L.act) {
+#pragma unroll
+            for (int g = 0; g < 4; ++g) {
+                v[g].x = v[g].x > 0.0f ? v[g].x : v[g].x * L.slope;
+                v[g].y = v[g].y > 0.0f ? v[g].y : v[g].y * L.slope;
+                v[g].z = v[g].z > 0.0f ? v[g].z : v[g].z * L.slope;
+                v[g].w = v[g].w > 0.0f ? v[g].w : v[g].w * L.slope;
+            }
+        }
+        if (L.gate.y || L.gate.drop.on) {
+#pragma unroll
+            for (int g = 0; g < 4; ++g) xb_gate4(v[g], L.gate, rr, col[g]);
+        }
+#pragma unroll
+        for (int g = 0; g < 4; ++g) {
+            acc[i][4 * g + 0] = v[g].x; acc[i][4 * g + 1] = v[g].y; acc[i][4 * g + 2] = v[g].z; acc[i][4 * g + 3] = v[g].w;
+        }
+    }
+}
+
+template <int NT>
+__device__ __forceinline__ void xb_rows_store_staged(const f32x16 (&acc)[NT], int64_t row0, int64_t m, int n, int lane,
+                                                     float* __restrict__ y, int64_t ldy, float* __restrict__ stage)
+{
+    const int idx = lane & 31, h = lane >> 5;
+    const int r8 = lane >> 3, c4 = lane & 7;
+#pragma unroll
+    for (int i = 0; i < NT; ++i) {
+        if (32 * i >= n) continue;
+#pragma unroll
+        for (int g = 0; g < 4; ++g)
+            *reinterpret_cast<float4*>(&stage[idx * XB_STAGE_LD + 8 * g + 4 * h]) =
+                make_float4(acc[i][4 * g + 0], acc[i][4 * g + 1], acc[i][4 * g + 2], acc[i][4 * g + 3]);
+        asm volatile("s_waitcnt lgkmcnt(0)" ::: "memory");
+        __builtin_amdgcn_wave_barrier();
+        const int col = 32 * i + 4 * c4;
+#pragma unroll
+        for (int p = 0; p < 4; ++p) {
+            const int rl = r8 + 8 * p;
+            const int64_t row = row0 + rl;
+            const float4 v = *reinterpret_cast<const float4*>(&stage[rl * XB_STAGE_LD + 4 * c4]);
+            if (row < m) *reinterpret_cast<float4*>(y + row * ldy + col) = v;
+        }
+        asm volatile("s_waitcnt lgkmcnt(0)" ::: "memory");
+        __builtin_amdgcn_wave_barrier();
+    }
+}
+
+template <int NT>
+__device__ __forceinline__ void chain_w_offsets(const XbChainLink& L, int t, int& woff, int& wlds)
+{
+    constexpr int BN = 32 * NT;
+    const bool wtr = L.ldb == 1;
+    const int c = wtr ? t / 8 : t % BN, q = wtr ? t % 8 : t / BN;
+    const int col = c < L.n ? c : L.n - 1;
+    woff = (4 * q * L.ldb + col * L.bcs) * 4;
+    wlds = ((((c >> 5) * 4 + (q >> 1)) * 2 + (q & 1)) * 32 + (c & 31)) * 4;
+}
+#define WS_CHAIN_LOAD_W(chunk)                                                                                              \
+    do {                                                                                                                    \
+        const int so__ = (chunk) * 32 * L.ldb * 4;                                                                          \
+        if (L.ldb == 1) {                                                                                                   \
+            _Pragma("unroll") for (int i = 0; i < NT; ++i) {                                                                \
+                const int to__ = 32 * i < L.n ? 32 * i * L.bcs * 4 : 0;                                                     \
+                const u32x4 v__ = __builtin_amdgcn_raw_buffer_load_b128(wsrd, woff, so__ + to__, 0);                        \
+                wv[i] = make_float4(__uint_as_float(v__.x), __uint_as_float(v__.y), __uint_as_float(v__.z), __uint_as_float(v__.w)); \
+            }                                                                                                               \
+        } else {                                                                                                            \
+            _Pragma("unroll") for (int i = 0; i < NT; ++i) {                                                                \
+                const int to__ = so__ + i * (8 / NT) * 4 * L.ldb * 4;                                                       \
+                wv[i].x = __uint_as_float(__builtin_amdgcn_raw_buffer_load_b32(wsrd, woff, to__, 0));                       \
+                wv[i].y = __uint_as_float(__builtin_amdgcn_raw_buffer_load_b32(wsrd, woff, to__ + L.ldb * 4, 0));           \
+                wv[i].z = __uint_as_float(__builtin_amdgcn_raw_buffer_load_b32(wsrd, woff, to__ + L.ldb * 8, 0));           \
+                wv[i].w = __uint_as_float(__builtin_amdgcn_raw_buffer_load_b32(wsrd, woff, to__ + L.ldb * 12, 0));          \
+            }                                                                                                               \
+        }                                                                                                                   \
+    } while (0)
+#define WS_CHAIN_STORE_W(buf)                                                                                               \
+    do {                                                                                                                    \
+        const int ws__ = L.ldb == 1 ? 1024 : (8 / NT) * 128;                                                                \
+        _Pragma("unroll") for (int i = 0; i < NT; ++i) *reinterpret_cast<float4*>(&Ws[(buf) * (NT * 1024) + wlds + i * ws__]) = wv[i]; \
+    } while (0)
+#define WS_CHAIN_MFMA(bq)                                                                                                   \
+    do {                                                                                                                    \
+        _Pragma("unroll") for (int j = 0; j < 4; ++j) {                                                                     \
+            __builtin_amdgcn_sched_barrier(0);                                                                              \
+            _Pragma("unroll") for (int i = 0; i < NT; ++i) {                                                                \
+                const float4 a4 = *reinterpret_cast<const float4*>(wb + (i * 4 + j) * 256);                                 \
+                acc[i] = __builtin_amdgcn_mfma_f32_32x32x2f32(a4.x, bq(j, 0), acc[i], 0, 0, 0);                             \
+                acc[i] = __builtin_amdgcn_mfma_f32_32x32x2f32(a4.y, bq(j, 1), acc[i], 0, 0, 0);                             \
+                acc[i] = __builtin_amdgcn_mfma_f32_32x32x2f32(a4.z, bq(j, 2), acc[i], 0, 0, 0);                             \
+                acc[i] = __builtin_amdgcn_mfma_f32_32x32x2f32(a4.w, bq(j, 3), acc[i], 0, 0, 0);                             \
+            }                                                                                                               \
+        }                                                                                                                   \
+    } while (0)
+
+template <int NT>
+__device__ __forceinline__ void chain_link_global(f32x16 (&acc)[NT], const float* __restrict__ x, int64_t m, int64_t ldx,
+                                                  const XbChainLink& L, float* __restrict__ Ws, int t, int wave, int idx, int h)
+{
+#pragma unroll
+    for (int i = 0; i < NT; ++i)
+#pragma unroll
+        for (int r = 0; r < 16; ++r) acc[i][r] = 0.0f;
+    const auto wsrd = __builtin_amdgcn_make_buffer_rsrc(const_cast<float*>(L.b), 0,
+                                                        (int)(((int64_t)(L.k - 1) * L.ldb + (int64_t)(L.n - 1) * L.bcs + 1) * 4), 0x00020000);
+    const int64_t brow0 = (int64_t)blockIdx.x * 128;
+    const int64_t brows = m - brow0 < 128 ? m - brow0 : 128;
+    const auto xsrd = __builtin_amdgcn_make_buffer_rsrc(const_cast<float*>(x + brow0 * ldx), 0, (int)(((brows - 1) * ldx + L.k) * 4), 0x00020000);
+    int woff, wlds;
+    chain_w_offsets<NT>(L, t, woff, wlds);
+    float4 wv[NT];
+    const int xoff = (int)((wave * 32 + idx) * ldx + 4 * h) * 4;
+    float xn[4][4], xc[4][4];
+    auto load_x = [&](int chunk) {
+#pragma unroll
+        for (int j = 0; j < 4; ++j) {
+            const u32x4 v = __builtin_amdgcn_raw_buffer_load_b128(xsrd, xoff + 32 * j, chunk * 128, 0);
+            xn[j][0] = __uint_as_float(v.x); xn[j][1] = __uint_as_float(v.y); xn[j][2] = __uint_as_float(v.z); xn[j][3] = __uint_as_float(v.w);
+        }
+    };
+    const int nch = L.k / 32, last = nch - 1;
+    WS_CHAIN_LOAD_W(0);
+    load_x(0);
+    {
+        float4 w0[NT];
+#pragma unroll
+        for (int i = 0; i < NT; ++i) w0[i] = wv[i];
+        WS_CHAIN_LOAD_W(last < 1 ? last : 1);
+        const int ws0 = L.ldb == 1 ? 1024 : (8 / NT) * 128;
+#pragma unroll
+        for (int i = 0; i < NT; ++i) *reinterpret_cast<float4*>(&Ws[wlds + i * ws0]) = w0[i];
+    }
+    __syncthreads();
+    for (int c = 0; c < nch; ++c) {
+#pragma unroll
+        for (int j = 0; j < 4; ++j)
+#pragma unroll
+            for (int e = 0; e < 4; ++e) xc[j][e] = xn[j][e];
+        WS_CHAIN_STORE_W((c + 1) & 1);
+        load_x(c + 1 < last ? c + 1 : last);
+        WS_CHAIN_LOAD_W(c + 2 < last ? c + 2 : last);
+        const float* wb = &Ws[(c & 1) * (NT * 1024) + (h * 32 + idx) * 4];
+#define WS_CHAIN_BQ(j, e) (xc[j][e])
+        WS_CHAIN_MFMA(WS_CHAIN_BQ);
+#undef WS_CHAIN_BQ
+        __syncthreads();
+    }
+}
+
+template <int NT>
+__device__ __forceinline__ void chain_link_regs(const f32x16 (&src)[NT], f32x16 (&acc)[NT], const XbChainLink& L,
+                                                float* __restrict__ Ws, int t, int idx, int h)
+{
+#pragma unroll
+    for (int i = 0; i < NT; ++i)
+#pragma unroll
+        for (int r = 0; r < 16; ++r) acc[i][r] = 0.0f;
+    const auto wsrd = __builtin_amdgcn_make_buffer_rsrc(const_cast<float*>(L.b), 0,
+                                                        (int)(((int64_t)(L.k - 1) * L.ldb + (int64_t)(L.n - 1) * L.bcs + 1) * 4), 0x00020000);
+    int woff, wlds;
+    chain_w_offsets<NT>(L, t, woff, wlds);
+    float4 wv[NT];
+    const int nch = L.k / 32, last = nch - 1;
+    WS_CHAIN_LOAD_W(0);
+    WS_CHAIN_STORE_W(0);
+    WS_CHAIN_LOAD_W(last < 1 ? last : 1);
+    __syncthreads();
+#pragma unroll
+    for (int c = 0; c < NT; ++c) {
+        if (c >= nch) break;
+        WS_CHAIN_STORE_W((c + 1) & 1);
+        WS_CHAIN_LOAD_W(c + 2 < last ? c + 2 : last);
+        const float* wb = &Ws[(c & 1) * (NT * 1024) + (h * 32 + idx) * 4];
+#define WS_CHAIN_BQ(j, e) (src[c][4 * (j) + (e)])
+        WS_CHAIN_MFMA(WS_CHAIN_BQ);
+#undef WS_CHAIN_BQ
+        __syncthreads();
+    }
+}
+
+template <int NT>
+__device__ __forceinline__ void chain_link_gen(f32x16 (&acc)[NT], const float* __restrict__ x, int64_t m, int64_t ldx, int64_t row,
+                                               const XbChainLink& L, float* __restrict__ Ws, int t, int h)
+{
+    const int k = L.k, n = L.n, kp = (k + 3) & ~3;
+    for (int e = t; e < kp * n / 4; e += 256)
+        reinterpret_cast<float4*>(Ws)[e] = e < k * n / 4 ? reinterpret_cast<const float4*>(L.b)[e] : make_float4(0.f, 0.f, 0.f, 0.f);
+    const float* xr = x + (row < m ? row : m - 1) * ldx;
+    float xv[CHAIN_GEN_K];
+#pragma unroll
+    for (int kk = 0; kk < CHAIN_GEN_K; ++kk) xv[kk] = kk < k ? xr[kk] : 0.0f;
+    __syncthreads();
+#pragma unroll
+    for (int i = 0; i < NT; ++i) {
+#pragma unroll
+        for (int r = 0; r < 16; ++r) acc[i][r] = 0.0f;
+        if (32 * i >= n) continue;
+#pragma unroll
+        for (int g = 0; g < 4; ++g) {
+            const float* bc = Ws + 32 * i + 8 * g + 4 * h;
+            float4 v = make_float4(0.f, 0.f, 0.f, 0.f);
+#pragma unroll
+            for (int kk = 0; kk < CHAIN_GEN_K; ++kk) {
+                if (kk >= kp) break;
+                const float4 w = *reinterpret_cast<const float4*>(bc + kk * n);
+                v.x = fmaf(xv[kk], w.x, v.x); v.y = fmaf(xv[kk], w.y, v.y); v.z = fmaf(xv[kk], w.z, v.z); v.w = fmaf(xv[kk], w.w, v.w);
+            }
+            acc[i][4 * g + 0] = v.x; acc[i][4 * g + 1] = v.y; acc[i][4 * g + 2] = v.z; acc[i][4 * g + 3] = v.w;
+        }
+    }
+    __syncthreads();
+}
+#undef WS_CHAIN_LOAD_W
+#undef WS_CHAIN_STORE_W
+#undef WS_CHAIN_MFMA
+
+template <int NT, int GEN>
+__global__ __launch_bounds__(256) __attribute__((amdgpu_waves_per_eu(3))) void gemm_xb2_chain_kernel(const XbChain a)
+{
+    __shared__ __attribute__((aligned(16))) float Ws[2 * NT * 1024];
+    __shared__ __attribute__((aligned(16))) float Stage[4 * XB_STAGE_FLOATS];
+    const int t = threadIdx.x;
+    const int wave = __builtin_amdgcn_readfirstlane(t >> 6);
+    const int lane = t & 63;
+    const int idx = lane & 31, h = lane >> 5;
+    const int64_t row0 = (int64_t)blockIdx.x * 128 + wave * 32;
+    const int64_t row = row0 + idx;
+    float* stage = &Stage[wave * XB_STAGE_FLOATS];
+    f32x16 r0[NT], r1[NT];
+    if (GEN) chain_link_gen<NT>(r0, a.x, a.m, a.ldx, row, a.l[0], Ws, t, h);
+    else chain_link_global<NT>(r0, a.x, a.m, a.ldx, a.l[0], Ws, t, wave, idx, h);
+    xb_rows_math<NT>(r0, row, a.m, h, a.l[0], GEN != 0);
+    if (a.l[0].y) xb_rows_store_staged<NT>(r0, row0, a.m, a.l[0].n, lane, a.l[0].y, a.l[0].ldy, stage);
+    chain_link_regs<NT>(r0, r1, a.l[1], Ws, t, idx, h);
+    xb_rows_math<NT>(r1, row, a.m, h, a.l[1], false);
+    if (a.l[1].y) xb_rows_store_staged<NT>(r1, row0, a.m, a.l[1].n, lane, a.l[1].y, a.l[1].ldy, stage);
+    if (GEN) {
+        chain_link_regs<NT>(r1, r0, a.l[2], Ws, t, idx, h);
+        xb_rows_math<NT>(r0, row, a.m, h, a.l[2], false);
+        if (a.l[2].y) xb_rows_store_staged<NT>(r0, row0, a.m, a.l[2].n, lane, a.l[2].y, a.l[2].ldy, stage);
     }
 }
 
@@ -1422,6 +1706,110 @@
             const int rc = cnt == 1 ? xb_problem_alone(q[ids[off]], stream) : xb2_group_launch(q, plan, ids.data() + off, cnt, st);
             if (rc != WS_OK) return rc;
         }
+    return WS_OK;
+}
+
+struct ChainPlan {
+    int lead;
+    int gen;
+    int nt;
+    dim3 grid;
+    const char* why;
+};
+static const char* chain_member_ok(const ws_xb_problem& a, const XbPlan& p, bool first)
+{
+    if (a.mask) return "byte mask";
+    if (a.n % 32 != 0 || a.n > 128) return "width not a multiple of 32 up to 128";
+    if (p.kind != XB_XB2 || p.splits != 1) return "member is not a single gemm_xb2 launch";
+    if (!first && a.k > 128) return "depth above 128";
+    return nullptr;
+}
+static int chain_plan(const ws_xb_problem* q, int count, ChainPlan& cp)
+{
+    cp = ChainPlan{count, 0, 0, dim3(1), ""};
+    WS_REQUIRE(q && (count == 2 || count == 3), "a chain has 2 or 3 members");
+    XbPlan plan[CHAIN_MAX];
+    for (int i = 0; i < count; ++i) {
+        const ws_xb_problem& a = q[i];
+        WS_REQUIRE(a.m == q[0].m && a.m >= 0 && a.k >= 1 && a.n >= 1 && a.ldx >= a.k && a.ldy >= a.n, "member %d: bad sizes m=%lld k=%d n=%d", i, (long long)a.m, a.k, a.n);
+        WS_REQUIRE(i == 0 || (a.x == q[i - 1].y && a.ldx == q[i - 1].ldy && a.k == q[i - 1].n), "member %d does not read member %d's output", i, i - 1);
+        WS_REQUIRE(!a.residual || a.ldr >= a.n, "member %d: residual leading dimension too small", i);
+        WS_REQUIRE(a.act == 0 || a.act == 1, "member %d: unknown activation %d", i, a.act);
+        WS_REQUIRE(a.drop_p >= 0.0f && a.drop_p < 1.0f, "member %d: bad drop probability %g", i, (double)a.drop_p);
+        WS_REQUIRE(!a.res_rows || (a.residual && a.res_rows_ld >= 1 && a.res_nrows >= 0), "member %d: gathered residual: NULL residual / bad sizes", i);
+        WS_REQUIRE(!a.gate_y || a.ldg >= a.n, "member %d: gate leading dimension too small", i);
+        if (a.m == 0) { cp.why = "(m == 0)"; return WS_OK; }
+        WS_REQUIRE(a.x && a.b && a.y, "member %d: NULL argument", i);
+        const int rc = xb_plan(a.x, a.m, a.k, a.ldx, a.b, a.n, a.bias, a.residual, a.ldr, a.y, a.ldy, a.scratch, a.scratch_bytes,
+                               a.b_row_stride < 0 ? a.n : a.b_row_stride, a.b_col_stride, xb_problem_gate(a), plan[i]);
+        if (rc != WS_OK) return rc;
+    }
+    if (ws_ceil_div(q[0].m, 128) >= (1ll << 31)) { cp.why = "m too large"; return WS_OK; }
+    int first = 0, gen = 0;
+    if (count == 3) {
+        const ws_xb_problem& a = q[0];
+        if (plan[0].kind == XB_SHALLOW && a.k <= CHAIN_GEN_K && a.n % 32 == 0 && a.n <= 128 && !a.mask && (a.b_row_stride < 0 || a.b_row_stride == a.n) &&
+            a.b_col_stride == 1)
+            gen = 1;
+        else
+            first = 1;
+    }
+    int nmax = 0;
+    for (int i = first; i < count; ++i) {
+        if (!(gen && i == 0)) {
+            const char* why = chain_member_ok(q[i], plan[i], i == first);
+            if (why) { cp.why = why; return WS_OK; }
+        }
+        if (q[i].n > nmax) nmax = q[i].n;
+    }
+    cp.lead = first; cp.gen = gen;
+    cp.nt = nmax <= 32 ? 1 : nmax <= 64 ? 2 : 4;
+    cp.grid = dim3((unsigned)ws_ceil_div(q[0].m, 128));
+    return WS_OK;
+}
+
+int ws_priv_gemm_xb_chain(const ws_xb_problem* q, int32_t count, void* stream)
+{
+    ChainPlan cp;
+    const int rc = chain_plan(q, count, cp);
+    if (rc != WS_OK) return rc;
+    for (int i = 0; i < cp.lead; ++i) {
+        const int r1 = xb_problem_alone(q[i], stream);
+        if (r1 != WS_OK) return r1;
+    }
+    if (cp.lead == count) return WS_OK;
+    XbChain a{};
+    a.x = q[cp.lead].x; a.m = q[cp.lead].m; a.ldx = q[cp.lead].ldx;
+    for (int i = cp.lead; i < count; ++i) {
+        const ws_xb_problem& s = q[i];
+        XbChainLink& L = a.l[i - cp.lead];
+        L.b = s.b; L.ldb = (int)(s.b_row_stride < 0 ? s.n : s.b_row_stride); L.bcs = (int)s.b_col_stride; L.k = s.k; L.n = s.n;
+        L.y = s.y; L.ldy = s.ldy; L.bias = s.bias; L.residual = s.residual; L.ldr = s.ldr; L.act = s.act; L.slope = s.slope;
+        L.gate = xb_problem_gate(s);
+    }
+    hipStream_t st = (hipStream_t)stream;
+#define WS_CHAIN(NTV)                                                                  \
+    do {                                                                               \
+        if (cp.gen) gemm_xb2_chain_kernel<NTV, 1><<<cp.grid, 256, 0, st>>>(a);         \
+        else gemm_xb2_chain_kernel<NTV, 0><<<cp.grid, 256, 0, st>>>(a);                \
+    } while (0)
+    if (cp.nt == 1) WS_CHAIN(1);
+    else if (cp.nt == 2) WS_CHAIN(2);
+    else WS_CHAIN(4);
+#undef WS_CHAIN
+    WS_LAUNCH_CHECK();
+    return WS_OK;
+}
+
+int ws_gemm_xb_chain_variant(const void* members, int32_t count, char* out, int32_t cap)
+{
+    WS_REQUIRE(out && cap > 0, "NULL output");
+    const ws_xb_problem* q = (const ws_xb_problem*)members;
+    ChainPlan cp;
+    const int rc = chain_plan(q, count, cp);
+    if (rc != WS_OK) return rc;
+    if (cp.lead == count) snprintf(out, (size_t)cap, "single launches: %s", cp.why);
+    else snprintf(out, (size_t)cap, "gemm_xb2_chain_kernel<NT=%d, GEN=%d> links=%d alone=%d", cp.nt, cp.gen, count - cp.lead, cp.lead);
     return WS_OK;
 }
 
diff --git a/weasal_amd/csrc/ws_common.h b/weasal_amd/csrc/ws_common.h
--- a/weasal_amd/csrc/ws_common.h
+++ b/weasal_amd/csrc/ws_common.h
@@ -73,6 +73,8 @@
 };
 extern "C" int ws_priv_gemm_xb_group(const ws_xb_problem* p, int32_t count, void* stream);
 extern "C" int ws_priv_gemm_xty_group(const ws_xty_problem* p, int32_t count, void* stream);
+extern "C" int ws_priv_gemm_xb_chain(const ws_xb_problem* p, int32_t count, void* stream);
+extern "C" int ws_gemm_xb_chain_variant(const void* members, int32_t count, char* out, int32_t cap);
 
 static inline int ws_grid(int64_t items, int per_block, int max_blocks = 256 * 16)
 {
diff --git a/weasal_amd/fused.py b/weasal_amd/fused.py
--- a/weasal_amd/fused.py
+++ b/weasal_amd/fused.py
@@ -46,6 +46,13 @@
                 ("drop_p", _f32), ("drop_seed", C.c_uint64), ("dout_pregated", _i32), ("gate_dxc", _i32)]
 
 
+class HeadChainDesc(C.Structure):
+    _fields_ = [("up", UpUnaryDesc), ("wm", _vp), ("bm", _vp), ("mid", _i32), ("mlp_relu", _i32), ("h", _vp),
+                ("wl", _vp), ("classes", _i32), ("dz", _vp), ("dh", _vp), ("dd", _vp)]
+
+
+HEAD_CHAIN = os.environ.get("WEASAL_HEAD_CHAIN", "1") != "0"
+
 _GATES_SET = False
 
 
@@ -58,6 +65,7 @@
         C.c_int.in_dll(lib, "ws_block_gather_residual").value = 0 if os.environ.get("WEASAL_BLOCK_GATHER_RESIDUAL", "1") == "0" else 1
         C.c_int.in_dll(lib, "ws_block_pool_order").value = 0 if os.environ.get("WEASAL_POOL_ORDER", "1") == "0" else 1
         C.c_int.in_dll(lib, "ws_block_packed_k4").value = 0 if os.environ.get("WEASAL_BLOCK_PACKED_K4", "1") == "0" else 1
+        C.c_int.in_dll(lib, "ws_block_head_chain").value = 1 if HEAD_CHAIN else 0
         if "WEASAL_BLOCK_GROUP_ROWS" in os.environ:
             C.c_int64.in_dll(lib, "ws_block_group_rows").value = int(os.environ["WEASAL_BLOCK_GROUP_ROWS"])
         _GATES_SET = True
@@ -364,7 +372,12 @@
 class _UpUnaryFn(torch.autograd.Function):
 
     @staticmethod
-    def forward(ctx, xc, skip, w, b, ups, table, relu, drop_p=0.0, drop_seed=0, links=None):
+    def forward(ctx, xc, skip, w, b, ups, table, relu, drop_p=0.0, drop_seed=0, links=None, wm_t=None, bm=None, wl_t=None, bl=None,
+                mlp_relu=True):
+        ctx.head = wm_t is not None
+        if ctx.head:
+            return _head_forward(ctx, xc, skip, w, b, wm_t, bm, wl_t, bl, ups, table, relu, mlp_relu, (float(drop_p), int(drop_seed)),
+                                 links[0] if links is not None else None)
         lib = _bind()
         dev = xc.device
         xc, skip, w = xc.contiguous(), skip.contiguous(), w.contiguous()
@@ -391,6 +404,8 @@
 
     @staticmethod
     def backward(ctx, dout):
+        if ctx.head:
+            return _head_backward(ctx, dout)
         lib = _bind()
         xc, skip, w, b, ups, out = ctx.saved_tensors
         dev = xc.device
@@ -421,7 +436,7 @@
             check(1)
         scratch = _scratch(nbytes, dev)
         check(lib.ws_upunary_bwd(C.byref(d), scratch.data_ptr(), scratch.numel(), current_stream()))
-        return dxc, dskip, dw, db, None, None, None, None, None, None
+        return dxc, dskip, dw, db, None, None, None, None, None, None, None, None, None, None, None
 
 
 def upunary_eligible(x, skip, unary):
@@ -448,3 +463,90 @@
     if batch is not None:
         links[1] = _link_out(batch, out, relu=not unary.no_relu)
     return out
+
+
+def _fill_upunary(d, xc, skip, w, b, ups, relu, drop):
+    d.xc, d.nc, d.c_up, d.skip, d.nf, d.c_skip = xc.data_ptr(), xc.shape[0], xc.shape[1], skip.data_ptr(), skip.shape[0], skip.shape[1]
+    d.ups, d.h_up = ups.data_ptr(), ups.shape[1]
+    d.w, d.ldw, d.b, d.out_dim, d.relu, d.slope = w.data_ptr(), w.stride(0), _p(b), w.shape[0], 1 if relu else 0, 0.1
+    d.drop_p, d.drop_seed = drop
+
+
+def _head_forward(ctx, xc, skip, w, b, wm_t, bm, wl_t, bl, ups, table, relu, mlp_relu, drop, link_in):
+    lib = _bind()
+    dev = xc.device
+    xc, skip, w = xc.contiguous(), skip.contiguous(), w.contiguous()
+    wm, wl = wm_t.t().contiguous(), wl_t.t().contiguous()
+    nf, out_dim, mid, classes = skip.shape[0], w.shape[0], wm.shape[0], wl.shape[0]
+    yc = torch.empty((xc.shape[0], out_dim), dtype=torch.float32, device=dev)
+    out = torch.empty((nf, out_dim), dtype=torch.float32, device=dev)
+    h = torch.empty((nf, mid), dtype=torch.float32, device=dev)
+    d = HeadChainDesc()
+    _fill_upunary(d.up, xc, skip, w, b, ups, relu, drop)
+    d.up.yc, d.up.out = yc.data_ptr(), out.data_ptr()
+    d.wm, d.bm, d.mid, d.mlp_relu, d.h = wm.data_ptr(), _p(bm), mid, 1 if mlp_relu else 0, h.data_ptr()
+    nbytes = lib.ws_headchain_fwd_scratch_bytes(C.byref(d))
+    if nbytes < 0:
+        check(1)
+    scratch = _scratch(nbytes, dev)
+    check(lib.ws_headchain_fwd(C.byref(d), scratch.data_ptr(), scratch.numel(), current_stream()))
+    wl_rows = wl_t.contiguous()
+    logits = torch.empty((nf, classes), dtype=torch.float32, device=dev)
+    ops._xb_launch(lib, h, nf, mid, wl_rows, classes, bl, None, 0.1, logits)
+    ctx.table, ctx.relu, ctx.mlp_relu, ctx.drop, ctx.link_in = table, relu, mlp_relu, drop, link_in
+    ctx.save_for_backward(xc, skip, w, b, ups, out, wm, bm, h, wl, bl, logits)
+    return logits
+
+
+def _head_backward(ctx, dy):
+    lib = _bind()
+    xc, skip, w, b, ups, out, wm, bm, h, wl, bl, logits = ctx.saved_tensors
+    dev = xc.device
+    need = ctx.needs_input_grad
+    dz, dbl = ops._act_bwd_colsum(ops._rowmajor(dy), logits, 0.1, bl is not None and need[13])
+    dh = torch.empty_like(h)
+    dd = torch.empty_like(out)
+    dxc, dskip, dw = torch.empty_like(xc), torch.empty_like(skip), torch.empty_like(w)
+    db = torch.empty_like(b) if b is not None else None
+    d = HeadChainDesc()
+    _fill_upunary(d.up, xc, skip, w, b, ups, ctx.relu, ctx.drop)
+    d.up.t_offsets, d.up.t_pairs = ctx.table.offsets.data_ptr(), ctx.table.pairs.data_ptr()
+    d.up.out = out.data_ptr()
+    d.up.dxc, d.up.dskip, d.up.dw, d.up.db = dxc.data_ptr(), dskip.data_ptr(), dw.data_ptr(), _p(db)
+    li = ctx.link_in
+    if li is not None:
+        li.pregated = bool(need[0])
+        d.up.gate_dxc = 1 if li.pregated else 0
+        global gate_link_hits
+        gate_link_hits += d.up.gate_dxc
+    d.wm, d.bm, d.mid, d.mlp_relu, d.h = wm.data_ptr(), _p(bm), wm.shape[0], 1 if ctx.mlp_relu else 0, h.data_ptr()
+    d.wl, d.classes, d.dz, d.dh, d.dd = wl.data_ptr(), wl.shape[0], dz.data_ptr(), dh.data_ptr(), dd.data_ptr()
+    nbytes = lib.ws_headchain_bwd_scratch_bytes(C.byref(d))
+    if nbytes < 0:
+        check(1)
+    scratch = _scratch(nbytes, dev)
+    check(lib.ws_headchain_bwd(C.byref(d), scratch.data_ptr(), scratch.numel(), current_stream()))
+    dwl_t = ops._gemm_xty(lib, h, dz) if need[12] else None
+    _, dbm = ops._act_bwd_colsum(dh, None, None, bm is not None and need[11])
+    dwm_t = ops._gemm_xty(lib, out, dh) if need[10] else None
+    return dxc, dskip, dw, db, None, None, None, None, None, None, dwm_t, dbm, dwl_t, dbl, None
+
+
+_MATMUL_EPILOGUE = ops.matmul_epilogue
+
+
+def headchain_eligible(x, skip, unary, head_mlp, head_softmax):
+    return (HEAD_CHAIN and upunary_eligible(x, skip, unary) and not unary.no_relu and ops.matmul_epilogue is _MATMUL_EPILOGUE
+            and head_mlp.in_dim == unary.out_dim and head_mlp.out_dim % 32 == 0 and head_softmax.in_dim == head_mlp.out_dim
+            and not head_softmax.no_relu and not head_mlp.out_f32 and not head_softmax.out_f32 and skip.shape[0] > 0
+            and unary.mlp.weight.dtype == torch.float32)
+
+
+def headchain(x, skip, unary, head_mlp, head_softmax, ups, drop=None, batch=None):
+    ups = ops._as_index(ups)
+    table = ops.col0_table(ups, x.shape[0]) if torch.is_grad_enabled() else None
+    link_in = _link_in(batch, x) if batch is not None else None
+    dr = (float(drop[0]), int(drop[1])) if drop is not None else (0.0, 0)
+    return _UpUnaryFn.apply(x, skip, unary.mlp.weight, unary.batch_norm.epilogue_bias(), ups, table, True, dr[0], dr[1], [link_in, None],
+                            head_mlp.mlp.weight.t(), head_mlp.batch_norm.epilogue_bias(), head_softmax.mlp.weight.t(),
+                            head_softmax.batch_norm.epilogue_bias(), not head_mlp.no_relu)
```

After: 32.89 million points/s (median of 2 runs). Within noise of the previous version (+0.0%).
